# vocdoni/zk-franchise-proof-circuit

Measured on AMD Instinct MI355X. Metric: zkCensus proofs/sec (nLevels=160), higher is better.
Workload: dtype u256 (8 x u32 Montgomery, BN254 Fr/Fq)

## Files before the change

### zk-franchise-proof-circuit_amd/csrc/zkc_finalize.hip

```cpp
#include "zkc_prover.h"
#include "zkc_f29_g1.h"
#include "zkc_f29_g2.h"

namespace zkc {

template <class F>
__device__ XYZZ<F> fb_mul(const Affine<F>* __restrict__ tab, const uint32_t k[8]) {
    XYZZ<F> acc = XYZZ<F>::inf();
    for (int w = 0; w < 32; w++) {
        uint32_t limb = 0;
#pragma unroll
        for (int q = 0; q < 8; q++) limb = (q == (w >> 2)) ? k[q] : limb;
        const uint32_t d = (limb >> (8 * (w & 3))) & 0xff;
        if (d) acc = xyzz_add_affine(acc, tab[w * 255 + d - 1]);
    }
    return acc;
}
__device__ void store_fq_std(uint8_t* out, const Fq& a) {
    uint32_t s[8]; fp_to_std<FqParams>(s, a);
    uint4* d = reinterpret_cast<uint4*>(out);
    d[0] = make_uint4(s[0], s[1], s[2], s[3]); d[1] = make_uint4(s[4], s[5], s[6], s[7]);
}

__device__ G1XYZZ var_mul29(const G1XYZZ& P, const uint32_t k[8], Acc29* tab) {
    if (P.is_inf()) return P;
    f29_pt_set_inf(tab[0]); tab[1] = f29_pt_from_xyzz(P);
    for (int i = 2; i < 16; i++) { Acc29 t = tab[i - 1]; f29_pt_add(t, t, tab[1]); tab[i] = t; }
    Acc29 acc; f29_pt_set_inf(acc);
    for (int w = 63; w >= 0; w--) {
        if (!f29_pt_is_inf(acc)) for (int d = 0; d < 4; d++) f29_pt_dbl(acc, acc);
        uint32_t limb = 0;
#pragma unroll
        for (int q = 0; q < 8; q++) limb = (q == (w >> 3)) ? k[q] : limb;
        const uint32_t dg = (limb >> (4 * (w & 7))) & 15u;
        if (dg) f29_pt_add(acc, acc, tab[dg]);
    }
    return f29_pt_is_inf(acc) ? G1XYZZ::inf() : f29_pt_to_xyzz(acc);
}

__device__ G1XYZZ var_mul29_g(const G1XYZZ& P, const uint32_t k[8], Acc29* __restrict__ tab) {
    if (P.is_inf()) return P;
    { Acc29 one = f29_pt_from_xyzz(P), t = one; tab[1] = one; for (int i = 2; i < 16; i++) { f29_pt_add(t, t, one); tab[i] = t; } }
    Acc29 acc; f29_pt_set_inf(acc);
    for (int w = 63; w >= 0; w--) {
        if (!f29_pt_is_inf(acc)) for (int d = 0; d < 4; d++) f29_pt_dbl(acc, acc);
        uint32_t limb = 0;
#pragma unroll
        for (int q = 0; q < 8; q++) limb = (q == (w >> 3)) ? k[q] : limb;
        const uint32_t dg = (limb >> (4 * (w & 7))) & 15u;
        if (dg) { const Acc29 e = tab[dg]; f29_pt_add(acc, acc, e); }
    }
    return f29_pt_is_inf(acc) ? G1XYZZ::inf() : f29_pt_to_xyzz(acc);
}

template <class P>
__device__ P fold_const(const P* __restrict__ tab, const FinalizeArgs& a, int q) {
    if (a.dc[q] == 255) return P::inf();
    return xyzz_add(tab[0], xyzz_add(tab[1 + a.dc[q]], tab[1 + a.fold_n + a.ds[q]]));
}
extern "C" __global__ void __launch_bounds__(256)
zkc_finalize(FinalizeArgs a) {
    __shared__ G1XYZZ sh[8];
    __shared__ Acc29 tab[2][16];
    const int q = blockIdx.x, wave = threadIdx.x >> 6, lane = threadIdx.x & 63;
    uint32_t r[8], s[8];
    { const uint4* p = reinterpret_cast<const uint4*>(a.rs + 64 * (size_t)q); uint4 x = p[0], y = p[1], z = p[2], w = p[3];
      r[0] = x.x; r[1] = x.y; r[2] = x.z; r[3] = x.w; r[4] = y.x; r[5] = y.y; r[6] = y.z; r[7] = y.w;
      s[0] = z.x; s[1] = z.y; s[2] = z.z; s[3] = z.w; s[4] = w.x; s[5] = w.y; s[6] = w.z; s[7] = w.w; }
    const int nq = gridDim.x;
    uint8_t* out = a.out + 256 * (size_t)q;
    if (wave == 0 && lane < 2) {
        const G1XYZZ P = lane == 0 ? xyzz_add(a.r1[nq + 3 * q + 0], fold_const(a.foldA, a, q)) : xyzz_add(a.r1[nq + 3 * q + 1], fold_const(a.foldB1, a, q));
        sh[lane] = var_mul29(P, lane == 0 ? s : r, tab[lane]);
    } else if (wave == 1 && lane < 5) {
        uint32_t k[8];
        if (lane == 2) { Fr rs = fp_from_std<FrParams>(r) * fp_from_std<FrParams>(s); fp_to_std<FrParams>(k, rs); }
        else {
#pragma unroll
            for (int i = 0; i < 8; i++) k[i] = (lane == 0 || lane == 4) ? r[i] : s[i];
        }
        const G1Affine* tb = lane <= 2 ? a.tblDelta1 : lane == 3 ? a.tblAlpha1 : a.tblBeta1;
        const G1XYZZ v = fb_mul<Fq>(tb, k);
        sh[2 + lane] = v;
        if (lane == 0) {
            const G1XYZZ A = xyzz_add(a.r1[nq + 3 * q + 0], fold_const(a.foldA, a, q));
            G1Affine p = xyzz_to_affine(xyzz_add(xyzz_add_affine(A, a.alpha1), v));
            store_fq_std(out, p.x); store_fq_std(out + 32, p.y);
        }
    } else if (wave == 2 && lane == 0) {
        const G2XYZZ sd = fb_mul<Fq2>(a.tblDelta2, s);
        G2Affine p = xyzz_to_affine(xyzz_add(xyzz_add_affine(xyzz_add(a.r2[q], fold_const(a.foldB2, a, q)), a.beta2), sd));
        store_fq_std(out + 64, p.x.c0); store_fq_std(out + 96, p.x.c1); store_fq_std(out + 128, p.y.c0); store_fq_std(out + 160, p.y.c1);
    }
    __syncthreads();
    if (threadIdx.x == 0) {
        G1XYZZ c = xyzz_add(xyzz_add(a.r1[nq + 3 * q + 2], fold_const(a.foldC, a, q)), a.r1[q]);
        c = xyzz_add(c, sh[0]); c = xyzz_add(c, sh[5]); c = xyzz_add(c, sh[1]); c = xyzz_add(c, sh[6]); c = xyzz_add(c, sh[4]);
        G1Affine p = xyzz_to_affine(c);
        store_fq_std(out + 192, p.x); store_fq_std(out + 224, p.y);
    }
}

__device__ __forceinline__ void load_rs(const FinalizeArgs& a, int q, uint32_t r[8], uint32_t s[8]) {
    const uint4* p = reinterpret_cast<const uint4*>(a.rs + 64 * (size_t)q); const uint4 x = p[0], y = p[1], z = p[2], w = p[3];
    r[0] = x.x; r[1] = x.y; r[2] = x.z; r[3] = x.w; r[4] = y.x; r[5] = y.y; r[6] = y.z; r[7] = y.w;
    s[0] = z.x; s[1] = z.y; s[2] = z.z; s[3] = z.w; s[4] = w.x; s[5] = w.y; s[6] = w.z; s[7] = w.w;
}
extern "C" __global__ void __launch_bounds__(64)
zkc_finalize_products(FinalizeArgs a, int nq) {
    const int q = blockIdx.x * 64 + threadIdx.x, task = blockIdx.y;
    if (q >= nq) return;
    uint32_t r[8], s[8]; load_rs(a, q, r, s);
    G1XYZZ* res1 = reinterpret_cast<G1XYZZ*>(a.scratch);
    G2XYZZ* res2 = reinterpret_cast<G2XYZZ*>(res1 + 7 * (size_t)nq);
    Acc29* tabs = reinterpret_cast<Acc29*>(res2 + nq);
    if (task < 2) {
        const G1XYZZ P = task == 0 ? xyzz_add(a.r1[nq + 3 * q + 0], fold_const(a.foldA, a, q)) : xyzz_add(a.r1[nq + 3 * q + 1], fold_const(a.foldB1, a, q));
        res1[(size_t)task * nq + q] = var_mul29_g(P, task == 0 ? s : r, tabs + ((size_t)task * nq + q) * 16);
    } else if (task == 3) {
        return;
    } else if (task < 7) {
        uint32_t k[8];
        if (task == 4) { Fr rs = fp_from_std<FrParams>(r) * fp_from_std<FrParams>(s); fp_to_std<FrParams>(k, rs); }
        else {
#pragma unroll
            for (int i = 0; i < 8; i++) k[i] = (task == 2 || task == 6) ? r[i] : s[i];
        }
        const G1Affine* tb = task <= 4 ? a.tblDelta1 : task == 5 ? a.tblAlpha1 : a.tblBeta1;
        res1[(size_t)task * nq + q] = fb_mul<Fq>(tb, k);
    } else {
        res2[q] = fb_mul<Fq2>(a.tblDelta2, s);
    }
}
extern "C" __global__ void __launch_bounds__(64)
zkc_finalize_combine(FinalizeArgs a, int nq) {
    const int q = blockIdx.x * 64 + threadIdx.x, role = blockIdx.y;
    if (q >= nq) return;
    const G1XYZZ* res1 = reinterpret_cast<const G1XYZZ*>(a.scratch);
    const G2XYZZ* res2 = reinterpret_cast<const G2XYZZ*>(res1 + 7 * (size_t)nq);
    uint8_t* out = a.out + 256 * (size_t)q;
    if (role == 0) {
        const G1XYZZ A = xyzz_add(a.r1[nq + 3 * q + 0], fold_const(a.foldA, a, q));
        G1Affine p = xyzz_to_affine(xyzz_add(xyzz_add_affine(A, a.alpha1), res1[2 * (size_t)nq + q]));
        store_fq_std(out, p.x); store_fq_std(out + 32, p.y);
    } else if (role == 1) {
        G1XYZZ c = xyzz_add(xyzz_add(a.r1[nq + 3 * q + 2], fold_const(a.foldC, a, q)), a.r1[q]);
        c = xyzz_add(c, res1[0 * (size_t)nq + q]); c = xyzz_add(c, res1[5 * (size_t)nq + q]); c = xyzz_add(c, res1[1 * (size_t)nq + q]);
        c = xyzz_add(c, res1[6 * (size_t)nq + q]); c = xyzz_add(c, res1[4 * (size_t)nq + q]);
        G1Affine p = xyzz_to_affine(c);
        store_fq_std(out + 192, p.x); store_fq_std(out + 224, p.y);
    } else {
        G2Affine p = xyzz_to_affine(xyzz_add(xyzz_add_affine(xyzz_add(a.r2[q], fold_const(a.foldB2, a, q)), a.beta2), res2[q]));
        store_fq_std(out + 64, p.x.c0); store_fq_std(out + 96, p.x.c1); store_fq_std(out + 128, p.y.c0); store_fq_std(out + 160, p.y.c1);
    }
}

extern "C" __global__ void __launch_bounds__(64) zkc_fb4_build_g1(const G1XYZZ* __restrict__ bases, int nbases, G1XYZZ* __restrict__ out) {
    const int t = blockIdx.x * 64 + threadIdx.x, b = t >> 6, w = t & 63;
    if (b >= nbases) return;
    G1XYZZ* o = out + (size_t)t * FB4_ROW;
    const G1XYZZ B = bases[b];
    if (B.is_inf()) { for (int d = 0; d < FB4_ROW; d++) o[d] = G1XYZZ::inf(); return; }
    Acc29 P = f29_pt_from_xyzz(B);
    for (int i = 0; i < 4 * w; i++) f29_pt_dbl(P, P);
    Acc29 acc = P; o[0] = f29_pt_to_xyzz(acc);
    for (int d = 1; d < FB4_ROW; d++) { f29_pt_add(acc, acc, P); o[d] = f29_pt_to_xyzz(acc); }
}
extern "C" __global__ void __launch_bounds__(64) zkc_fb4_build_g2(G2XYZZ B, G2XYZZ beta2, G2XYZZ beta2_base, G2XYZZ* __restrict__ out) {
    const int w = threadIdx.x;
    if (w == 0) { out[(size_t)FB4_WIN * FB4_ROW] = beta2; out[(size_t)FB4_WIN * FB4_ROW + 1] = beta2_base; }
    G2XYZZ* o = out + (size_t)w * FB4_ROW;
    Acc29G2 P = f29g2_pt_from_xyzz(B);
    for (int i = 0; i < 4 * w; i++) f29g2_pt_dbl(P, P);
    Acc29G2 acc = P; o[0] = f29g2_pt_to_xyzz(acc);
    for (int d = 1; d < FB4_ROW; d++) { f29g2_pt_add(acc, acc, P); o[d] = f29g2_pt_to_xyzz(acc); }
}
int fb4_build(zkc_ctx* ctx, hipStream_t st, const G1XYZZ* d_bases, int nbases, G1XYZZ* d_out, const G2XYZZ& delta2, const G2XYZZ& beta2, const G2XYZZ& beta2_base, G2XYZZ* d_out2) {
    hipLaunchKernelGGL(zkc_fb4_build_g1, dim3(nbases), dim3(64), 0, st, d_bases, nbases, d_out);
    hipLaunchKernelGGL(zkc_fb4_build_g2, dim3(1), dim3(64), 0, st, delta2, beta2, beta2_base, d_out2);
    hipError_t e = hipGetLastError();
    if (e != hipSuccess) return zkc_fail(ctx, ZKC_ERR_HIP, std::string("zkc_fb4_build: ") + hipGetErrorString(e));
    return ZKC_OK;
}
extern "C" __global__ void __launch_bounds__(256) zkc_blind_scalars(BlindArgs a) {
    const int q = blockIdx.y >> 1, sec = blockIdx.y & 1;
    const uint32_t j = blockIdx.x * 256 + threadIdx.x, cnt = sec ? a.nB[q] : a.nA[q];
    if (j >= cnt) return;
    const uint32_t* map = sec ? a.mapB[q] : a.mapA[q];
    const uint32_t idx = map ? map[j] : j;
    const uint4* kp = reinterpret_cast<const uint4*>(a.rs + 64 * (size_t)q + (sec ? 0 : 32)); const uint4 k0 = kp[0], k1 = kp[1];
    const uint32_t ks[8] = {k0.x, k0.y, k0.z, k0.w, k1.x, k1.y, k1.z, k1.w};
    const uint4* wp = reinterpret_cast<const uint4*>(a.w[q] + 8 * (size_t)idx); const uint4 w0 = wp[0], w1 = wp[1];
    const uint32_t ws[8] = {w0.x, w0.y, w0.z, w0.w, w1.x, w1.y, w1.z, w1.w};
    uint4* o = reinterpret_cast<uint4*>(a.out[q] + ((size_t)sec * a.nv + idx) * 8);
    if ((ws[0] | ws[1] | ws[2] | ws[3] | ws[4] | ws[5] | ws[6] | ws[7]) == 0) { o[0] = make_uint4(0, 0, 0, 0); o[1] = make_uint4(0, 0, 0, 0); return; }
    uint32_t pr[8]; fp_to_std<FrParams>(pr, fp_from_std<FrParams>(ws) * fp_from_std<FrParams>(ks));
    o[0] = make_uint4(pr[0], pr[1], pr[2], pr[3]); o[1] = make_uint4(pr[4], pr[5], pr[6], pr[7]);
}
int blind_scalars_launch(zkc_ctx* ctx, hipStream_t st, const BlindArgs& a, int nproofs) {
    uint32_t mx = 1; for (int q = 0; q < nproofs; q++) mx = std::max(mx, std::max(a.nA[q], a.nB[q]));
    hipLaunchKernelGGL(zkc_blind_scalars, dim3((mx + 255) / 256, 2 * nproofs), dim3(256), 0, st, a);
    hipError_t e = hipGetLastError();
    if (e != hipSuccess) return zkc_fail(ctx, ZKC_ERR_HIP, std::string("zkc_blind_scalars: ") + hipGetErrorString(e));
    return ZKC_OK;
}

__device__ __forceinline__ uint32_t nibble_of(const uint32_t k[8], int i) {
    uint32_t limb = 0;
#pragma unroll
    for (int q = 0; q < 8; q++) limb = (q == (i >> 3)) ? k[q] : limb;
    return (limb >> (4 * (i & 7))) & 15u;
}
__device__ __forceinline__ void shfl_xor_words(uint32_t* dst, const uint32_t* src, int nwords, int mask) {
    for (int k = 0; k < nwords; k++) dst[k] = (uint32_t)__shfl_xor((int)src[k], mask, 64);
}
__device__ __forceinline__ Acc29 load_pt29(const G1XYZZ& p) { Acc29 a; if (p.is_inf()) f29_pt_set_inf(a); else a = f29_pt_from_xyzz(p); return a; }
__device__ __forceinline__ Acc29G2 load_pt29(const G2XYZZ& p) { Acc29G2 a; if (p.is_inf()) f29g2_pt_set_inf(a); else a = f29g2_pt_from_xyzz(p); return a; }
__device__ __forceinline__ void store_xyzz(uint8_t* out, const Acc29& p) {
    G1XYZZ* o = reinterpret_cast<G1XYZZ*>(out);
    if (f29_pt_is_inf(p)) *o = G1XYZZ::inf(); else *o = f29_pt_to_xyzz(p);
}
__device__ __forceinline__ void store_xyzz(uint8_t* out, const Acc29G2& p) {
    G2XYZZ* o = reinterpret_cast<G2XYZZ*>(out);
    if (f29g2_pt_is_inf(p)) *o = G2XYZZ::inf(); else *o = f29g2_pt_to_xyzz(p);
}
extern "C" __global__ void __launch_bounds__(64)
zkc_blind_tree_g1(FinalizeArgs a) {
    const int task = blockIdx.x, q = blockIdx.y, nq = gridDim.y, lane = threadIdx.x;
    uint32_t r[8], s[8]; load_rs(a, q, r, s);
    const bool folded = a.dc[q] != 255; const int n = a.fold_n, dc = a.dc[q], ds = a.ds[q];
    const G1XYZZ* res = a.r1 + nq + 5 * (size_t)q;
    Acc29* outv = reinterpret_cast<Acc29*>(a.scratch) + (size_t)q * 10 + task;
    Acc29 v; f29_pt_set_inf(v);
    if (task < 8) {
        int base; bool use_r;
        switch (task) {
            case 0: base = 0; use_r = true; break;
            case 1: base = 0; use_r = true; break;
            case 2: base = folded ? 3 : 1; use_r = false; break;
            case 3: base = folded ? 5 + dc : -1; use_r = false; break;
            case 4: base = folded ? 5 + n + ds : -1; use_r = false; break;
            case 5: base = folded ? 4 : 2; use_r = true; break;
            case 6: base = folded ? 5 + 2 * n + dc : -1; use_r = true; break;
            default: base = folded ? 5 + 3 * n + ds : -1; use_r = true; break;
        }
        uint32_t k[8];
#pragma unroll
        for (int i = 0; i < 8; i++) k[i] = use_r ? r[i] : s[i];
        if (task == 1) { const Fr rs = fp_from_std<FrParams>(r) * fp_from_std<FrParams>(s); fp_to_std<FrParams>(k, rs); }
        if (base >= 0) {
            const uint32_t d = nibble_of(k, lane);
            if (d) v = load_pt29(a.fb4[((size_t)base * FB4_WIN + lane) * FB4_ROW + d - 1]);
            v = wave_sum_g1(v);
        }
    } else if (task == 8) {
        if (lane == 0) v = load_pt29(res[0]);
        else if (lane == 1) v = load_pt29(a.fb4[((size_t)(folded ? 3 : 1) * FB4_WIN) * FB4_ROW]);
        else if (lane == 2 && folded) v = load_pt29(a.foldA[1 + dc]);
        else if (lane == 3 && folded) v = load_pt29(a.foldA[1 + n + ds]);
        v = wave_sum_g1(v, 2);
    } else {
        if (lane == 0) v = load_pt29(res[2]);
        else if (lane == 1 && folded) v = load_pt29(a.foldC[0]);
        else if (lane == 2 && folded) v = load_pt29(a.foldC[1 + dc]);
        else if (lane == 3 && folded) v = load_pt29(a.foldC[1 + n + ds]);
        else if (lane == 4) v = load_pt29(a.r1[q]);
        else if (lane == 5) v = load_pt29(res[3]);
        else if (lane == 6) v = load_pt29(res[4]);
        v = wave_sum_g1(v, 4);
    }
    if (lane == 0) *outv = v;
}
extern "C" __global__ void __launch_bounds__(128)
zkc_blind_tree_g1_out(FinalizeArgs a) {
    const int q = blockIdx.x, wave = threadIdx.x >> 6, lane = threadIdx.x & 63;
    const Acc29* sv = reinterpret_cast<const Acc29*>(a.scratch) + (size_t)q * 10;
    uint8_t* out = a.out_xyzz + 512 * (size_t)q;
    Acc29 v; f29_pt_set_inf(v);
    if (wave == 0) {
        if (lane == 0) v = sv[9]; else if (lane < 8) v = sv[lane];
        v = wave_sum_g1(v, 4);
        if (lane == 0) store_xyzz(out + 384, v);
    } else {
        if (lane == 0) v = sv[8]; else if (lane == 1) v = sv[0];
        v = wave_sum_g1(v, 1);
        if (lane == 0) store_xyzz(out, v);
    }
}
extern "C" __global__ void __launch_bounds__(128)
zkc_blind_tree_g2(FinalizeArgs a) {
    __shared__ Acc29G2 pre;
    const int q = blockIdx.x, wave = threadIdx.x >> 6, lane = threadIdx.x & 63;
    const bool folded = a.dc[q] != 255;
    Acc29G2 v; f29g2_pt_set_inf(v);
    if (wave == 0) {
        uint32_t r[8], s[8]; load_rs(a, q, r, s);
        const uint32_t d = nibble_of(s, lane);
        if (d) v = load_pt29(a.fb4g2[(size_t)lane * FB4_ROW + d - 1]);
        v = wave_sum_g2(v, 32);
    } else {
        if (lane == 0) v = load_pt29(a.r2[q]);
        else if (lane == 1) v = load_pt29(a.fb4g2[(size_t)FB4_WIN * FB4_ROW + (folded ? 1 : 0)]);
        else if (lane == 2 && folded) v = load_pt29(a.foldB2[1 + a.dc[q]]);
        else if (lane == 3 && folded) v = load_pt29(a.foldB2[1 + a.fold_n + a.ds[q]]);
        v = wave_sum_g2(v, 2);
        if (lane == 0) pre = v;
    }
    __syncthreads();
    if (threadIdx.x == 0) { Acc29G2 t; f29g2_pt_add(t, v, pre); store_xyzz(a.out_xyzz + 512 * (size_t)q + 128, t); }
}
int finalize_tree_g2_launch(zkc_ctx* ctx, hipStream_t st, const FinalizeArgs& a, int nproofs) {
    hipLaunchKernelGGL(zkc_blind_tree_g2, dim3(nproofs), dim3(128), 0, st, a);
    hipError_t e = hipGetLastError();
    if (e != hipSuccess) return zkc_fail(ctx, ZKC_ERR_HIP, std::string("zkc_blind_tree_g2: ") + hipGetErrorString(e));
    return ZKC_OK;
}

size_t finalize_scratch_bytes(int nproofs) { return (size_t)nproofs * (7 * sizeof(G1XYZZ) + sizeof(G2XYZZ) + 2 * 16 * sizeof(Acc29)); }

int finalize_launch(zkc_ctx* ctx, hipStream_t st, const FinalizeArgs& a, int nproofs) {
    const bool v1 = sw::on<sw::ZKC_FINALIZE_WAVES>();
    if (a.per == 5) {
        hipLaunchKernelGGL(zkc_blind_tree_g1, dim3(10, nproofs), dim3(64), 0, st, a);
        hipLaunchKernelGGL(zkc_blind_tree_g1_out, dim3(nproofs), dim3(128), 0, st, a);
    }
    else if (v1 || !a.scratch || nproofs <= 2) hipLaunchKernelGGL(zkc_finalize, dim3(nproofs), dim3(256), 0, st, a);
    else {
        hipLaunchKernelGGL(zkc_finalize_products, dim3((nproofs + 63) / 64, 8), dim3(64), 0, st, a, nproofs);
        hipLaunchKernelGGL(zkc_finalize_combine, dim3((nproofs + 63) / 64, 3), dim3(64), 0, st, a, nproofs);
    }
    hipError_t e = hipGetLastError();
    if (e != hipSuccess) return zkc_fail(ctx, ZKC_ERR_HIP, std::string("zkc_finalize: ") + hipGetErrorString(e));
    return ZKC_OK;
}

}
```

### zk-franchise-proof-circuit_amd/csrc/zkc_msm_sort.hip

```cpp
#include "zkc_prover.h"
#include <algorithm>

namespace zkc {

struct TileState { uint32_t s[MSM_TILE_SCALARS / MSM_TILE][8]; uint32_t pt[MSM_TILE_SCALARS / MSM_TILE]; uint32_t carry[MSM_TILE_SCALARS / MSM_TILE]; bool live[MSM_TILE_SCALARS / MSM_TILE]; };
__device__ __forceinline__ void msm_tile_load(TileState& t, const MsmJob& job, uint32_t i0) {
#pragma unroll
    for (int k = 0; k < MSM_TILE_SCALARS / MSM_TILE; k++) {
        const uint32_t i = i0 + k * MSM_TILE;
        t.live[k] = i < job.count; t.pt[k] = 0; t.carry[k] = 0;
#pragma unroll
        for (int q = 0; q < 8; q++) t.s[k][q] = 0;
        if (t.live[k]) {
            const uint32_t wire = job.vmap ? job.vmap[i] : i;
            const uint4* sp = reinterpret_cast<const uint4*>(job.scalars + 8 * (size_t)wire); const uint4 a = sp[0], b = sp[1];
            t.s[k][0] = a.x; t.s[k][1] = a.y; t.s[k][2] = a.z; t.s[k][3] = a.w; t.s[k][4] = b.x; t.s[k][5] = b.y; t.s[k][6] = b.z; t.s[k][7] = b.w;
            t.pt[k] = (uint32_t)((int32_t)wire - job.pt_shift);
        }
    }
}
__device__ __forceinline__ uint32_t msm_tile_digit(TileState& t, int k, uint32_t w, uint32_t c, uint32_t& neg) {
    const uint32_t half = 1u << (c - 1), mask = (1u << c) - 1;
    const uint32_t bit = w * c, li = bit >> 5, sh = bit & 31;
    uint32_t lo = 0, hi = 0;
#pragma unroll
    for (int q = 0; q < 8; q++) { lo = ((uint32_t)q == li) ? t.s[k][q] : lo; hi = ((uint32_t)q == li + 1) ? t.s[k][q] : hi; }
    const uint64_t two = (uint64_t)lo | ((uint64_t)hi << 32);
    uint32_t d = (uint32_t)((two >> sh) & mask) + t.carry[k];
    neg = 0;
    if (d > half) { d = (1u << c) - d; neg = 1; t.carry[k] = 1; } else t.carry[k] = 0;
    return d;
}

__global__ void __launch_bounds__(MSM_TILE)
zkc_msm_count(const MsmJobList* __restrict__ jlp, const uint16_t* __restrict__ tilejob, uint32_t* __restrict__ tilecnt) {
    __shared__ uint32_t cnt[1u << MSM_MAX_HBITS];
    const MsmJobList& jl = *jlp;
    const uint32_t j = tilejob[blockIdx.x];
    const MsmJob job = jl.job[j];
    const uint32_t nbins = 1u << job.hbits, tile = blockIdx.x - job.tile0, ntiles = (job.count + MSM_TILE_SCALARS - 1) / MSM_TILE_SCALARS;
    for (uint32_t b = threadIdx.x; b < nbins; b += MSM_TILE) cnt[b] = 0;
    __syncthreads();
    TileState t; msm_tile_load(t, job, tile * MSM_TILE_SCALARS + threadIdx.x);
    for (uint32_t w = 0; w < job.nw; w++) {
#pragma unroll
        for (int k = 0; k < MSM_TILE_SCALARS / MSM_TILE; k++) { uint32_t neg; const uint32_t d = msm_tile_digit(t, k, w, job.c, neg); if (t.live[k] && d) atomicAdd(&cnt[(d - 1) >> job.lbits], 1u); }
    }
    __syncthreads();
    for (uint32_t b = threadIdx.x; b < nbins; b += MSM_TILE) tilecnt[job.cnt0 + b * ntiles + tile] = cnt[b];
}
__global__ void __launch_bounds__(256)
zkc_msm_binscan(const MsmJobList* __restrict__ jlp, uint32_t* __restrict__ tilecnt, uint32_t* __restrict__ hist, uint32_t* __restrict__ bin_start,
                unsigned long long* __restrict__ entry_counter) {
    __shared__ uint32_t part[256];
    __shared__ uint32_t carry_sh;
    const MsmJob& job = jlp->job[blockIdx.x];
    const uint32_t nbins = 1u << job.hbits, ntiles = (job.count + MSM_TILE_SCALARS - 1) / MSM_TILE_SCALARS, total = nbins * ntiles;
    uint32_t* c = tilecnt + job.cnt0;
    if (threadIdx.x == 0) carry_sh = job.ent_off;
    __syncthreads();
    for (uint32_t base = 0; base < total; base += 1024) {
        uint32_t v[4], sum = 0;
#pragma unroll
        for (int k = 0; k < 4; k++) { const uint32_t i = base + threadIdx.x * 4 + k; v[k] = i < total ? c[i] : 0; sum += v[k]; }
        part[threadIdx.x] = sum; __syncthreads();
        for (int o = 1; o < 256; o <<= 1) { uint32_t a = (int)threadIdx.x >= o ? part[threadIdx.x - o] : 0; __syncthreads(); part[threadIdx.x] += a; __syncthreads(); }
        uint32_t run = carry_sh + part[threadIdx.x] - sum;
#pragma unroll
        for (int k = 0; k < 4; k++) { const uint32_t i = base + threadIdx.x * 4 + k; if (i < total) c[i] = run; run += v[k]; }
        __syncthreads();
        if (threadIdx.x == 255) carry_sh = run;
        __syncthreads();
    }
    const uint32_t end = carry_sh;
    if (entry_counter && threadIdx.x == 0) atomicAdd(entry_counter, (unsigned long long)(end - job.ent_off));
    for (uint32_t b = threadIdx.x; b < nbins; b += 256) {
        const uint32_t st = c[b * ntiles], en = b + 1 < nbins ? c[(b + 1) * ntiles] : end;
        bin_start[job.bin0 + b] = st; hist[job.bin0 + b] = en - st;
    }
}
__global__ void __launch_bounds__(MSM_TILE)
zkc_msm_split(const MsmJobList* __restrict__ jlp, const uint16_t* __restrict__ tilejob, const uint32_t* __restrict__ tilecnt, uint32_t* __restrict__ vals) {
    __shared__ uint32_t cur[1u << MSM_MAX_HBITS];
    const MsmJobList& jl = *jlp;
    const uint32_t j = tilejob[blockIdx.x];
    const MsmJob job = jl.job[j];
    const uint32_t nbins = 1u << job.hbits, tile = blockIdx.x - job.tile0, ntiles = (job.count + MSM_TILE_SCALARS - 1) / MSM_TILE_SCALARS;
    for (uint32_t b = threadIdx.x; b < nbins; b += MSM_TILE) cur[b] = tilecnt[job.cnt0 + b * ntiles + tile];
    TileState t; msm_tile_load(t, job, tile * MSM_TILE_SCALARS + threadIdx.x);
    const uint32_t lowmask = (1u << job.lbits) - 1, lowshift = 31 - job.lbits;
    for (uint32_t w = 0; w < job.nw; w++) {
        __syncthreads();
#pragma unroll
        for (int k = 0; k < MSM_TILE_SCALARS / MSM_TILE; k++) {
            uint32_t neg; const uint32_t d = msm_tile_digit(t, k, w, job.c, neg);
            if (t.live[k] && d) {
                const uint32_t idx = d - 1, pos = atomicAdd(&cur[idx >> job.lbits], 1u);
                vals[pos] = (neg << 31) | ((idx & lowmask) << lowshift) | (t.pt[k] + w * job.tbl_count);
            }
        }
    }
}
template <bool CHUNKED>
__global__ void __launch_bounds__(256)
zkc_msm_bucket(const MsmJobList* __restrict__ jlp, const uint32_t* __restrict__ hist, const uint32_t* __restrict__ bin_start, const uint32_t* __restrict__ vals,
               uint32_t* __restrict__ vals2, uint32_t* __restrict__ off, uint32_t* __restrict__ bcnt) {
    __shared__ uint32_t cnt[256], pos[256];
    __shared__ uint32_t stage[256 * 32];
    const MsmJobList& jl = *jlp;
    const uint32_t bin = blockIdx.x, j = jl.job_of_bin(bin);
    const MsmJob& job = jl.job[j];
    const uint32_t lbits = job.lbits, nb2 = 1u << lbits, lowshift = 31 - lbits, lowmask = nb2 - 1, rowmask = (1u << lowshift) - 1;
    const uint32_t start = bin_start[bin], n = hist[bin];
    const uint32_t bucket_first = job.bucket0 + ((bin - job.bin0) << lbits);
    constexpr int BIG = 32, SMALL = 8;
    const bool in_regs = n <= 256u * BIG;
    uint32_t e[BIG];
    cnt[threadIdx.x] = 0; __syncthreads();
    if (in_regs) {
#pragma unroll
        for (int k = 0; k < BIG; k++) { const uint32_t i = k * 256 + threadIdx.x; e[k] = i < n ? vals[start + i] : 0u; }
#pragma unroll
        for (int k = 0; k < BIG; k++) if ((uint32_t)k * 256 + threadIdx.x < n) atomicAdd(&cnt[(e[k] >> lowshift) & lowmask], 1u);
    } else {
        for (uint32_t i0 = 0; i0 < n; i0 += 256 * SMALL) {
            uint32_t v[SMALL];
#pragma unroll
            for (int k = 0; k < SMALL; k++) { const uint32_t i = i0 + k * 256 + threadIdx.x; v[k] = i < n ? vals[start + i] : 0u; }
#pragma unroll
            for (int k = 0; k < SMALL; k++) if (i0 + k * 256 + threadIdx.x < n) atomicAdd(&cnt[(v[k] >> lowshift) & lowmask], 1u);
        }
    }
    __syncthreads();
    const uint32_t mine = cnt[threadIdx.x];
    pos[threadIdx.x] = mine; __syncthreads();
    for (int o = 1; o < 256; o <<= 1) { uint32_t a = (int)threadIdx.x >= o ? pos[threadIdx.x - o] : 0; __syncthreads(); pos[threadIdx.x] += a; __syncthreads(); }
    const uint32_t excl = pos[threadIdx.x] - mine;
    __syncthreads();
    if (threadIdx.x < nb2) { off[bucket_first + threadIdx.x] = start + excl; bcnt[bucket_first + threadIdx.x] = mine; }
    pos[threadIdx.x] = excl; __syncthreads();
    constexpr uint32_t excl_base = 0;
    if (in_regs) {
#pragma unroll
        for (int k = 0; k < BIG; k++) {
            if ((uint32_t)k * 256 < n) {
                if ((uint32_t)k * 256 + threadIdx.x < n) { const uint32_t p = atomicAdd(&pos[(e[k] >> lowshift) & lowmask], 1u) - excl_base; stage[p] = (e[k] & 0x80000000u) | (e[k] & rowmask); }
                __syncthreads();
            }
        }
        for (uint32_t i = threadIdx.x; i < n; i += 256) vals2[start + i] = stage[i];
    } else if constexpr (!CHUNKED) {
        for (uint32_t i0 = 0; i0 < n; i0 += 256 * SMALL) {
            uint32_t v[SMALL];
#pragma unroll
            for (int k = 0; k < SMALL; k++) { const uint32_t i = i0 + k * 256 + threadIdx.x; v[k] = i < n ? vals[start + i] : 0u; }
#pragma unroll
            for (int k = 0; k < SMALL; k++) {
                if (i0 + k * 256 + threadIdx.x < n) { const uint32_t p = atomicAdd(&pos[(v[k] >> lowshift) & lowmask], 1u); vals2[start + p] = (v[k] & 0x80000000u) | (v[k] & rowmask); }
                __syncthreads();
            }
        }
    } else {
        uint32_t* ccnt = cnt;
        __shared__ uint32_t cbase[256];
        __shared__ uint32_t cpos[256];
        constexpr int CH = BIG / 2;
        uint8_t* sbkt = reinterpret_cast<uint8_t*>(stage + 256 * CH);
        for (uint32_t c0 = 0; c0 < n; c0 += 256u * CH) {
            const uint32_t m = n - c0 < 256u * CH ? n - c0 : 256u * CH;
            ccnt[threadIdx.x] = 0; __syncthreads();
// ... 178 lines not shown
```

### zk-franchise-proof-circuit_amd/csrc/zkc_ntt.hip

```cpp
#include "zkc_internal.h"
#include "zkc_prover.h"
#include "zkc_f29.h"
#include "zkc_kernels.h"

namespace zkc {

__device__ __forceinline__ Fr ld_fr(const Fr* p) {
    const uint4* d = reinterpret_cast<const uint4*>(p); uint4 a = d[0], b = d[1];
    Fr r; r.v[0] = a.x; r.v[1] = a.y; r.v[2] = a.z; r.v[3] = a.w; r.v[4] = b.x; r.v[5] = b.y; r.v[6] = b.z; r.v[7] = b.w; return r;
}
__device__ __forceinline__ void st_fr(Fr* p, const Fr& r) {
    uint4* d = reinterpret_cast<uint4*>(p);
    d[0] = make_uint4(r.v[0], r.v[1], r.v[2], r.v[3]); d[1] = make_uint4(r.v[4], r.v[5], r.v[6], r.v[7]);
}

constexpr uint32_t MV_UNIT = 0x80000000u, MV_NEG = 0x40000000u, MV_COL = 0x3fffffffu;
extern "C" __global__ void __launch_bounds__(256)
zkc_wtns_mont(const Fr* __restrict__ wtns_std, size_t wtns_stride, Fr* __restrict__ wm, size_t wm_stride, uint32_t nv) {
    const uint32_t i = blockIdx.x * blockDim.x + threadIdx.x;
    if (i >= nv) return;
    Fr r2;
#pragma unroll
    for (int k = 0; k < 8; k++) r2.v[k] = FrParams::r2[k];
    st_fr(wm + (size_t)blockIdx.y * wm_stride + i, ld_fr(wtns_std + (size_t)blockIdx.y * wtns_stride + i) * r2);
// ... 69 lines not shown
    o[0] = make_uint4(r[0], r[1], r[2], r[3]); o[1] = make_uint4(r[4], r[5], r[6], r[7]); o[2] = make_uint4(r[8], 0, 0, 0);
}
struct NttDom { static constexpr L9 D24 = f29_dominator<FrParams>(1u << 29, 1u << 24); static constexpr L9 D27 = f29_dominator<FrParams>(1u << 29, 1u << 27); };
__device__ __forceinline__ void ntt_ld_w(uint32_t w[9], const uint32_t* __restrict__ tw29, size_t e) {
    const uint4* wp = reinterpret_cast<const uint4*>(tw29 + (size_t)TW29_WORDS * e);
    const uint4 w0 = wp[0], w1 = wp[1], w2 = wp[2];
    w[0] = w0.x; w[1] = w0.y; w[2] = w0.z; w[3] = w0.w; w[4] = w1.x; w[5] = w1.y; w[6] = w1.z; w[7] = w1.w; w[8] = w2.x;
}
__device__ __forceinline__ void ntt_bfly(uint32_t* pu, uint32_t* pv, const uint32_t w[9], bool plain, bool carry) {
    uint32_t u[9], v[9], tt[9];
#pragma unroll
    for (int i = 0; i < 9; i++) { u[i] = pu[i]; v[i] = pv[i]; }
    if (plain) {
#pragma unroll
        for (int i = 0; i < 9; i++) { const uint32_t vi = v[i]; v[i] = u[i] + NttDom::D27.l[i] - vi; u[i] += vi; }
    } else {
        f29_mul<FrParams>(tt, v, w);
#pragma unroll
        for (int i = 0; i < 9; i++) { v[i] = u[i] + NttDom::D24.l[i] - tt[i]; u[i] += tt[i]; }
    }
    if (carry) { f29_carry(u); f29_carry(v); }
#pragma unroll
    for (int i = 0; i < 9; i++) { pu[i] = u[i]; pv[i] = v[i]; }
}
__device__ __forceinline__ void ntt_r4(uint32_t* p0, uint32_t* p1, uint32_t* p2, uint32_t* p3, const uint32_t wa[9], const uint32_t wb[9], const uint32_t wc[9], bool swap_mid) {
    uint32_t a[9], b[9], c[9], d[9], t[9];
#pragma unroll
    for (int i = 0; i < 9; i++) { a[i] = p0[i]; b[i] = p1[i]; c[i] = p2[i]; d[i] = p3[i]; }
    f29_mul<FrParams>(t, b, wa);
#pragma unroll
    for (int i = 0; i < 9; i++) { b[i] = a[i] + NttDom::D24.l[i] - t[i]; a[i] += t[i]; }
    f29_mul<FrParams>(t, d, wa);
#pragma unroll
    for (int i = 0; i < 9; i++) { d[i] = c[i] + NttDom::D24.l[i] - t[i]; c[i] += t[i]; }
    f29_mul<FrParams>(t, c, wb);
#pragma unroll
    for (int i = 0; i < 9; i++) { c[i] = a[i] + NttDom::D24.l[i] - t[i]; a[i] += t[i]; }
    f29_mul<FrParams>(t, d, wc);
#pragma unroll
    for (int i = 0; i < 9; i++) { d[i] = b[i] + NttDom::D24.l[i] - t[i]; b[i] += t[i]; }
    f29_carry(a); f29_carry(b); f29_carry(c); f29_carry(d);
    (void)swap_mid;
#pragma unroll
    for (int i = 0; i < 9; i++) { p0[i] = a[i]; p1[i] = b[i]; p2[i] = c[i]; p3[i] = d[i]; }
}
extern "C" __global__ void __launch_bounds__(256)
zkc_ntt_pass(const Fr* src_all, Fr* dst_all, const uint32_t* __restrict__ tw29, const Fr* __restrict__ scale,
             int logn, int s0, int b, int first) {
    const Fr* src = src_all + ((size_t)blockIdx.y << logn);
    Fr* dst = dst_all + ((size_t)blockIdx.y << logn);
    extern __shared__ uint32_t tile[];
    const int mid_n = 1 << b;
    const int lo_bits = s0;
    const int lo_t = (NTT_TILE >> b) < (1 << lo_bits) ? (NTT_TILE >> b) : (1 << lo_bits);
    const int tiles_per_hi = (1 << lo_bits) / lo_t;
    const int hi = blockIdx.x / tiles_per_hi, lo0 = (blockIdx.x % tiles_per_hi) * lo_t;
    const int elems = mid_n * lo_t;
    const size_t base = (size_t)hi << (s0 + b);
    for (int e = threadIdx.x; e < elems; e += blockDim.x) {
        const int mid = e / lo_t, l = e - mid * lo_t;
        size_t gi = base + ((size_t)mid << s0) + lo0 + l;
        if (first) gi = __brev((unsigned)gi) >> (32 - logn);
        const Fr x = ld_fr(src + gi);
        uint32_t t[9]; f29_from_fp_shl5(t, x.v);
#pragma unroll
        for (int k = 0; k < 9; k++) tile[9 * e + k] = t[k];
    }
    __syncthreads();
    int t = 1;
    auto single = [&](int t1, bool carry) {
        const int half = 1 << (t1 - 1);
        const int s = s0 + t1;
        for (int q = threadIdx.x; q < elems / 2; q += blockDim.x) {
            const int l = q % lo_t, pr = q / lo_t;
            const int j = pr & (half - 1), blk = pr >> (t1 - 1);
            const int m0 = (blk << t1) + j, m1 = m0 + half;
            const unsigned k = ((unsigned)j << s0) + lo0 + l;
            uint32_t w[9]; ntt_ld_w(w, tw29, (size_t)k << (logn - s));
            ntt_bfly(tile + 9 * (m0 * lo_t + l), tile + 9 * (m1 * lo_t + l), w, s == 1, carry);
        }
        __syncthreads();
    };
    if (s0 == 0) { single(1, true); t = 2; }
    for (; t + 1 <= b; t += 2) {
        const int half = 1 << (t - 1), s = s0 + t;
        for (int q = threadIdx.x; q < elems / 4; q += blockDim.x) {
            const int l = q % lo_t, u = q / lo_t;
            const int j = u & (half - 1), blk = u >> (t - 1);
            const int m = (blk << (t + 1)) + j;
            const unsigned k = ((unsigned)j << s0) + lo0 + l, kh = k + ((unsigned)half << s0);
            uint32_t wa[9], wb[9], wc[9];
            ntt_ld_w(wa, tw29, (size_t)k << (logn - s)); ntt_ld_w(wb, tw29, (size_t)k << (logn - s - 1)); ntt_ld_w(wc, tw29, (size_t)kh << (logn - s - 1));
            uint32_t* p = tile + 9 * (m * lo_t + l);
            ntt_r4(p, p + 9 * half * lo_t, p + 9 * 2 * half * lo_t, p + 9 * 3 * half * lo_t, wa, wb, wc, false);
        }
        __syncthreads();
    }
    if (t <= b) single(t, true);
    for (int e = threadIdx.x; e < elems; e += blockDim.x) {
        const int mid = e / lo_t, l = e - mid * lo_t;
        const size_t gi = base + ((size_t)mid << s0) + lo0 + l;
        uint32_t r[9];
#pragma unroll
        for (int k = 0; k < 9; k++) r[k] = tile[9 * e + k];
        if (scale) { const Fr sc = ld_fr(scale + gi); uint32_t s29[9], o[9]; f29_from_fp_shl5(s29, sc.v); f29_mul<FrParams>(o, r, s29);
#pragma unroll
            for (int k = 0; k < 9; k++) r[k] = o[k]; }
        else f29_reduce_small<FrParams>(r);
        st_fr(dst + gi, f29_to_fp<FrParams>(r));
    }
}

template <int RADIX, class Slot>
__device__ __forceinline__ void ntt_nr_stages(uint32_t* tile, Slot slot, int b, int lo_t, int q0, uint32_t prefix_of_l0, int prefix_per_l, const uint32_t* __restrict__ tw29, int logn, bool fresh) {
    const int mid_n = 1 << b;
    auto tw_of = [&](int q, uint32_t i) -> size_t { return q ? (size_t)((__brev(i) >> (32 - q)) << (logn - q - 1)) : (size_t)0; };
    int r = 0;
    if (fresh) {
        const int span = mid_n >> 1, pairs = span * lo_t;
        for (int x = threadIdx.x; x < pairs; x += blockDim.x) {
            const int l = x % lo_t, j = x / lo_t;
            uint32_t w[9] = {0, 0, 0, 0, 0, 0, 0, 0, 0};
            ntt_bfly(tile + 9 * slot(j, l), tile + 9 * slot(j + span, l), w, true, true);
        }
        __syncthreads();
        r = 1;
    }
    for (; RADIX >= 4 && r + 1 < b; r += 2) {
        const int q = q0 + r, span = mid_n >> (r + 1), hspan = span >> 1, units = (mid_n >> 2) * lo_t;
        for (int x = threadIdx.x; x < units; x += blockDim.x) {
            const int l = x % lo_t, u = x / lo_t;
            const int blk = u / hspan, j = u - blk * hspan;
            const int m = blk * 2 * span + j;
            const uint32_t i = ((prefix_of_l0 + (uint32_t)(prefix_per_l * l)) << r) | (uint32_t)blk;
            uint32_t wa[9], wb[9], wc[9];
            ntt_ld_w(wa, tw29, tw_of(q, i)); ntt_ld_w(wb, tw29, tw_of(q + 1, 2 * i)); ntt_ld_w(wc, tw29, tw_of(q + 1, 2 * i + 1));
            ntt_r4(tile + 9 * slot(m, l), tile + 9 * slot(m + span, l), tile + 9 * slot(m + hspan, l), tile + 9 * slot(m + span + hspan, l), wa, wb, wc, false);
        }
        __syncthreads();
    }
    for (; r < b; r++) {
        const int q = q0 + r, span = mid_n >> (r + 1), pairs = (mid_n >> 1) * lo_t;
        for (int x = threadIdx.x; x < pairs; x += blockDim.x) {
            const int l = x % lo_t, pr = x / lo_t;
            const int blk = pr / span, j = pr - blk * span;
            const int m0 = blk * 2 * span + j;
            const uint32_t i = ((prefix_of_l0 + (uint32_t)(prefix_per_l * l)) << r) | (uint32_t)blk;
            uint32_t w[9]; ntt_ld_w(w, tw29, tw_of(q, i));
            ntt_bfly(tile + 9 * slot(m0, l), tile + 9 * slot(m0 + span, l), w, false, RADIX >= 4 || (r & 1) == 1 || r == b - 1);
        }
        __syncthreads();
    }
}
template <int RADIX>
__device__ __forceinline__ void ntt_nr_head_body(const Fr* src_all, Fr* dst_all, const uint32_t* __restrict__ tw29, int logn, int q0, int b) {
    const Fr* src = src_all + ((size_t)blockIdx.y << logn);
    Fr* dst = dst_all + ((size_t)blockIdx.y << logn);
    extern __shared__ uint32_t tile[];
    const int mid_n = 1 << b, sh = logn - q0 - b, lo_t = NTT_TILE >> b, elems = mid_n * lo_t;
    const int bpp = (1 << sh) / lo_t;
    const uint32_t prefix = blockIdx.x / bpp;
    const size_t base = ((size_t)prefix << (logn - q0)) + (size_t)(blockIdx.x % bpp) * lo_t;
    for (int e = threadIdx.x; e < elems; e += blockDim.x) {
        const int mid = e / lo_t, l = e - mid * lo_t;
        const Fr x = ld_fr(src + (base + ((size_t)mid << sh) + l));
        uint32_t t[9]; f29_from_fp_shl5(t, x.v);
#pragma unroll
        for (int k = 0; k < 9; k++) tile[9 * e + k] = t[k];
    }
    __syncthreads();
    ntt_nr_stages<RADIX>(tile, [lo_t](int mid, int l) { return mid * lo_t + l; }, b, lo_t, q0, prefix, 0, tw29, logn, q0 == 0);
    for (int e = threadIdx.x; e < elems; e += blockDim.x) {
        const int mid = e / lo_t, l = e - mid * lo_t;
        uint32_t r[9];
#pragma unroll
        for (int k = 0; k < 9; k++) r[k] = tile[9 * e + k];
        f29_reduce_small<FrParams>(r);
        st_fr(dst + (base + ((size_t)mid << sh) + l), f29_to_fp<FrParams>(r));
    }
}
extern "C" __global__ void __launch_bounds__(256)
zkc_ntt_nr_head(const Fr* src_all, Fr* dst_all, const uint32_t* __restrict__ tw29, int logn, int q0, int b) { ntt_nr_head_body<1>(src_all, dst_all, tw29, logn, q0, b); }
extern "C" __global__ void __launch_bounds__(256)
zkc_ntt_nr_head_r4(const Fr* src_all, Fr* dst_all, const uint32_t* __restrict__ tw29, int logn, int q0, int b) { ntt_nr_head_body<4>(src_all, dst_all, tw29, logn, q0, b); }
extern "C" __global__ void __launch_bounds__(256)
zkc_ntt_mid(Fr* __restrict__ data_all, const uint32_t* __restrict__ tw_inv29, const uint32_t* __restrict__ tw_fwd29, const Fr* __restrict__ scale_br, int logn) {
    Fr* __restrict__ data = data_all + ((size_t)blockIdx.y << logn);
    extern __shared__ uint32_t tile[];
    constexpr int B = 9, MID = 1 << B, NSUB = NTT_TILE / MID;
    const size_t base = (size_t)blockIdx.x * NTT_TILE;
    for (int e = threadIdx.x; e < NTT_TILE; e += blockDim.x) {
        const Fr x = ld_fr(data + base + e);
        uint32_t t[9]; f29_from_fp_shl5(t, x.v);
#pragma unroll
        for (int k = 0; k < 9; k++) tile[9 * e + k] = t[k];
    }
    __syncthreads();
    ntt_nr_stages<4>(tile, [](int mid, int l) { return l * MID + mid; }, B, NSUB, logn - B, (uint32_t)blockIdx.x * NSUB, 1, tw_inv29, logn, false);
    for (int e = threadIdx.x; e < NTT_TILE; e += blockDim.x) {
        uint32_t r[9], s29[9], o[9];
#pragma unroll
        for (int k = 0; k < 9; k++) r[k] = tile[9 * e + k];
        const Fr sc = ld_fr(scale_br + base + e);
        f29_from_fp_shl5(s29, sc.v); f29_mul<FrParams>(o, r, s29);
#pragma unroll
        for (int k = 0; k < 9; k++) tile[9 * e + k] = o[k];
    }
    __syncthreads();
    for (int x = threadIdx.x; x < NTT_TILE / 2; x += blockDim.x) {
        const int l = x / (MID / 2), pr = x - l * (MID / 2);
        uint32_t w[9] = {0, 0, 0, 0, 0, 0, 0, 0, 0};
        ntt_bfly(tile + 9 * (l * MID + 2 * pr), tile + 9 * (l * MID + 2 * pr + 1), w, true, true);
    }
    __syncthreads();
    for (int t = 2; t + 1 <= B; t += 2) {
        const int half = 1 << (t - 1);
        for (int x = threadIdx.x; x < NTT_TILE / 4; x += blockDim.x) {
            const int l = x / (MID / 4), u = x - l * (MID / 4);
            const int j = u & (half - 1), blk = u >> (t - 1);
            const int m = (blk << (t + 1)) + j;
            uint32_t wa[9], wb[9], wc[9];
            ntt_ld_w(wa, tw_fwd29, (size_t)j << (logn - t)); ntt_ld_w(wb, tw_fwd29, (size_t)j << (logn - t - 1)); ntt_ld_w(wc, tw_fwd29, (size_t)(j + half) << (logn - t - 1));
            uint32_t* p = tile + 9 * (l * MID + m);
            ntt_r4(p, p + 9 * half, p + 9 * 2 * half, p + 9 * 3 * half, wa, wb, wc, false);
        }
        __syncthreads();
    }
    for (int e = threadIdx.x; e < NTT_TILE; e += blockDim.x) {
        uint32_t r[9];
#pragma unroll
        for (int k = 0; k < 9; k++) r[k] = tile[9 * e + k];
        f29_reduce_small<FrParams>(r);
        st_fr(data + base + e, f29_to_fp<FrParams>(r));
    }
}
extern "C" __global__ void __launch_bounds__(256)
zkc_bitrev_copy(const Fr* __restrict__ src, Fr* __restrict__ dst, int logn) {
    const uint32_t i = blockIdx.x * blockDim.x + threadIdx.x;
    if (i >> logn) return;
    st_fr(dst + i, ld_fr(src + (__brev(i) >> (32 - logn))));
}
int ntt_bitrev_table(zkc_ctx* ctx, const Fr* d_src, Fr** out, int logn) {
    ZKC_HIP_CHECK(ctx, hipMalloc((void**)out, sizeof(Fr) << logn));
    hipLaunchKernelGGL(zkc_bitrev_copy, dim3(((1u << logn) + 255) / 256), dim3(256), 0, ctx->stream, d_src, *out, logn);
    ZKC_HIP_CHECK(ctx, hipGetLastError());
    return ZKC_OK;
}
int ntt_pair_run(zkc_ctx* ctx, hipStream_t st, Fr* data, const uint32_t* tw_inv29, const uint32_t* tw_fwd29, const Fr* scale_br, int logn, int nvec) {
    if (logn < 12 || logn > 27) return zkc_fail(ctx, ZKC_ERR_BAD_ARG, "ntt_pair_run: 12 <= logn <= 27");
    const int bh = logn - 9;
    const int b1 = bh <= 9 ? bh : (bh + 1) / 2, b2 = bh - b1;
    const unsigned blocks = (1u << logn) / NTT_TILE;
    const int radix = (int)sw::value<sw::ZKC_NTT_RADIX>(4);
    auto head = radix >= 4 ? zkc_ntt_nr_head_r4 : zkc_ntt_nr_head;
    hipLaunchKernelGGL(head, dim3(blocks, nvec), dim3(256), (size_t)NTT_TILE * 36, st, (const Fr*)data, data, tw_inv29, logn, 0, b1);
    if (b2) hipLaunchKernelGGL(head, dim3(blocks, nvec), dim3(256), (size_t)NTT_TILE * 36, st, (const Fr*)data, data, tw_inv29, logn, b1, b2);
    hipLaunchKernelGGL(zkc_ntt_mid, dim3(blocks, nvec), dim3(256), (size_t)NTT_TILE * 36, st, data, tw_inv29, tw_fwd29, scale_br, logn);
    hipLaunchKernelGGL(zkc_ntt_pass, dim3(blocks, nvec), dim3(256), (size_t)NTT_TILE * 36, st, (const Fr*)data, data, tw_fwd29, (const Fr*)nullptr, logn, 9, b1, 0);
    if (b2) hipLaunchKernelGGL(zkc_ntt_pass, dim3(blocks, nvec), dim3(256), (size_t)NTT_TILE * 36, st, (const Fr*)data, data, tw_fwd29, (const Fr*)nullptr, logn, 9 + b1, b2, 0);
    hipError_t e = hipGetLastError();
    if (e != hipSuccess) return zkc_fail(ctx, ZKC_ERR_HIP, std::string("ntt_pair_run: ") + hipGetErrorString(e));
    return ZKC_OK;
}

int ntt_make_tw29(zkc_ctx* ctx, const Fr* d_tw, uint32_t count, uint32_t** out) {
    ZKC_HIP_CHECK(ctx, hipMalloc((void**)out, (size_t)count * TW29_WORDS * 4));
    hipLaunchKernelGGL(zkc_tw29, dim3((count + 255) / 256), dim3(256), 0, ctx->stream, d_tw, *out, count);
    ZKC_HIP_CHECK(ctx, hipGetLastError());
    ZKC_HIP_CHECK(ctx, hipStreamSynchronize(ctx->stream));
    return ZKC_OK;
}

int ntt_run(zkc_ctx* ctx, hipStream_t st, const Fr* src, Fr* dst, const uint32_t* tw29, const Fr* scale, int logn, int nvec) {
    int s0 = 0; bool first = true;
    while (s0 < logn) {
        int b = logn - s0 < 9 ? logn - s0 : 9;
        if (logn - s0 > 9 && logn - s0 < 18) b = (logn - s0 + 1) / 2;
        if (b > 9) b = 9;
        const int lo_t = (NTT_TILE >> b) < (1 << s0) ? (NTT_TILE >> b) : (1 << s0);
        const int nblocks = (1 << logn) / ((1 << b) * lo_t);
        const bool last = s0 + b == logn;
        hipLaunchKernelGGL(zkc_ntt_pass, dim3(nblocks, nvec), dim3(256), (size_t)(1 << b) * lo_t * 36, st,
                           first ? src : dst, dst, tw29, last ? scale : nullptr, logn, s0, b, first ? 1 : 0);
        hipError_t e = hipGetLastError();
        if (e != hipSuccess) return zkc_fail(ctx, ZKC_ERR_HIP, std::string("zkc_ntt_pass: ") + hipGetErrorString(e));
        s0 += b; first = false;
    }
    return ZKC_OK;
}

}
```

### zk-franchise-proof-circuit_amd/csrc/zkc_prove.hip

```cpp
#include "zkc_prover.h"
#include "zkc_fixedbase.h"
#include "zkc_hostparse.h"
#include "zkc_kernels.h"
#include <cstring>
#include <ctime>
#include <cstdio>
#include <algorithm>
#include <atomic>

using namespace zkc;

static void matvec_launch(zkc_zkey* zk, zkc_lane& L, const uint32_t* d_wtns0, int nb, hipStream_t mv) {
    const uint32_t n = zk->n, nv = zk->nVars;
    const bool units = zk->n_unit_coeffs > 0 && nv <= 3 * (size_t)n && sw::on<sw::ZKC_MATVEC_UNITS>();
    if (units) hipLaunchKernelGGL(zkc_wtns_mont, dim3((nv + 255) / 256, nb), dim3(256), 0, mv, (const Fr*)d_wtns0, (size_t)nv, L.d_t, 3 * (size_t)n, nv);
    hipLaunchKernelGGL(zkc_matvec_jds, dim3((2 * n + 63 * zk->nlong + 255) / 256, nb), dim3(256), 0, mv, zk->d_perm, zk->d_rowlen, zk->d_jdptr, zk->d_col, zk->d_val,
                       (const Fr*)d_wtns0, (size_t)nv, L.d_abc, (int)n, zk->nlong, units ? (const Fr*)L.d_t : (const Fr*)nullptr, 3 * (size_t)n);
    hipLaunchKernelGGL(zkc_pointwise_mul, dim3((n + 255) / 256, nb), dim3(256), 0, mv, L.d_abc, (int)n);
}
static constexpr uint32_t MATVEC_LONG = 16;

namespace {
uint32_t rd32(const uint8_t* p) { uint32_t v; memcpy(&v, p, 4); return v; }
uint64_t rd64(const uint8_t* p) { uint64_t v; memcpy(&v, p, 8); return v; }
G1Affine rd_g1(const uint8_t* p) { G1Affine a; memcpy(a.x.v, p, 32); memcpy(a.y.v, p + 32, 32); return a; }
G2Affine rd_g2(const uint8_t* p) { G2Affine a; memcpy(a.x.c0.v, p, 32); memcpy(a.x.c1.v, p + 32, 32); memcpy(a.y.c0.v, p + 64, 32); memcpy(a.y.c1.v, p + 96, 32); return a; }
Fr fr_root_of_unity(int logn) {
    uint32_t e[8]; for (int i = 0; i < 8; i++) e[i] = FrParams::p[i]; e[0] -= 1;
    for (int i = 0; i < 8; i++) e[i] = (e[i] >> 28) | (i < 7 ? e[i + 1] << 4 : 0);
    Fr g = fp_from_u32<FrParams>(5), w = Fr::one();
    for (int i = 255; i >= 0; i--) { w = w * w; if ((e[i >> 5] >> (i & 31)) & 1) w = w * g; }
    for (int i = 28; i > logn; i--) w = w * w;
    return w;
}
template <class T> int dmalloc(zkc_ctx* ctx, T** p, size_t count) { ZKC_HIP_CHECK(ctx, hipMalloc((void**)p, count * sizeof(T))); return ZKC_OK; }
void g1_to_std(uint8_t* out, const G1Affine& a) { uint32_t s[8]; fp_to_std<FqParams>(s, a.x); memcpy(out, s, 32); fp_to_std<FqParams>(s, a.y); memcpy(out + 32, s, 32); }
void g2_to_std(uint8_t* out, const G2Affine& a) {
    uint32_t s[8]; fp_to_std<FqParams>(s, a.x.c0); memcpy(out, s, 32); fp_to_std<FqParams>(s, a.x.c1); memcpy(out + 32, s, 32);
    fp_to_std<FqParams>(s, a.y.c0); memcpy(out + 64, s, 32); fp_to_std<FqParams>(s, a.y.c1); memcpy(out + 96, s, 32);
}
}

uint32_t* zkc_get_template(zkc_ctx* ctx, int nLevels);
int zkc_lane_streams(zkc_ctx* ctx, int l, bool with_red, zkc_ctx::LaneStreams* out);

extern "C" __global__ void __launch_bounds__(64)
zkc_fold_check(WitnessLayout L, const uint32_t* __restrict__ wtns, const uint32_t* __restrict__ tmpl, uint32_t* __restrict__ flags, int B) {
    const int n = L.n, g = blockIdx.x, tree = blockIdx.y, b = blockIdx.z;
    const int blk = tree == 0 ? L.off_census : L.off_sikver;
    int start, end;
    if (g < n - 1) {
        const int nctrl = (g == n - 3) + (g > 0 && g < n - 2) + 1;
        start = blk + L.lvl_off(g) + nctrl; end = blk + (g + 1 < n - 1 ? L.lvl_off(g + 1) : L.lvl_off(n - 1));
    } else { start = blk + L.off_n2bold; end = start + 253 + 127 + 133; }
    const uint4* w = reinterpret_cast<const uint4*>(wtns + (size_t)b * L.nWires * 8) + 2 * (size_t)start;
    const uint4* t = reinterpret_cast<const uint4*>(tmpl) + 2 * (size_t)start;
    uint32_t diff = 0;
    for (int i = threadIdx.x; i < 2 * (end - start); i += 64) { uint4 x = w[i], y = t[i]; diff |= (x.x ^ y.x) | (x.y ^ y.y) | (x.z ^ y.z) | (x.w ^ y.w); }
    const unsigned long long any = __ballot(diff != 0);
    if (threadIdx.x == 0) flags[((size_t)b * 2 + tree) * n + g] = any ? 1u : 0u;
}

extern "C" __global__ void __launch_bounds__(64)
zkc_input_depths(const uint32_t* __restrict__ inputs, int nInputs, int n, uint32_t* __restrict__ out) {
    const int b = blockIdx.x, tree = blockIdx.y;
    const uint32_t* sib = inputs + ((size_t)b * nInputs + 12 + (size_t)tree * n) * 8;
    int d = 0;
    for (int i = threadIdx.x; i < n; i += 64) {
        const uint4* q = reinterpret_cast<const uint4*>(sib + 8 * (size_t)i); const uint4 x = q[0], y = q[1];
        if (x.x | x.y | x.z | x.w | y.x | y.y | y.z | y.w) d = i + 1;
    }
    for (int m = 32; m >= 1; m >>= 1) { const int o = __shfl_xor(d, m, 64); d = o > d ? o : d; }
    if (threadIdx.x == 0) out[2 * b + tree] = (uint32_t)d;
}

extern "C" void zkc_zkey_free(zkc_zkey* zk) {
    if (!zk) return;
    ZKC_LOCK(zk->ctx);
    (void)hipSetDevice(zk->ctx->device);
    (void)hipStreamSynchronize(zk->ctx->stream);
    void* ptrs[] = {zk->d_perm, zk->d_rowlen, zk->d_jdptr, zk->d_col, zk->d_val, zk->d_tw_fwd, zk->d_tw_inv, zk->d_tw_fwd29, zk->d_tw_inv29, zk->d_coset, zk->d_coset_br, zk->d_g1, zk->d_g2, zk->d_g2_29, zk->d_g2_29_lone, zk->d_g2_29_deep,
                    zk->d_tblDelta1, zk->d_tblAlpha1, zk->d_tblBeta1, zk->d_tblDelta2, zk->d_fb4, zk->d_fb4g2, zk->d_depths};
    for (void* p : ptrs) if (p) (void)hipFree(p);
    for (auto& kv : zk->fold.vmaps) if (kv.second.d) (void)hipFree(kv.second.d);
    for (void* q : {(void*)zk->fold.d_foldA, (void*)zk->fold.d_foldB1, (void*)zk->fold.d_foldC, (void*)zk->fold.d_foldB2}) if (q) (void)hipFree(q);
    if (zk->h_depths) (void)hipHostFree(zk->h_depths);
    for (auto& c : zk->call) { for (void* q : {(void*)c.d_rs, (void*)c.d_proofs, (void*)c.d_flags, (void*)c.d_status3}) if (q) (void)hipFree(q); if (c.h_flags) (void)hipHostFree(c.h_flags); if (c.h_out) (void)hipHostFree(c.h_out); if (c.h_rs) (void)hipHostFree(c.h_rs); if (c.h_xyzz) (void)hipHostFree(c.h_xyzz); if (c.h_early) (void)hipHostFree(c.h_early); if (c.d_xyzz) (void)hipFree(c.d_xyzz); for (hipEvent_t e : c.ev_done) if (e) (void)hipEventDestroy(e); for (hipEvent_t e : c.ev_chunk) (void)hipEventDestroy(e); }
    if (zk->ctx->lanes) for (int l = 0; l < zk->nlanes; l++) for (hipStream_t q : {zk->ctx->lanes[l].st, zk->ctx->lanes[l].st2, zk->ctx->lanes[l].fin, zk->ctx->lanes[l].red}) if (q) (void)hipStreamSynchronize(q);
    delete zk;
}

static size_t dev_free_bytes() { size_t f = 0, t = 0; if (hipMemGetInfo(&f, &t) != hipSuccess) { (void)hipGetLastError(); return 0; } return f; }
static int fold_prepare(zkc_zkey* zk);
static int fb4_prepare(zkc_zkey* zk);
struct LaneNeed { size_t abc, p, fin, bs, e1, b1, e2, b2; int j1, j2; };
static LaneNeed lane_need(const zkc_zkey* zk, int inflight) {
    const uint32_t n = zk->n, nv = zk->nVars; const int NWS = msm_nw(zk->c_sec), NWB = msm_nw(zk->c_h);
    const size_t per_proof_entries = (size_t)NWS * 3 * nv + (size_t)NWB * n;
    const size_t per_proof_buckets = 3 * (size_t)msm_half(std::max(zk->c_sec, zk->c_deep)) + msm_half(zk->c_h);
    LaneNeed nd; nd.abc = 3 * (size_t)n * inflight; nd.p = 8 * (size_t)n * inflight; nd.fin = finalize_scratch_bytes(inflight); nd.bs = 2 * 2 * 8 * (size_t)nv;
    nd.e1 = per_proof_entries * inflight; nd.b1 = per_proof_buckets * inflight; nd.j1 = 4 * inflight;
    nd.e2 = (size_t)NWS * nv * inflight; nd.b2 = (size_t)msm_half(std::max(zk->c_sec, zk->c_deep)) * inflight; nd.j2 = inflight;
    return nd;
}
static bool lane_holds(const zkc_lane& L, const LaneNeed& nd) {
    return L.cap_abc >= nd.abc && L.cap_p >= nd.p && L.cap_fin >= nd.fin && L.cap_bs >= nd.bs && L.w1.max_entries >= nd.e1 && L.w1.max_buckets >= nd.b1 && L.w1.max_jobs >= nd.j1 &&
           L.w2.max_entries >= nd.e2 && L.w2.max_buckets >= nd.b2 && L.w2.max_jobs >= nd.j2;
}
static void lane_release(zkc_lane& L) {
    for (void** q : {(void**)&L.d_abc, (void**)&L.d_t, (void**)&L.d_p, &L.d_fin, (void**)&L.d_bs}) if (*q) { (void)hipFree(*q); *q = nullptr; }
    msm_work_free(L.w1); msm_work_free(L.w2);
    L.cap_abc = L.cap_p = L.cap_fin = L.cap_bs = 0; L.bytes = 0;
}
static zkc_lane* ctx_lanes(zkc_ctx* ctx) { if (!ctx->lanes) ctx->lanes = new zkc_lane[MAX_LANES]; return ctx->lanes; }
static size_t ctx_work_bytes(const zkc_ctx* ctx) { size_t t = 0; if (ctx->lanes) for (int l = 0; l < MAX_LANES; l++) t += ctx->lanes[l].bytes; return t; }
void zkc_ctx_lanes_destroy(zkc_ctx* ctx) {
    if (!ctx->lanes) return;
    for (int l = 0; l < MAX_LANES; l++) {
        zkc_lane& L = ctx->lanes[l];
        lane_release(L);
        for (hipEvent_t e : {L.ev_msm, L.ev_msm2, L.ev_sorted, L.ev_ntt, L.ev_mv, L.ev_acc, L.ev_fin[0], L.ev_fin[1], L.ev_red}) if (e) (void)hipEventDestroy(e);
    }
    delete[] ctx->lanes; ctx->lanes = nullptr;
}
static int lane_init(zkc_ctx* ctx, int l) {
    zkc_lane& L = ctx_lanes(ctx)[l];
    if (L.made) return ZKC_OK;
    zkc_ctx::LaneStreams ls; int rc = zkc_lane_streams(ctx, l, sw::on<sw::ZKC_REDUCE_STREAM>(), &ls); if (rc) return rc;
    L.st = ls.st; L.st2 = ls.st2; L.fin = ls.fin; L.red = ls.red;
    for (hipEvent_t* e : {&L.ev_msm, &L.ev_msm2, &L.ev_sorted, &L.ev_ntt, &L.ev_mv, &L.ev_acc, &L.ev_fin[0], &L.ev_fin[1], &L.ev_red}) if (!*e) ZKC_HIP_CHECK(ctx, hipEventCreateWithFlags(e, hipEventDisableTiming));
    L.made = true; return ZKC_OK;
}
struct LaneSt { hipStream_t st, st2, fin, red; };
static LaneSt lane_st(const zkc_zkey* zk, const zkc_lane& L) { hipStream_t c = zk->ctx->stream; return zk->serial_streams ? LaneSt{c, c, c, c} : LaneSt{L.st, L.st2, L.fin, L.red}; }
static int lane_ensure(zkc_zkey* zk, int l, int inflight) {
    zkc_ctx* ctx = zk->ctx; int rc;
    if ((rc = lane_init(ctx, l))) return rc;
    zkc_lane& L = ctx->lanes[l];
    inflight = std::max(1, std::min(inflight, zk->max_inflight));
    if (lane_holds(L, lane_need(zk, inflight))) return ZKC_OK;
    inflight = std::min(inflight <= 4 ? 4 : zk->max_inflight, zk->max_inflight);
    LaneNeed nd = lane_need(zk, inflight);
    nd.abc = std::max(nd.abc, L.cap_abc); nd.p = std::max(nd.p, L.cap_p); nd.fin = std::max(nd.fin, L.cap_fin); nd.bs = std::max(nd.bs, L.cap_bs);
    nd.e1 = std::max(nd.e1, L.w1.max_entries); nd.b1 = std::max(nd.b1, L.w1.max_buckets); nd.j1 = std::max(nd.j1, L.w1.max_jobs);
    nd.e2 = std::max(nd.e2, L.w2.max_entries); nd.b2 = std::max(nd.b2, L.w2.max_buckets); nd.j2 = std::max(nd.j2, L.w2.max_jobs);
    for (hipStream_t q : {L.st, L.st2, L.fin, L.red}) if (q) ZKC_HIP_CHECK(ctx, hipStreamSynchronize(q));
    ZKC_HIP_CHECK(ctx, hipStreamSynchronize(ctx->stream));
    lane_release(L);
    const size_t free_before = dev_free_bytes();
    const auto fail_at = sw::given<sw::ZKC_TEST_FAIL_ALLOC>();
    rc = (fail_at && inflight >= *fail_at) ? zkc_fail(ctx, ZKC_ERR_HIP, "lanes_ensure: allocation failure injected by ZKC_TEST_FAIL_ALLOC") : ZKC_OK;
    if (!rc) rc = dmalloc(ctx, &L.d_abc, nd.abc);
    if (!rc) rc = dmalloc(ctx, &L.d_t, nd.abc);
    if (!rc) rc = dmalloc(ctx, &L.d_p, nd.p);
    if (!rc && hipMalloc(&L.d_fin, nd.fin) != hipSuccess) rc = zkc_fail(ctx, ZKC_ERR_HIP, "lanes_ensure: hipMalloc failed (blinding scratch)");
    if (!rc) rc = dmalloc(ctx, &L.d_bs, nd.bs);
    if (!rc) rc = msm_work_alloc(ctx, L.w1, nd.e1, nd.b1, nd.j1, false);
    if (!rc) rc = msm_work_alloc(ctx, L.w2, nd.e2, nd.b2, nd.j2, true);
    if (rc) { (void)hipGetLastError(); lane_release(L); return rc; }
    L.cap_abc = nd.abc; L.cap_p = nd.p; L.cap_fin = nd.fin; L.cap_bs = nd.bs;
    { const size_t f = dev_free_bytes(); L.bytes = free_before > f ? free_before - f : 0; }
    return ZKC_OK;
}
static int lanes_ensure(zkc_zkey* zk, int inflight, int first = 0, int count = -1) {
    if (count < 0) count = zk->nlanes - first;
    for (int l = first; l < first + count && l < zk->nlanes; l++) { const int rc = lane_ensure(zk, l, inflight); if (rc) return rc; }
    return ZKC_OK;
}
extern "C" int zkc_zkey_load(zkc_ctx* ctx, const void* zkey_bytes, size_t len, zkc_zkey** out) { return zkc::zkey_load_opts(ctx, zkey_bytes, len, 0, 0, out); }
size_t zkc::zkey_device_bytes(const zkc_zkey* zk, size_t* tables, size_t* work) {
    if (!zk) return 0;
    const size_t w = ctx_work_bytes(zk->ctx);
    if (tables) *tables = zk->bytes_tables; if (work) *work = w;
    return zk->bytes_tables + w;
}
int zkc::zkey_load_opts(zkc_ctx* ctx, const void* zkey_bytes, size_t len, int opt_lanes, int opt_inflight, zkc_zkey** out) {
    if (!ctx || !zkey_bytes || !out) return zkc_fail(ctx, ZKC_ERR_BAD_ARG, "zkc_zkey_load: bad argument");
    ZKC_LOCK(ctx);
    ZKC_HIP_CHECK(ctx, hipSetDevice(ctx->device));
    const size_t free_at_entry = dev_free_bytes(), work_at_entry = ctx_work_bytes(ctx);
    const uint8_t* buf = (const uint8_t*)zkey_bytes;
    parse::BinSections bs; parse::ZkeyHeader zh; std::string perr;
    if (!parse::binfile_sections(buf, len, "zkey", 1, bs, perr) || !parse::zkey_check(bs, zh, perr)) return zkc_fail(ctx, ZKC_ERR_FORMAT, perr);
    const uint8_t* const* sec = bs.sec;
    const uint8_t* h = sec[2];
    zkc_zkey* zk = new zkc_zkey(); zk->ctx = ctx;
    zk->nVars = zh.nVars; zk->nPub = zh.nPub; zk->n = zh.n; zk->logn = zh.logn; zk->nCoeffs = zh.nCoeffs;
    parse::sha256(buf, len, zk->sha256); parse::zkey_fingerprint(buf, len, bs, zk->fingerprint);
    const uint32_t n = zk->n, nv = zk->nVars, np = zk->nPub, nc = nv - np - 1;
    zk->alpha1 = rd_g1(h + 84); zk->beta1 = rd_g1(h + 148); zk->beta2 = rd_g2(h + 212); zk->gamma2 = rd_g2(h + 340);
    zk->delta1 = rd_g1(h + 468); zk->delta2 = rd_g2(h + 532);
    for (uint32_t i = 0; i <= np; i++) zk->ic.push_back(rd_g1(sec[3] + 64ull * i));
    {
        auto zero64 = [](const uint8_t* q) { for (int i = 0; i < 64; i++) if (q[i]) return false; return true; };
        zk->fold.infA.resize(nv); zk->fold.infB.resize(nv); zk->fold.infC.assign(nv, 0);
        for (uint32_t i = 0; i < nv; i++) { zk->fold.infA[i] = zero64(sec[5] + 64ull * i); zk->fold.infB[i] = zero64(sec[6] + 64ull * i); if (i > np) zk->fold.infC[i] = zero64(sec[8] + 64ull * (i - np - 1)); }
    }
    if (np == 8 && !sw::on<sw::ZKC_NO_FOLD>()) for (int nl = 3; nl <= 253; nl++) if ((uint32_t)WitnessLayout::make(nl).nWires == nv) { zk->nLevels = nl; break; }
    int rc = ZKC_OK;
    auto bail = [&](int code) { zkc_zkey_free(zk); return code; };
#define ZKC_HIP_BAIL(call)                                                                                      \
    do { hipError_t _e = (call); if (_e != hipSuccess) return bail(zkc_fail(ctx, ZKC_ERR_HIP, std::string(#call) + ": " + hipGetErrorString(_e))); } while (0)
#define ZKC_UP(dst, src, bytes) ZKC_HIP_BAIL(hipMemcpy((dst), (src), (bytes), hipMemcpyHostToDevice))
    {
        std::vector<uint32_t> rowptr(2 * (size_t)n + 1, 0), col(zk->nCoeffs); std::vector<Fr> val(zk->nCoeffs);
        const uint8_t* c = sec[4] + 4;
        for (uint32_t i = 0; i < zk->nCoeffs; i++) {
            uint32_t m = rd32(c + 44ull * i), cc = rd32(c + 44ull * i + 4), s = rd32(c + 44ull * i + 8);
            rowptr[(size_t)m * n + cc + 1]++;
        }
        for (size_t r = 0; r < 2 * (size_t)n; r++) rowptr[r + 1] += rowptr[r];
        std::vector<uint32_t> fill(rowptr.begin(), rowptr.end() - 1);
        for (uint32_t i = 0; i < zk->nCoeffs; i++) {
            uint32_t m = rd32(c + 44ull * i), cc = rd32(c + 44ull * i + 4), s = rd32(c + 44ull * i + 8);
            uint32_t k = fill[(size_t)m * n + cc]++;
            col[k] = s; memcpy(val[k].v, c + 44ull * i + 12, 32);
        }
        const size_t nrows = 2 * (size_t)n;
        std::vector<uint32_t> perm(nrows), rowlen(nrows);
        for (size_t r = 0; r < nrows; r++) perm[r] = (uint32_t)r;
        std::stable_sort(perm.begin(), perm.end(), [&](uint32_t a, uint32_t b) { return rowptr[a + 1] - rowptr[a] > rowptr[b + 1] - rowptr[b]; });
        for (size_t r = 0; r < nrows; r++) rowlen[r] = rowptr[perm[r] + 1] - rowptr[perm[r]];
        const uint32_t maxlen = nrows ? rowlen[0] : 0;
        zk->nlong = 0; while (zk->nlong < nrows && rowlen[zk->nlong] > MATVEC_LONG) zk->nlong++;
        std::vector<uint32_t> jdptr(maxlen + 1, 0);
        { size_t live = nrows; for (uint32_t k = 0; k < maxlen; k++) { while (live > 0 && rowlen[live - 1] <= k) live--; jdptr[k + 1] = jdptr[k] + (uint32_t)live; } }
        std::vector<uint32_t> jcol(zk->nCoeffs); std::vector<Fr> jval(zk->nCoeffs);
        if (nv >= (1u << 30)) return bail(zkc_fail(ctx, ZKC_ERR_FORMAT, "zkey too large for 30-bit wire indices"));
        Fr one_r2, neg_r2; for (int i = 0; i < 8; i++) one_r2.v[i] = FrParams::r2[i];
        neg_r2 = Fr::zero() - one_r2;
        zk->n_unit_coeffs = 0;
        for (size_t r = 0; r < nrows; r++) for (uint32_t k = 0; k < rowlen[r]; k++) {
            const size_t dst = (size_t)jdptr[k] + r, src = (size_t)rowptr[perm[r]] + k;
            uint32_t c = col[src];
            if (val[src] == one_r2) { c |= 0x80000000u; zk->n_unit_coeffs++; } else if (val[src] == neg_r2) { c |= 0xc0000000u; zk->n_unit_coeffs++; }
            jcol[dst] = c; jval[dst] = val[src];
        }
        if ((rc = dmalloc(ctx, &zk->d_perm, nrows)) || (rc = dmalloc(ctx, &zk->d_rowlen, nrows)) || (rc = dmalloc(ctx, &zk->d_jdptr, jdptr.size())) ||
            (rc = dmalloc(ctx, &zk->d_col, jcol.size() + 1)) || (rc = dmalloc(ctx, &zk->d_val, jval.size() + 1))) return bail(rc);
        ZKC_UP(zk->d_perm, perm.data(), nrows * 4); ZKC_UP(zk->d_rowlen, rowlen.data(), nrows * 4); ZKC_UP(zk->d_jdptr, jdptr.data(), jdptr.size() * 4);
        ZKC_UP(zk->d_col, jcol.data(), jcol.size() * 4);
        ZKC_UP(zk->d_val, jval.data(), jval.size() * sizeof(Fr));
    }
    {
        const Fr w = fr_root_of_unity((int)zk->logn), g = fr_root_of_unity((int)zk->logn + 1);
        const Fr wi = fp_inv<FrParams>(w), ninv = fp_inv<FrParams>(fp_from_u32<FrParams>(n));
        std::vector<Fr> f(n / 2), b(n / 2), cs(n);
        f[0] = b[0] = Fr::one(); for (uint32_t i = 1; i < n / 2; i++) { f[i] = f[i - 1] * w; b[i] = b[i - 1] * wi; }
        cs[0] = ninv; for (uint32_t i = 1; i < n; i++) cs[i] = cs[i - 1] * g;
        if ((rc = dmalloc(ctx, &zk->d_tw_fwd, n / 2)) || (rc = dmalloc(ctx, &zk->d_tw_inv, n / 2)) || (rc = dmalloc(ctx, &zk->d_coset, n))) return bail(rc);
        ZKC_UP(zk->d_tw_fwd, f.data(), f.size() * sizeof(Fr));
        ZKC_UP(zk->d_tw_inv, b.data(), b.size() * sizeof(Fr));
        ZKC_UP(zk->d_coset, cs.data(), cs.size() * sizeof(Fr));
        if ((rc = ntt_make_tw29(ctx, zk->d_tw_fwd, n / 2, &zk->d_tw_fwd29)) || (rc = ntt_make_tw29(ctx, zk->d_tw_inv, n / 2, &zk->d_tw_inv29))) return bail(rc);
        if ((rc = ntt_bitrev_table(ctx, zk->d_coset, &zk->d_coset_br, (int)zk->logn))) return bail(rc);
    }
    { const auto e_c = sw::given<sw::ZKC_C_SECTIONS>(); zk->c_sec = e_c ? (int)*e_c : zk->nLevels >= 0 ? MSM_C_SMALL : msm_c_for(nv); }
    { const auto e_h = sw::given<sw::ZKC_C_H>(); zk->c_h = e_h ? (int)*e_h : zk->nLevels >= 0 ? MSM_C_BIG : std::max(msm_c_for(n), n >= 12000 ? 15 : 12); }
    const int NWS = msm_nw(zk->c_sec);
    { const int dt = (int)sw::value<sw::ZKC_DEEP_TABLES>(1); const auto e_c = sw::given<sw::ZKC_C_DEEP>();
      const int cd = e_c ? (int)*e_c : msm_c_for(dt == 2 ? (size_t)40000 : (size_t)nv * 4 / 5);
      zk->c_deep = (zk->nLevels >= 0 && (nv >= (1u << 16) || dt == 2) && zk->c_sec < cd && dt != 0) ? cd : 0; }
    zk->c_h = std::max(zk->c_h, std::max(zk->c_sec, zk->c_deep));
    const int NWB = msm_nw(zk->c_h);
    zk->offA = 0; zk->offB1 = NWS * nv; zk->offC = 2 * NWS * nv; zk->offH = 2 * NWS * nv + NWS * nc;
    const int NWD = zk->c_deep ? msm_nw(zk->c_deep) : 0;
    zk->offA_deep = zk->offH + NWB * n; zk->offB1_deep = zk->offA_deep + NWD * nv; zk->offC_deep = zk->offB1_deep + NWD * nv;
    const size_t g1_points = (size_t)NWS * (2 * (size_t)nv + nc) + (size_t)NWB * n + (size_t)NWD * (2 * (size_t)nv + nc);
    if (g1_points >= (1ull << 31)) return bail(zkc_fail(ctx, ZKC_ERR_FORMAT, "zkey too large for 31-bit point indices"));
    if ((rc = dmalloc(ctx, &zk->d_g1, g1_points)) || (rc = dmalloc(ctx, &zk->d_g2, (size_t)NWS * nv))) return bail(rc);
    ZKC_UP(zk->d_g1 + zk->offA, sec[5], 64ull * nv); ZKC_UP(zk->d_g1 + zk->offB1, sec[6], 64ull * nv);
    ZKC_UP(zk->d_g1 + zk->offC, sec[8], 64ull * nc); ZKC_UP(zk->d_g1 + zk->offH, sec[9], 64ull * n);
    ZKC_UP(zk->d_g2, sec[7], 128ull * nv);
    if ((rc = msm_precompute_g1(ctx, nv, zk->d_g1 + zk->offA, zk->c_sec)) || (rc = msm_precompute_g1(ctx, nv, zk->d_g1 + zk->offB1, zk->c_sec)) ||
        (rc = msm_precompute_g1(ctx, nc, zk->d_g1 + zk->offC, zk->c_sec)) || (rc = msm_precompute_g1(ctx, n, zk->d_g1 + zk->offH, zk->c_h)) ||
        (rc = msm_precompute_g2(ctx, nv, zk->d_g2, zk->c_sec))) return bail(rc);
    if ((rc = dmalloc(ctx, &zk->d_g2_29, 60 * (size_t)NWS * nv)) || (rc = msm_g2_table29(ctx, zk->d_g2, zk->d_g2_29, (size_t)NWS * nv))) return bail(rc);
    if (zk->c_deep) {
        ZKC_UP(zk->d_g1 + zk->offA_deep, sec[5], 64ull * nv); ZKC_UP(zk->d_g1 + zk->offB1_deep, sec[6], 64ull * nv); ZKC_UP(zk->d_g1 + zk->offC_deep, sec[8], 64ull * nc);
        if ((rc = msm_precompute_g1(ctx, nv, zk->d_g1 + zk->offA_deep, zk->c_deep)) || (rc = msm_precompute_g1(ctx, nv, zk->d_g1 + zk->offB1_deep, zk->c_deep)) ||
            (rc = msm_precompute_g1(ctx, nc, zk->d_g1 + zk->offC_deep, zk->c_deep))) return bail(rc);
        G2Affine* tmp = nullptr;
        if ((rc = dmalloc(ctx, &tmp, (size_t)NWD * nv))) return bail(rc);
        hipError_t e2 = hipMemcpyAsync(tmp, zk->d_g2, 128ull * nv, hipMemcpyDeviceToDevice, ctx->stream);
        if (e2 == hipSuccess) rc = msm_precompute_g2(ctx, nv, tmp, zk->c_deep);
        if (e2 == hipSuccess && !rc) rc = dmalloc(ctx, &zk->d_g2_29_deep, 60 * (size_t)NWD * nv);
        if (e2 == hipSuccess && !rc) rc = msm_g2_table29(ctx, tmp, zk->d_g2_29_deep, (size_t)NWD * nv);
        if (e2 == hipSuccess && !rc) e2 = hipStreamSynchronize(ctx->stream);
        (void)hipFree(tmp);
        if (rc) return bail(rc);
        if (e2 != hipSuccess) return bail(zkc_fail(ctx, ZKC_ERR_HIP, std::string("second section tables: ") + hipGetErrorString(e2)));
    }
    {
        if (sw::on<sw::ZKC_G2_LONE_TABLE>() && (zk->nLevels >= 0 || nv < (1u << 16))) {
            constexpr int NWL = msm_nw(MSM_C_G2_LONE);
            G2Affine* tmp = nullptr;
            if ((rc = dmalloc(ctx, &tmp, (size_t)NWL * nv))) return bail(rc);
            hipError_t e2 = hipMemcpyAsync(tmp, zk->d_g2, 128ull * nv, hipMemcpyDeviceToDevice, ctx->stream);
            if (e2 == hipSuccess) rc = msm_precompute_g2(ctx, nv, tmp, MSM_C_G2_LONE);
            if (e2 == hipSuccess && !rc) rc = dmalloc(ctx, &zk->d_g2_29_lone, 60 * (size_t)NWL * nv);
            if (e2 == hipSuccess && !rc) rc = msm_g2_table29(ctx, tmp, zk->d_g2_29_lone, (size_t)NWL * nv);
            if (e2 == hipSuccess && !rc) e2 = hipStreamSynchronize(ctx->stream);
            (void)hipFree(tmp);
            if (rc) return bail(rc);
            if (e2 != hipSuccess) return bail(zkc_fail(ctx, ZKC_ERR_HIP, std::string("lone-proof G2 table: ") + hipGetErrorString(e2)));
        }
    }
    const auto e_inf = sw::given<sw::ZKC_INFLIGHT>();
    zk->max_inflight = opt_inflight > 0 ? std::min(opt_inflight, MSM_MAX_JOBS / 4) : e_inf ? (int)*e_inf : zk->nLevels >= 0 ? 64 : 96;
    {
        const size_t per_proof_entries = (size_t)NWS * 3 * nv + (size_t)NWB * n, census_pass = 96ull * (22ull * 3 * 82754 + 15ull * 131072);
        const int fit = (int)std::max<size_t>(1, census_pass / std::max<size_t>(per_proof_entries, 1));
        zk->max_inflight = std::min(zk->max_inflight, fit);
    }
    { const auto e_l = sw::given<sw::ZKC_LANES>(); zk->nlanes = opt_lanes > 0 ? std::min(opt_lanes, (int)MAX_LANES) : e_l ? (int)*e_l : zk->nLevels >= 0 ? (int)MAX_LANES : 1; }
    zk->serial_streams = sw::on<sw::ZKC_SERIAL_STREAMS>();
    if ((rc = lanes_ensure(zk, 1, 0, 1))) return bail(rc);
    {
        FixedBase<Fq> td(zk->delta1), ta(zk->alpha1), tb(zk->beta1); FixedBase<Fq2> t2(zk->delta2);
        if ((rc = dmalloc(ctx, &zk->d_tblDelta1, td.tab.size())) || (rc = dmalloc(ctx, &zk->d_tblAlpha1, ta.tab.size())) ||
            (rc = dmalloc(ctx, &zk->d_tblBeta1, tb.tab.size())) || (rc = dmalloc(ctx, &zk->d_tblDelta2, t2.tab.size()))) return bail(rc);
        ZKC_UP(zk->d_tblDelta1, td.tab.data(), td.tab.size() * sizeof(G1Affine)); ZKC_UP(zk->d_tblAlpha1, ta.tab.data(), ta.tab.size() * sizeof(G1Affine));
        ZKC_UP(zk->d_tblBeta1, tb.tab.data(), tb.tab.size() * sizeof(G1Affine)); ZKC_UP(zk->d_tblDelta2, t2.tab.data(), t2.tab.size() * sizeof(G2Affine));
    }
    ZKC_HIP_BAIL(hipStreamSynchronize(ctx->stream));
    if (zk->nLevels >= 0 && (rc = fold_prepare(zk))) return bail(rc);
    if ((rc = fb4_prepare(zk))) return bail(rc);
    { const size_t f = dev_free_bytes(), grown = ctx_work_bytes(ctx) > work_at_entry ? ctx_work_bytes(ctx) - work_at_entry : 0; zk->bytes_tables = free_at_entry > f + grown ? free_at_entry - f - grown : 0; }
    *out = zk;
    return ZKC_OK;
#undef ZKC_UP
#undef ZKC_HIP_BAIL
}

int zkc::prove_reserve(zkc_zkey* zk, int inflight) {
    if (!zk) return ZKC_ERR_BAD_ARG;
    ZKC_LOCK(zk->ctx);
    ZKC_HIP_CHECK(zk->ctx, hipSetDevice(zk->ctx->device));
    return lanes_ensure(zk, inflight);
}
extern "C" int zkc_zkey_pass_info(const zkc_zkey* zk, int* pass_size, int* lanes) {
    if (!zk) return ZKC_ERR_BAD_ARG;
    if (pass_size) *pass_size = zk->max_inflight; if (lanes) *lanes = zk->nlanes;
    return ZKC_OK;
}
extern "C" int zkc_zkey_info(const zkc_zkey* zk, uint32_t* nVars, uint32_t* nPublic, uint32_t* domainSize) {
    if (!zk) return ZKC_ERR_BAD_ARG;
    if (nVars) *nVars = zk->nVars; if (nPublic) *nPublic = zk->nPub; if (domainSize) *domainSize = zk->n;
    return ZKC_OK;
}

static std::vector<std::pair<int, int>> fold_group_ranges(const WitnessLayout& L, int tree) {
    std::vector<std::pair<int, int>> r; const int n = L.n, blk = tree == 0 ? L.off_census : L.off_sikver;
    for (int g = 0; g < n - 1; g++) {
        const int nctrl = (g == n - 3) + (g > 0 && g < n - 2) + 1;
        r.push_back({blk + L.lvl_off(g) + nctrl, blk + (g + 1 < n - 1 ? L.lvl_off(g + 1) : L.lvl_off(n - 1))});
    }
    r.push_back({blk + L.off_n2bold, blk + L.off_n2bold + 253 + 127 + 133});
    return r;
}
template <class X> static void suffix_sums(std::vector<X>& suf, const X* g, int n) {
    suf.assign(n, X::inf());
    for (int D = n - 2; D >= 0; D--) suf[D] = xyzz_add(suf[D + 1], g[D]);
}
template <class PT> static int fold_upload(zkc_ctx* ctx, PT** d, const std::vector<PT>& b, const std::vector<PT>* suf) {
    std::vector<PT> t; t.push_back(b[0]); t.insert(t.end(), suf[0].begin(), suf[0].end()); t.insert(t.end(), suf[1].begin(), suf[1].end());
    ZKC_HIP_CHECK(ctx, hipMalloc((void**)d, t.size() * sizeof(PT)));
    ZKC_HIP_CHECK(ctx, hipMemcpy(*d, t.data(), t.size() * sizeof(PT), hipMemcpyHostToDevice));
    return ZKC_OK;
}
static int fold_prepare(zkc_zkey* zk) {
    if (zk->fold.ready) return ZKC_OK;
    zkc_ctx* ctx = zk->ctx; const WitnessLayout L = WitnessLayout::make(zk->nLevels); const int n = L.n;
    uint32_t* tmpl = zkc_get_template(ctx, zk->nLevels); if (!tmpl) return ZKC_ERR_HIP;
    std::vector<uint32_t> wires, gstart;
    for (int tree = 0; tree < 2; tree++) for (auto& rg : fold_group_ranges(L, tree)) { gstart.push_back((uint32_t)wires.size()); for (int w = rg.first; w < rg.second; w++) wires.push_back((uint32_t)w); }
    gstart.push_back((uint32_t)wires.size());
    const uint32_t ng = 2 * n;
    uint32_t *d_w = nullptr, *d_g = nullptr;
    ZKC_HIP_CHECK(ctx, hipMalloc((void**)&d_w, wires.size() * 4)); ZKC_HIP_CHECK(ctx, hipMalloc((void**)&d_g, gstart.size() * 4));
    ZKC_HIP_CHECK(ctx, hipMemcpy(d_w, wires.data(), wires.size() * 4, hipMemcpyHostToDevice));
    ZKC_HIP_CHECK(ctx, hipMemcpy(d_g, gstart.data(), gstart.size() * 4, hipMemcpyHostToDevice));
    std::vector<G1XYZZ> gA(ng), gB1(ng), gC(ng); std::vector<G2XYZZ> gB2(ng);
    int rc;
    if ((rc = fold_group_sums_g1(ctx, zk->d_g1 + zk->offA, tmpl, d_w, (uint32_t)wires.size(), 0, d_g, ng, gA.data())) ||
        (rc = fold_group_sums_g1(ctx, zk->d_g1 + zk->offB1, tmpl, d_w, (uint32_t)wires.size(), 0, d_g, ng, gB1.data())) ||
        (rc = fold_group_sums_g1(ctx, zk->d_g1 + zk->offC, tmpl, d_w, (uint32_t)wires.size(), (int32_t)zk->nPub + 1, d_g, ng, gC.data())) ||
        (rc = fold_group_sums_g2(ctx, zk->d_g2, tmpl, d_w, (uint32_t)wires.size(), 0, d_g, ng, gB2.data()))) return rc;
    ZKC_HIP_CHECK(ctx, hipFree(d_w)); ZKC_HIP_CHECK(ctx, hipFree(d_g));
    auto& f = zk->fold;
    for (int t = 0; t < 2; t++) {
        suffix_sums(f.sufA[t], gA.data() + t * n, n); suffix_sums(f.sufB1[t], gB1.data() + t * n, n);
        suffix_sums(f.sufC[t], gC.data() + t * n, n); suffix_sums(f.sufB2[t], gB2.data() + t * n, n);
    }
    f.baseA = {xyzz_add(gA[n - 1], gA[2 * n - 1])}; f.baseB1 = {xyzz_add(gB1[n - 1], gB1[2 * n - 1])};
    f.baseC = {xyzz_add(gC[n - 1], gC[2 * n - 1])}; f.baseB2 = {xyzz_add(gB2[n - 1], gB2[2 * n - 1])};
    if ((rc = fold_upload(ctx, &f.d_foldA, f.baseA, f.sufA)) || (rc = fold_upload(ctx, &f.d_foldB1, f.baseB1, f.sufB1)) || (rc = fold_upload(ctx, &f.d_foldC, f.baseC, f.sufC)) ||
        (rc = fold_upload(ctx, &f.d_foldB2, f.baseB2, f.sufB2))) return rc;
    f.ready = true;
    return ZKC_OK;
}
static int fb4_prepare(zkc_zkey* zk) {
    if (!sw::on<sw::ZKC_BLIND_TREE>() || zk->d_fb4) return ZKC_OK;
    zkc_ctx* ctx = zk->ctx;
    std::vector<G1XYZZ> bases = {G1XYZZ::from_affine(zk->delta1), G1XYZZ::from_affine(zk->alpha1), G1XYZZ::from_affine(zk->beta1)};
    const auto& f = zk->fold;
    if (f.ready) {
        bases.push_back(xyzz_add_affine(f.baseA[0], zk->alpha1)); bases.push_back(xyzz_add_affine(f.baseB1[0], zk->beta1));
        for (int t = 0; t < 2; t++) bases.insert(bases.end(), f.sufA[t].begin(), f.sufA[t].end());
        for (int t = 0; t < 2; t++) bases.insert(bases.end(), f.sufB1[t].begin(), f.sufB1[t].end());
    }
    G1XYZZ* d_bases = nullptr; int rc;
    if ((rc = dmalloc(ctx, &d_bases, bases.size()))) return rc;
    if ((rc = dmalloc(ctx, &zk->d_fb4, bases.size() * FB4_WIN * FB4_ROW)) || (rc = dmalloc(ctx, &zk->d_fb4g2, (size_t)FB4_WIN * FB4_ROW + 2))) { (void)hipFree(d_bases); return rc; }
    hipError_t e = hipMemcpyAsync(d_bases, bases.data(), bases.size() * sizeof(G1XYZZ), hipMemcpyHostToDevice, ctx->stream);
    if (e == hipSuccess) { rc = fb4_build(ctx, ctx->stream, d_bases, (int)bases.size(), zk->d_fb4, G2XYZZ::from_affine(zk->delta2), G2XYZZ::from_affine(zk->beta2),
                                             f.ready ? xyzz_add_affine(f.baseB2[0], zk->beta2) : G2XYZZ::from_affine(zk->beta2), zk->d_fb4g2); if (!rc) e = hipStreamSynchronize(ctx->stream); }
    (void)hipFree(d_bases);
    if (rc || e != hipSuccess) {
        (void)hipFree(zk->d_fb4); (void)hipFree(zk->d_fb4g2); zk->d_fb4 = nullptr; zk->d_fb4g2 = nullptr;
        return rc ? rc : zkc_fail(ctx, ZKC_ERR_HIP, std::string("fb4_prepare: ") + hipGetErrorString(e));
    }
    zk->fb4_bases = (int)bases.size();
    return ZKC_OK;
}
static int fold_vmap(zkc_zkey* zk, int Dc, int Ds, zkc_zkey::Fold::VMap* out) {
    auto it = zk->fold.vmaps.find({Dc, Ds});
    if (it != zk->fold.vmaps.end()) { *out = it->second; return ZKC_OK; }
    zkc_ctx* ctx = zk->ctx; const WitnessLayout L = WitnessLayout::make(zk->nLevels); const int n = L.n;
    std::vector<uint8_t> folded(L.nWires, 0);
    for (int tree = 0; tree < 2; tree++) {
        auto rg = fold_group_ranges(L, tree); const int D = tree == 0 ? Dc : Ds;
        for (int g = D; g < n - 1; g++) for (int w = rg[g].first; w < rg[g].second; w++) folded[w] = 1;
        for (int w = rg[n - 1].first; w < rg[n - 1].second; w++) folded[w] = 1;
    }
    std::vector<uint32_t> v; zkc_zkey::Fold::VMap m;
    m.offA = 0; for (int w = 0; w < L.nWires; w++) if (!folded[w] && !zk->fold.infA[w]) v.push_back((uint32_t)w); m.nA = (uint32_t)v.size();
    m.offB = (uint32_t)v.size(); for (int w = 0; w < L.nWires; w++) if (!folded[w] && !zk->fold.infB[w]) v.push_back((uint32_t)w); m.nB = (uint32_t)v.size() - m.offB;
    m.offC = (uint32_t)v.size(); for (int w = (int)zk->nPub + 1; w < L.nWires; w++) if (!folded[w] && !zk->fold.infC[w]) v.push_back((uint32_t)w); m.nC = (uint32_t)v.size() - m.offC;
    ZKC_HIP_CHECK(ctx, hipMalloc((void**)&m.d, v.size() * 4 + 4));
    ZKC_HIP_CHECK(ctx, hipMemcpyAsync(m.d, v.data(), v.size() * 4, hipMemcpyHostToDevice, ctx->stream));
    ZKC_HIP_CHECK(ctx, hipStreamSynchronize(ctx->stream));
    zk->fold.vmaps[{Dc, Ds}] = m; *out = m;
    return ZKC_OK;
}

static int nofold_vmap(zkc_zkey* zk, zkc_zkey::Fold::VMap* out) {
    auto it = zk->fold.vmaps.find({-1, -1});
    if (it != zk->fold.vmaps.end()) { *out = it->second; return ZKC_OK; }
    zkc_ctx* ctx = zk->ctx; const uint32_t nv = zk->nVars, np = zk->nPub;
    std::vector<uint32_t> v; zkc_zkey::Fold::VMap m;
    m.offA = 0; for (uint32_t w = 0; w < nv; w++) if (!zk->fold.infA[w]) v.push_back(w); m.nA = (uint32_t)v.size();
    m.offB = (uint32_t)v.size(); for (uint32_t w = 0; w < nv; w++) if (!zk->fold.infB[w]) v.push_back(w); m.nB = (uint32_t)v.size() - m.offB;
    m.offC = (uint32_t)v.size(); for (uint32_t w = np + 1; w < nv; w++) if (!zk->fold.infC[w]) v.push_back(w); m.nC = (uint32_t)v.size() - m.offC;
    if ((size_t)m.nA + m.nB + m.nC + (size_t)nv / 50 < 3 * (size_t)nv - np - 1) {
        ZKC_HIP_CHECK(ctx, hipMalloc((void**)&m.d, v.size() * 4 + 4));
        ZKC_HIP_CHECK(ctx, hipMemcpyAsync(m.d, v.data(), v.size() * 4, hipMemcpyHostToDevice, ctx->stream));
        ZKC_HIP_CHECK(ctx, hipStreamSynchronize(ctx->stream));
    }
    zk->fold.vmaps[{-1, -1}] = m; *out = m;
    return ZKC_OK;
}

static int h_matvec_dev(zkc_zkey* zk, zkc_lane& L, const uint32_t* d_wtns0, int nb, hipStream_t mv) {
    zkc_ctx* ctx = zk->ctx; const uint32_t n = zk->n, nv = zk->nVars;
    zkc_prof_scope _ps(ctx, ZKC_PROF_MATVEC, (uint64_t)nb * ((uint64_t)zk->nCoeffs * 68 + 3ull * n * 32), mv);
    matvec_launch(zk, L, d_wtns0, nb, mv);
    ZKC_HIP_CHECK(ctx, hipGetLastError());
    return ZKC_OK;
}
static int h_evals_dev(zkc_zkey* zk, zkc_lane& L, hipStream_t st, const uint32_t* d_wtns0, int nb, bool with_matvec = true) {
    zkc_ctx* ctx = zk->ctx; const uint32_t n = zk->n;
    if (with_matvec) { int rc0 = h_matvec_dev(zk, L, d_wtns0, nb, st); if (rc0) return rc0; }
    zkc_prof_scope _pn(ctx, ZKC_PROF_NTT, (uint64_t)nb * (6ull * 2 * n * 32 + 4ull * n * 32), st);
    int rc;
    if (!sw::on<sw::ZKC_NTT_SEPARATE>() && zk->logn >= 12 && zk->logn <= 27) {
        if ((rc = ntt_pair_run(ctx, st, L.d_abc, zk->d_tw_inv29, zk->d_tw_fwd29, zk->d_coset_br, (int)zk->logn, 3 * nb))) return rc;
    } else {
        if ((rc = ntt_run(ctx, st, L.d_abc, L.d_t, zk->d_tw_inv29, zk->d_coset, (int)zk->logn, 3 * nb))) return rc;
        if ((rc = ntt_run(ctx, st, L.d_t, L.d_abc, zk->d_tw_fwd29, nullptr, (int)zk->logn, 3 * nb))) return rc;
    }
    hipLaunchKernelGGL(zkc_join_abc, dim3((n + 255) / 256, nb), dim3(256), 0, st, L.d_abc, L.d_p, (int)n);
    ZKC_HIP_CHECK(ctx, hipGetLastError());
    return ZKC_OK;
}

extern "C" int zkc_debug_stage(zkc_zkey* zk, const void* d_wtns, int stage, void* host_out) {
    if (!zk || !d_wtns || !host_out) return ZKC_ERR_BAD_ARG;
    zkc_ctx* ctx = zk->ctx; const uint32_t n = zk->n;
    ZKC_LOCK(ctx);
    ZKC_HIP_CHECK(ctx, hipSetDevice(ctx->device)); ZKC_HIP_CHECK(ctx, hipStreamSynchronize(ctx->stream));
    { int rc0 = lanes_ensure(zk, 1, 0, 1); if (rc0) return rc0; }
    zkc_lane& L0 = ctx->lanes[0]; const hipStream_t st0 = lane_st(zk, L0).st;
    if (stage == 0) {
        matvec_launch(zk, L0, (const uint32_t*)d_wtns, 1, st0);
        ZKC_HIP_CHECK(ctx, hipGetLastError());
        ZKC_HIP_CHECK(ctx, hipMemcpyAsync(host_out, L0.d_abc, 96ull * n, hipMemcpyDeviceToHost, st0));
    } else {
        int rc = h_evals_dev(zk, L0, st0, (const uint32_t*)d_wtns, 1); if (rc) return rc;
        ZKC_HIP_CHECK(ctx, hipMemcpyAsync(host_out, L0.d_p, 32ull * n, hipMemcpyDeviceToHost, st0));
    }
    ZKC_HIP_CHECK(ctx, hipStreamSynchronize(st0));
    return ZKC_OK;
}

extern "C" int zkc_msm_debug(zkc_zkey* zk, int which, const void* d_scalars, uint32_t count, void* host_out) {
    if (!zk || !d_scalars || !host_out || which < 0 || which > 4) return ZKC_ERR_BAD_ARG;
    zkc_ctx* ctx = zk->ctx;
    ZKC_LOCK(ctx);
    ZKC_HIP_CHECK(ctx, hipSetDevice(ctx->device)); ZKC_HIP_CHECK(ctx, hipStreamSynchronize(ctx->stream));
    { int rc0 = lanes_ensure(zk, 1, 0, 1); if (rc0) return rc0; }
    zkc_lane& L0 = ctx->lanes[0]; const hipStream_t st_l0 = lane_st(zk, L0).st;
    const uint32_t full = which == 3 ? zk->nVars - zk->nPub - 1 : which == 4 ? zk->n : zk->nVars;
    if (count != full) return zkc_fail(ctx, ZKC_ERR_BAD_ARG, "zkc_msm_debug: count must equal the section size");
    static thread_local MsmJobList jl; jl.clear(256, 1024, which == 2 ? (uint32_t)MSM_MAX_VW_PER_JOB : (uint32_t)MSM_MAX_VW_G1);
    const uint32_t offs[5] = {zk->offA, zk->offB1, 0, zk->offC, zk->offH};
    jl.add((const uint32_t*)d_scalars, nullptr, count, offs[which], full, 0, which == 4 ? zk->c_h : zk->c_sec);
    int rc = which == 2 ? msm_pass_g2(zk, L0.w2, jl, 0, true, st_l0) : msm_pass_g1(zk, L0.w1, jl, 0, true, st_l0); if (rc) return rc;
    ZKC_HIP_CHECK(ctx, hipStreamSynchronize(st_l0));
    if (which == 2) g2_to_std((uint8_t*)host_out, xyzz_to_affine(*(G2XYZZ*)L0.w2.h_results));
    else g1_to_std((uint8_t*)host_out, xyzz_to_affine(*(G1XYZZ*)L0.w1.h_results));
    return ZKC_OK;
}

int zkc_witness_chunk_async(zkc_ctx* ctx, int nLevels, const void* d_inputs, int B, void* d_wtns, int32_t* d_status3, int32_t* d_status, hipStream_t st);
int zkc::prove_batch_begin(zkc_zkey* zk, int cs, const void* d_wtns, uint32_t nWitness, int B, const uint8_t* rs, bool want_publics, const void* d_inputs, int32_t* d_status,
                           int lane0, hipEvent_t wait_first, const uint8_t* host_depths, bool no_early) {
    if (!zk || !d_wtns || !rs || B <= 0 || cs < 0 || cs >= CALL_SLOTS || lane0 >= zk->nlanes) return zkc_fail(zk ? zk->ctx : nullptr, ZKC_ERR_BAD_ARG, "zkc_prove_batch_dev: bad argument");
    zkc_ctx* ctx = zk->ctx;
    ZKC_LOCK(ctx);
    if (nWitness != zk->nVars) return zkc_fail(ctx, ZKC_ERR_INVALID_WITNESS_LENGTH, "Invalid witness length. Circuit: " + std::to_string(zk->nVars) + ", witness: " + std::to_string(nWitness));
    for (int b = 0; b < 2 * B; b++) { uint32_t t[8]; memcpy(t, rs + 32 * (size_t)b, 32); if (!fp_std_lt_p<FrParams>(t)) return zkc_fail(ctx, ZKC_ERR_BAD_ARG, "r or s >= field order"); }
    ZKC_HIP_CHECK(ctx, hipSetDevice(ctx->device));
    const uint32_t nv = zk->nVars, np = zk->nPub, nc = nv - np - 1, n = zk->n;
    const bool can_fold = zk->nLevels >= 0;
    WitnessLayout L{}; int rc;
    {
        const int npasses0 = (B + zk->max_inflight - 1) / zk->max_inflight, per0 = (B + npasses0 - 1) / npasses0;
        if ((rc = lanes_ensure(zk, per0, lane0 >= 0 ? lane0 : 0, lane0 >= 0 ? 1 : std::min(zk->nlanes, npasses0)))) return rc;
    }
    hipStream_t st0 = (lane0 >= 0 && !zk->serial_streams && B <= zk->max_inflight) ? ctx->lanes[lane0].st : ctx->stream;
    zkc_zkey::CallSlot& CS = zk->call[cs];
    if (CS.pending) return zkc_fail(ctx, ZKC_ERR_BAD_ARG, "prove_batch_begin: this call slot has a call in flight (finish it first)");
    if (CS.cap < (size_t)B) {
        if (CS.d_rs) { ZKC_HIP_CHECK(ctx, hipFree(CS.d_rs)); ZKC_HIP_CHECK(ctx, hipFree(CS.d_proofs)); ZKC_HIP_CHECK(ctx, hipHostFree(CS.h_out)); ZKC_HIP_CHECK(ctx, hipHostFree(CS.h_rs)); ZKC_HIP_CHECK(ctx, hipFree(CS.d_xyzz)); ZKC_HIP_CHECK(ctx, hipHostFree(CS.h_xyzz));
                       CS.d_rs = CS.d_proofs = CS.h_out = CS.h_rs = CS.d_xyzz = CS.h_xyzz = nullptr; CS.cap = 0; }
        const size_t want = std::max<size_t>((size_t)B, std::max<size_t>(256, std::min<size_t>(2 * CS.cap, 4096)));
        ZKC_HIP_CHECK(ctx, hipMalloc((void**)&CS.d_rs, 64 * want)); ZKC_HIP_CHECK(ctx, hipMalloc((void**)&CS.d_proofs, 256 * want));
        ZKC_HIP_CHECK(ctx, hipHostMalloc((void**)&CS.h_out, (256 + 32 * (size_t)zk->nPub) * want)); ZKC_HIP_CHECK(ctx, hipHostMalloc((void**)&CS.h_rs, 64 * want));
        ZKC_HIP_CHECK(ctx, hipMalloc((void**)&CS.d_xyzz, 512 * want)); ZKC_HIP_CHECK(ctx, hipHostMalloc((void**)&CS.h_xyzz, 512 * want)); CS.cap = want;
    }
    static const unsigned ev_host_flags = hipEventDisableTiming;
    for (int l = 0; l < zk->nlanes; l++) if (!CS.ev_done[l]) ZKC_HIP_CHECK(ctx, hipEventCreateWithFlags(&CS.ev_done[l], ev_host_flags));
    CS.as_xyzz.assign((size_t)B, 0); CS.lanes_used = 0;
    if (wait_first) ZKC_HIP_CHECK(ctx, hipStreamWaitEvent(st0, wait_first, 0));
    uint8_t* const h_pub = CS.h_out + 256ull * CS.cap;
    if (rs != CS.h_rs_copy.data()) CS.h_rs_copy.assign(rs, rs + 64 * (size_t)B);
    memcpy(CS.h_rs, rs, 64 * (size_t)B);
    ZKC_HIP_CHECK(ctx, hipMemcpyAsync(CS.d_rs, CS.h_rs, 64 * (size_t)B, hipMemcpyHostToDevice, st0));
    uint32_t* tmpl = nullptr;
    if (can_fold) {
        L = WitnessLayout::make(zk->nLevels);
        if ((rc = fold_prepare(zk))) return rc;
        tmpl = zkc_get_template(ctx, zk->nLevels); if (!tmpl) return ZKC_ERR_HIP;
        const size_t nflags = (size_t)B * 2 * L.n;
        if (CS.flags_cap < nflags) {
            if (CS.d_flags) { ZKC_HIP_CHECK(ctx, hipFree(CS.d_flags)); ZKC_HIP_CHECK(ctx, hipHostFree(CS.h_flags)); CS.d_flags = CS.h_flags = nullptr; CS.flags_cap = 0; }
            const size_t want = std::max(nflags, (size_t)256 * 2 * L.n);
            ZKC_HIP_CHECK(ctx, hipMalloc((void**)&CS.d_flags, want * 4)); ZKC_HIP_CHECK(ctx, hipHostMalloc((void**)&CS.h_flags, want * 4)); CS.flags_cap = want;
        }
    }
    CS.early_n = 0; CS.arg_wtns = d_wtns; CS.arg_nw = nWitness; CS.arg_publics = want_publics; CS.arg_lane0 = lane0; CS.arg_inputs = d_inputs != nullptr; CS.arg_wait = nullptr;
    const size_t ecap = MSM_MAX_JOBS / 4;
    const bool early_wanted = !no_early && can_fold && B <= zk->max_inflight && (B <= 2 ? zk->d_fb4 != nullptr : sw::on<sw::ZKC_EARLY_LAYOUT>());
    if (early_wanted && !CS.h_early) { ZKC_HIP_CHECK(ctx, hipHostMalloc((void**)&CS.h_early, (ecap + ecap * 2 * 256) * 4)); CS.early_cap = ecap; }
    if (early_wanted && host_depths) {
        bool ok = true; for (int i = 0; i < 2 * B; i++) ok = ok && host_depths[i] < (uint8_t)L.n && L.n <= 255;
        if (ok) { CS.early_n = B; CS.early_depth.assign(host_depths, host_depths + 2 * (size_t)B); }
    } else if (early_wanted && d_inputs) {
        if (!zk->d_depths) { ZKC_HIP_CHECK(ctx, hipMalloc((void**)&zk->d_depths, 2 * ecap * 4)); ZKC_HIP_CHECK(ctx, hipHostMalloc((void**)&zk->h_depths, 2 * ecap * 4)); }
        uint32_t* hd = zk->h_depths;
        if (wait_first) ZKC_HIP_CHECK(ctx, hipStreamWaitEvent(ctx->stream2, wait_first, 0));
        hipLaunchKernelGGL(zkc_input_depths, dim3(B, 2), dim3(64), 0, ctx->stream2, (const uint32_t*)d_inputs, L.nInputs, L.n, zk->d_depths);
        ZKC_HIP_CHECK(ctx, hipGetLastError());
        ZKC_HIP_CHECK(ctx, hipMemcpyAsync(hd, zk->d_depths, 8 * (size_t)B, hipMemcpyDeviceToHost, ctx->stream2));
        ZKC_HIP_CHECK(ctx, hipStreamSynchronize(ctx->stream2));
        bool ok = true; for (int i = 0; i < 2 * B; i++) ok = ok && hd[i] < (uint32_t)L.n;
        if (ok) { CS.early_n = B; CS.early_depth.resize(2 * (size_t)B); for (int i = 0; i < 2 * B; i++) CS.early_depth[i] = (uint8_t)hd[i]; }
    }
    const int npasses = (B + zk->max_inflight - 1) / zk->max_inflight;
    const int per_pass = (B + npasses - 1) / npasses;
    while ((int)CS.ev_chunk.size() < npasses) { hipEvent_t e; ZKC_HIP_CHECK(ctx, hipEventCreateWithFlags(&e, ev_host_flags)); CS.ev_chunk.push_back(e); }
    int32_t* d_status3 = nullptr;
    if (d_inputs) {
        if ((rc = zkc_ensure(ctx, (void**)&CS.d_status3, &CS.status3_cap, std::max<size_t>((size_t)B, 256) * 3 * sizeof(int32_t)))) return rc;
        d_status3 = CS.d_status3;
    }
    const int wgroup = (int)sw::value<sw::ZKC_WITNESS_GROUP>(8);
    for (int c = 0; c < npasses; c++) {
        const int p0 = c * per_pass, nb = std::min(per_pass, B - p0);
        uint32_t* wc = (uint32_t*)d_wtns + (size_t)p0 * nv * 8;
        if (d_inputs && (c % wgroup == 0 || c == 1)) {
            const int glast = c == 0 ? 1 : std::min(((c / wgroup) + 1) * wgroup, npasses);
            const int g0 = p0, gn = std::min((glast - c) * per_pass, B - g0);
            if (gn > 0 && (rc = zkc_witness_chunk_async(ctx, zk->nLevels, (const uint8_t*)d_inputs + (size_t)g0 * L.nInputs * 32, gn, wc, d_status3 + 3 * (size_t)g0, d_status + g0, st0))) return rc;
        }
        if (can_fold) {
            uint32_t* fl = CS.d_flags + (size_t)p0 * 2 * L.n;
            hipLaunchKernelGGL(zkc_fold_check, dim3(L.n, 2, nb), dim3(64), 0, st0, L, (const uint32_t*)wc, tmpl, fl, nb);
            ZKC_HIP_CHECK(ctx, hipGetLastError());
            ZKC_HIP_CHECK(ctx, hipMemcpyAsync(CS.h_flags + (size_t)p0 * 2 * L.n, fl, (size_t)nb * 2 * L.n * 4, hipMemcpyDeviceToHost, st0));
        }
        if (CS.early_n) {
            if (d_status) ZKC_HIP_CHECK(ctx, hipMemcpyAsync(CS.h_early, d_status, 4 * (size_t)B, hipMemcpyDeviceToHost, st0));
            else memset(CS.h_early, 0, 4 * (size_t)B);
            ZKC_HIP_CHECK(ctx, hipMemcpyAsync(CS.h_early + CS.early_cap, CS.d_flags + (size_t)p0 * 2 * L.n, (size_t)nb * 2 * L.n * 4, hipMemcpyDeviceToHost, st0));
        }
        ZKC_HIP_CHECK(ctx, hipEventRecord(CS.ev_chunk[c], st0));
    }
    const bool trace_host = sw::on<sw::ZKC_TRACE_HOST>();
    auto now_ms = [] { timespec t; clock_gettime(CLOCK_MONOTONIC, &t); return t.tv_sec * 1e3 + t.tv_nsec * 1e-6; };
    const double t_begin = now_ms(); double tr[6] = {0};
    int pass = 0, done_on_st_lane = -1;
    const bool one_lane = lane0 >= 0 || zk->nlanes == 1;
    for (int p0 = 0; p0 < B; p0 += per_pass, pass++) {
        const int nb = std::min(per_pass, B - p0);
        const int li = lane0 >= 0 ? lane0 : pass % zk->nlanes; CS.lanes_used |= 1u << li;
        zkc_lane& LN = ctx->lanes[li]; const LaneSt LS = lane_st(zk, LN); const int slot = LN.npass & 1;
        tr[0] = now_ms();
        const bool early = CS.early_n > 0;
        if (!early) ZKC_HIP_CHECK(ctx, zkc_wait_event(CS.ev_chunk[pass]));
        tr[1] = now_ms();
        ZKC_HIP_CHECK(ctx, hipStreamWaitEvent(LS.st, CS.ev_chunk[pass], 0)); ZKC_HIP_CHECK(ctx, hipStreamWaitEvent(LS.st2, CS.ev_chunk[pass], 0));
        hipStream_t st = LS.st, st2 = LS.st2, fin = LS.fin;
        const uint32_t* w0 = (const uint32_t*)d_wtns + (size_t)p0 * nv * 8;
        uint8_t dcq[MSM_MAX_JOBS / 4], dsq[MSM_MAX_JOBS / 4]; bool fold = can_fold;
        if (early) for (int q = 0; q < nb; q++) { dcq[q] = CS.early_depth[2 * q]; dsq[q] = CS.early_depth[2 * q + 1]; }
        else for (int q = 0; q < nb && fold; q++) for (int t = 0; t < 2; t++) {
            const uint32_t* f = CS.h_flags + ((size_t)(p0 + q) * 2 + t) * L.n;
            if (f[L.n - 1]) { fold = false; break; }
            int D = 0; for (int g = 0; g < L.n - 1; g++) if (f[g]) D = g + 1;
            (t == 0 ? dcq : dsq)[q] = (uint8_t)D;
        }
        static thread_local zkc_zkey::Fold::VMap vms[MSM_MAX_JOBS / 4];
        if (fold) for (int q = 0; q < nb; q++) if ((rc = fold_vmap(zk, dcq[q], dsq[q], &vms[q]))) return rc;
        const bool nofold_lists = sw::on<sw::ZKC_NOFOLD_LISTS>();
        if (!fold && nofold_lists) {
            zkc_zkey::Fold::VMap nf; if ((rc = nofold_vmap(zk, &nf))) return rc;
            for (int q = 0; q < nb; q++) vms[q] = nf;
        }
        const bool listed = fold || (nofold_lists && vms[0].d != nullptr);
        if (LN.npass >= 2) { ZKC_HIP_CHECK(ctx, hipStreamWaitEvent(st, LN.ev_fin[slot], 0)); ZKC_HIP_CHECK(ctx, hipStreamWaitEvent(st2, LN.ev_fin[slot], 0)); }
        LN.npass++;
        const bool mv_prefetch = !sw::on<sw::ZKC_MATVEC_INLINE>() && one_lane;
        const bool mv_done = mv_prefetch && pass > 0;
        if (mv_done) ZKC_HIP_CHECK(ctx, hipStreamWaitEvent(st, LN.ev_mv, 0));
        if ((rc = h_evals_dev(zk, LN, st, w0, nb, !mv_done))) return rc;
        ZKC_HIP_CHECK(ctx, hipEventRecord(LN.ev_ntt, st));
        tr[2] = now_ms();
        static thread_local MsmJobList j1, j2;
        const uint32_t vwb_env = (uint32_t)sw::value<sw::ZKC_VW_BIG>(0), vws_env = (uint32_t)sw::value<sw::ZKC_VW_SMALL>(0);
        const uint32_t vws = nb <= 4 ? 64u : vws_env ? vws_env : nb < 32 ? 256u : 2048u, vwb = nb <= 4 ? 256u : vwb_env ? vwb_env : nb < 32 ? 1024u : 4096u;
        size_t lone_entries = 0; for (int q = 0; q < nb; q++) lone_entries += (size_t)msm_nw(MSM_C_G2_LONE) * (listed ? vms[q].nB : nv);
        const size_t deep_wires = (size_t)sw::value<sw::ZKC_DEEP_WIRES>(16000);
        size_t live_wires = 0; for (int q = 0; q < nb; q++) live_wires += listed ? (size_t)vms[q].nA + vms[q].nB + vms[q].nC : 2 * (size_t)nv + nc;
        const bool deep = zk->c_deep != 0 && nb > 2 && live_wires >= 3 * deep_wires * (size_t)nb;
        const int cw = deep ? zk->c_deep : zk->c_sec;
        const uint32_t oA = deep ? zk->offA_deep : zk->offA, oB1 = deep ? zk->offB1_deep : zk->offB1, oC = deep ? zk->offC_deep : zk->offC;
        const int c2 = (nb <= 2 && zk->d_g2_29_lone && lone_entries <= LN.w2.max_entries) ? MSM_C_G2_LONE : cw;
        const uint32_t vwg2_env = (uint32_t)sw::value<sw::ZKC_VW_G2>(0);
        j1.clear(vws, vwb, MSM_MAX_VW_G1); j2.clear(c2 == MSM_C_G2_LONE ? 128u : (vwg2_env && nb >= 32) ? vwg2_env : vws, 1024, MSM_MAX_VW_PER_JOB);
        for (int q = 0; q < nb; q++) j1.add(LN.d_p + 8 * (size_t)n * q, nullptr, n, zk->offH, n, 0, zk->c_h);
        size_t tree_entries = 0; for (int q = 0; q < nb; q++) tree_entries += (size_t)msm_nw(zk->c_h) * n + (size_t)msm_nw(zk->c_sec) * (listed ? 2 * (size_t)vms[q].nA + 2 * (size_t)vms[q].nB + vms[q].nC : 4 * (size_t)nv + nc);
        const bool tree = zk->d_fb4 != nullptr && nb <= 2 && 6 * nb <= LN.w1.max_jobs && tree_entries <= LN.w1.max_entries && (size_t)nb * (5 * msm_half(zk->c_sec) + msm_half(zk->c_h)) <= LN.w1.max_buckets;
        BlindArgs ba{}; ba.rs = CS.d_rs + 64 * (size_t)p0; ba.nv = nv;
        for (int q = 0; q < nb; q++) {
            const uint32_t* w = w0 + (size_t)q * nv * 8;
            uint32_t* bs = tree ? LN.d_bs + (size_t)q * 2 * nv * 8 : nullptr;
            if (tree) { ba.w[q] = w; ba.out[q] = bs; }
            if (listed) {
                const zkc_zkey::Fold::VMap& vm = vms[q];
                j1.add(w, vm.d + vm.offA, vm.nA, oA, nv, 0, cw);
                j1.add(w, vm.d + vm.offB, vm.nB, oB1, nv, 0, cw);
                j1.add(w, vm.d + vm.offC, vm.nC, oC, nc, (int32_t)np + 1, cw);
                if (tree) { j1.add(bs, vm.d + vm.offA, vm.nA, oA, nv, 0, cw); j1.add(bs + 8ull * nv, vm.d + vm.offB, vm.nB, oB1, nv, 0, cw); }
                j2.add(w, vm.d + vm.offB, vm.nB, 0, nv, 0, c2);
                if (tree) { ba.mapA[q] = vm.d + vm.offA; ba.nA[q] = vm.nA; ba.mapB[q] = vm.d + vm.offB; ba.nB[q] = vm.nB; }
            } else {
                j1.add(w, nullptr, nv, oA, nv, 0, cw);
                j1.add(w, nullptr, nv, oB1, nv, 0, cw);
                j1.add(w + 8ull * (np + 1), nullptr, nc, oC, nc, 0, cw);
                if (tree) { j1.add(bs, nullptr, nv, oA, nv, 0, cw); j1.add(bs + 8ull * nv, nullptr, nv, oB1, nv, 0, cw); }
                j2.add(w, nullptr, nv, 0, nv, 0, c2);
                if (tree) { ba.mapA[q] = ba.mapB[q] = nullptr; ba.nA[q] = ba.nB[q] = nv; }
            }
        }
        if (tree && (rc = blind_scalars_launch(ctx, st, ba, nb))) return rc;
        FinalizeArgs fa{};
        fa.r1 = (const G1XYZZ*)LN.w1.results + (size_t)slot * LN.w1.max_jobs; fa.r2 = (const G2XYZZ*)LN.w2.results + (size_t)slot * LN.w2.max_jobs;
        fa.foldA = zk->fold.d_foldA; fa.foldB1 = zk->fold.d_foldB1; fa.foldC = zk->fold.d_foldC; fa.foldB2 = zk->fold.d_foldB2; fa.fold_n = can_fold ? L.n : 0;
        for (int q = 0; q < nb; q++) { fa.dc[q] = fold ? dcq[q] : (uint8_t)255; fa.ds[q] = fold ? dsq[q] : (uint8_t)255; }
        fa.tblDelta1 = zk->d_tblDelta1; fa.tblAlpha1 = zk->d_tblAlpha1; fa.tblBeta1 = zk->d_tblBeta1; fa.tblDelta2 = zk->d_tblDelta2;
        fa.alpha1 = zk->alpha1; fa.beta2 = zk->beta2; fa.rs = CS.d_rs + 64 * (size_t)p0; fa.out = CS.d_proofs + 256 * (size_t)p0; fa.scratch = LN.d_fin;
        fa.per = tree ? 5 : 3; fa.fb4 = zk->d_fb4; fa.fb4g2 = zk->d_fb4g2; fa.out_xyzz = CS.d_xyzz + 512 * (size_t)p0;
        const bool g2_early = !sw::on<sw::ZKC_G2_LATE>();
        const bool g2_hold_env = sw::on<sw::ZKC_G2_ACC_HOLD>(), g2_early_env = sw::on<sw::ZKC_G2_ACC_EARLY>();
        const bool g2_acc_with_sort = g2_hold_env || ((nb < 32 || !one_lane) && !g2_early_env);
        if (g2_early) {
            if ((rc = msm_pass_g2(zk, LN.w2, j2, slot, false, st2, g2_acc_with_sort ? LN.ev_ntt : nullptr))) return rc;
            if (tree && (rc = finalize_tree_g2_launch(ctx, st2, fa, nb))) return rc;
            ZKC_HIP_CHECK(ctx, hipEventRecord(LN.ev_msm2, st2));
        }
        tr[3] = now_ms();
        ZKC_HIP_CHECK(ctx, hipStreamWaitEvent(st, LN.ev_red, 0));
        const bool red_split = sw::on<sw::ZKC_REDUCE_STREAM>() && !zk->serial_streams && nb >= 32;
        if ((rc = msm_pass_g1(zk, LN.w1, j1, slot, false, st, LN.ev_sorted, LN.ev_acc, (red_split && LS.red) ? LS.red : nullptr, LN.ev_red))) return rc;
        tr[4] = now_ms();
        if (!g2_early) {
            ZKC_HIP_CHECK(ctx, hipStreamWaitEvent(st2, LN.ev_sorted, 0));
            if ((rc = msm_pass_g2(zk, LN.w2, j2, slot, false, st2))) return rc;
            if (tree && (rc = finalize_tree_g2_launch(ctx, st2, fa, nb))) return rc;
            ZKC_HIP_CHECK(ctx, hipEventRecord(LN.ev_msm2, st2));
        }
        if (want_publics)
            ZKC_HIP_CHECK(ctx, hipMemcpy2DAsync(h_pub + 32ull * np * p0, 32ull * np, w0 + 8, 32ull * nv, 32ull * np, nb, hipMemcpyDeviceToHost, st));
        ZKC_HIP_CHECK(ctx, hipEventRecord(LN.ev_msm, st));
        if (mv_prefetch && p0 + per_pass < B) {
            const int p1 = p0 + per_pass, nb1 = std::min(per_pass, B - p1);
            ZKC_HIP_CHECK(ctx, hipStreamWaitEvent(fin, sw::on<sw::ZKC_MV_PREFETCH_AT_NTT>() ? LN.ev_ntt : LN.ev_sorted, 0));
            ZKC_HIP_CHECK(ctx, hipStreamWaitEvent(fin, CS.ev_chunk[pass + 1], 0));
            if ((rc = h_matvec_dev(zk, LN, (const uint32_t*)d_wtns + (size_t)p1 * nv * 8, nb1, fin))) return rc;
            ZKC_HIP_CHECK(ctx, hipEventRecord(LN.ev_mv, fin));
        }
        hipStream_t bl = ((tree || lane0 >= 0) && npasses == 1) ? st : fin;
        if (bl == fin) { ZKC_HIP_CHECK(ctx, hipStreamWaitEvent(fin, LN.ev_msm, 0)); ZKC_HIP_CHECK(ctx, hipStreamWaitEvent(fin, LN.ev_red, 0)); }
        else { if (LN.npass >= 2) ZKC_HIP_CHECK(ctx, hipStreamWaitEvent(st, LN.ev_fin[slot ^ 1], 0)); if (red_split) ZKC_HIP_CHECK(ctx, hipStreamWaitEvent(st, LN.ev_red, 0)); }
        if (!tree) ZKC_HIP_CHECK(ctx, hipStreamWaitEvent(bl, LN.ev_msm2, 0));
        if ((rc = finalize_launch(ctx, bl, fa, nb))) return rc;
        if (tree) ZKC_HIP_CHECK(ctx, hipStreamWaitEvent(bl, LN.ev_msm2, 0));
        if (tree) { ZKC_HIP_CHECK(ctx, hipMemcpyAsync(CS.h_xyzz + 512ull * p0, CS.d_xyzz + 512 * (size_t)p0, 512ull * nb, hipMemcpyDeviceToHost, bl)); for (int q = 0; q < nb; q++) CS.as_xyzz[p0 + q] = 1; }
        else ZKC_HIP_CHECK(ctx, hipMemcpyAsync(CS.h_out + 256ull * p0, CS.d_proofs + 256 * (size_t)p0, 256ull * nb, hipMemcpyDeviceToHost, bl));
        ZKC_HIP_CHECK(ctx, hipEventRecord(LN.ev_fin[slot], bl));
        if (bl == st) done_on_st_lane = li;
        tr[5] = now_ms();
        if (trace_host) fprintf(stderr, "[zkc host] pass %2d: start %8.2f | chunk wait %6.2f | h_evals %6.2f | g2 pass %6.2f | g1 pass %6.2f | blinding %6.2f ms\n", pass, tr[0] - t_begin,
                                tr[1] - tr[0], tr[2] - tr[1], tr[3] - tr[2], tr[4] - tr[3], tr[5] - tr[4]);
    }
    for (int l = 0; l < zk->nlanes; l++) if (CS.lanes_used >> l & 1) { const LaneSt ls = lane_st(zk, ctx->lanes[l]); ZKC_HIP_CHECK(ctx, hipEventRecord(CS.ev_done[l], done_on_st_lane == l ? ls.st : ls.fin)); }
    CS.B = B; CS.pending = true;
    return ZKC_OK;
}
static std::atomic<unsigned long long> g_early_retries{0};
extern "C" unsigned long long zkc_debug_early_retries(void) { return g_early_retries.load(); }
int zkc::prove_batch_finish(zkc_zkey* zk, int cs, uint8_t* proofs, uint8_t* publics) {
    if (!zk || !proofs || cs < 0 || cs >= CALL_SLOTS) return zkc_fail(zk ? zk->ctx : nullptr, ZKC_ERR_BAD_ARG, "prove_batch_finish: bad argument");
    zkc_zkey::CallSlot& CS = zk->call[cs];
    if (!CS.pending) return zkc_fail(zk->ctx, ZKC_ERR_BAD_ARG, "prove_batch_finish: no call in flight on this slot");
    hipError_t e = hipSuccess;
    for (int l = 0; l < zk->nlanes && e == hipSuccess; l++) if (CS.lanes_used >> l & 1) e = zkc_wait_event(CS.ev_done[l], CS.B <= 2 ? 6000u : 0u);
    CS.pending = false;
    if (e != hipSuccess) { ZKC_LOCK(zk->ctx); return zkc_fail(zk->ctx, ZKC_ERR_HIP, std::string("prove_batch_finish: ") + hipGetErrorString(e)); }
    if (CS.early_n) {
        const WitnessLayout L = WitnessLayout::make(zk->nLevels);
        for (int q = 0; q < CS.early_n; q++) {
            if ((int32_t)CS.h_early[q] != ZKC_W_OK) continue;
            for (int t = 0; t < 2; t++) {
                const uint32_t* f = CS.h_early + CS.early_cap + ((size_t)q * 2 + t) * L.n;
                int D = 0; for (int g = 0; g < L.n - 1; g++) if (f[g]) D = g + 1;
                if (f[L.n - 1] || D > (int)CS.early_depth[2 * q + t]) {
                    if (!CS.arg_inputs) { g_early_retries++; int rc = prove_batch_begin(zk, cs, CS.arg_wtns, CS.arg_nw, CS.B, CS.h_rs_copy.data(), CS.arg_publics, nullptr, nullptr, CS.arg_lane0, nullptr, nullptr, true); if (rc) return rc; return prove_batch_finish(zk, cs, proofs, publics); }
                    ZKC_LOCK(zk->ctx); return zkc_fail(zk->ctx, ZKC_ERR_GENERIC, "prove_batch_finish: the witness does not fold at the depth its inputs gave (internal error)");
                }
            }
        }
    }
    memcpy(proofs, CS.h_out, 256ull * CS.B);
    for (int q = 0; q < CS.B; q++) if (CS.as_xyzz[q]) {
        const uint8_t* x = CS.h_xyzz + 512 * (size_t)q; uint8_t* o = proofs + 256 * (size_t)q;
        G1XYZZ a, c; G2XYZZ b; memcpy(&a, x, 128); memcpy(&b, x + 128, 256); memcpy(&c, x + 384, 128);
        g1_to_std(o, xyzz_to_affine_gcd(a)); g2_to_std(o + 64, xyzz_to_affine_gcd(b)); g1_to_std(o + 192, xyzz_to_affine_gcd(c));
    }
    if (publics) memcpy(publics, CS.h_out + 256ull * CS.cap, 32ull * zk->nPub * CS.B);
    return ZKC_OK;
}
static int prove_batch_impl(zkc_zkey* zk, const void* d_wtns, uint32_t nWitness, int B, const uint8_t* rs, uint8_t* proofs, uint8_t* publics,
                            const void* d_inputs, int32_t* d_status) {
    if (!zk || !proofs) return zkc_fail(zk ? zk->ctx : nullptr, ZKC_ERR_BAD_ARG, "zkc_prove_batch_dev: bad argument");
    ZKC_LOCK(zk->ctx);
    for (int c = 1; c < CALL_SLOTS; c++) if (zk->call[c].pending) return zkc_fail(zk->ctx, ZKC_ERR_BAD_ARG, "zkc_prove_batch_dev: the key has a split call in flight (proving service)");
    int rc = prove_batch_begin(zk, 0, d_wtns, nWitness, B, rs, publics != nullptr, d_inputs, d_status);
    if (rc) return rc;
    return prove_batch_finish(zk, 0, proofs, publics);
}

extern "C" int zkc_batch_begin(zkc_zkey* zk, int slot, const void* d_inputs, int B, void* d_wtns, int32_t* d_status, const uint8_t* rs) {
    if (!zk || !d_wtns || (d_inputs && !d_status) || slot < 0 || slot >= CALL_SLOTS) return zkc_fail(zk ? zk->ctx : nullptr, ZKC_ERR_BAD_ARG, "zkc_batch_begin: bad argument");
    if (d_inputs && zk->nLevels < 0) return zkc_fail(zk->ctx, ZKC_ERR_BAD_ARG, "zkc_batch_begin: the key is not a ZkFranchiseProofCircuit(nLevels) key; compute the witness elsewhere and pass d_inputs = NULL");
    return prove_batch_begin(zk, slot, d_wtns, zk->nVars, B, rs, true, d_inputs, d_status);
}
extern "C" int zkc_batch_finish(zkc_zkey* zk, int slot, uint8_t* proofs, uint8_t* publics) { return prove_batch_finish(zk, slot, proofs, publics); }

extern "C" int zkc_prove_batch_dev(zkc_zkey* zk, const void* d_wtns, uint32_t nWitness, int B, const uint8_t* rs, uint8_t* proofs, uint8_t* publics) {
    return prove_batch_impl(zk, d_wtns, nWitness, B, rs, proofs, publics, nullptr, nullptr);
}
extern "C" int zkc_fullprove_batch_dev(zkc_zkey* zk, const void* d_inputs, int B, void* d_wtns, int32_t* d_status, const uint8_t* rs, uint8_t* proofs, uint8_t* publics) {
    if (!zk || !d_inputs || !d_status) return zkc_fail(zk ? zk->ctx : nullptr, ZKC_ERR_BAD_ARG, "zkc_fullprove_batch_dev: bad argument");
    if (zk->nLevels < 0) return zkc_fail(zk->ctx, ZKC_ERR_BAD_ARG, "zkc_fullprove_batch_dev: the key is not a ZkFranchiseProofCircuit(nLevels) key; compute the witness elsewhere and call zkc_prove_batch_dev");
    return prove_batch_impl(zk, d_wtns, zk->nVars, B, rs, proofs, publics, d_inputs, d_status);
}

extern "C" int zkc_prove_dev(zkc_zkey* zk, const void* d_wtns, uint32_t nWitness, const uint8_t r32[32], const uint8_t s32[32],
                             uint8_t proof[256], uint8_t* public_out) {
    if (!r32 || !s32) return zkc_fail(zk ? zk->ctx : nullptr, ZKC_ERR_BAD_ARG, "zkc_prove_dev: bad argument");
    uint8_t rs[64]; memcpy(rs, r32, 32); memcpy(rs + 32, s32, 32);
    return zkc_prove_batch_dev(zk, d_wtns, nWitness, 1, rs, proof, public_out);
}

extern "C" int zkc_prove(zkc_zkey* zk, const void* wtns, uint32_t nWitness, const uint8_t r32[32], const uint8_t s32[32],
                         uint8_t proof[256], uint8_t* public_out) {
    if (!zk || !wtns) return zkc_fail(zk ? zk->ctx : nullptr, ZKC_ERR_BAD_ARG, "zkc_prove: bad argument");
    zkc_ctx* ctx = zk->ctx;
    ZKC_LOCK(ctx);
    if (nWitness != zk->nVars) return zkc_fail(ctx, ZKC_ERR_INVALID_WITNESS_LENGTH, "Invalid witness length. Circuit: " + std::to_string(zk->nVars) + ", witness: " + std::to_string(nWitness));
    if (const long long bad = first_unreduced_wire(wtns, nWitness); bad >= 0) return zkc_fail(ctx, ZKC_ERR_FORMAT, unreduced_wire_msg(bad));
    ZKC_HIP_CHECK(ctx, hipSetDevice(ctx->device));
    int rc = zkc_ensure(ctx, &ctx->d_scratch_out, &ctx->scratch_out_sz, 32ull * nWitness); if (rc) return rc;
    ZKC_HIP_CHECK(ctx, hipMemcpyAsync(ctx->d_scratch_out, wtns, 32ull * nWitness, hipMemcpyHostToDevice, ctx->stream));
    return zkc_prove_dev(zk, ctx->d_scratch_out, nWitness, r32, s32, proof, public_out);
}
```

### zk-franchise-proof-circuit_amd/csrc/zkc_prover.h

```cpp
#pragma once
#include <cstring>
#include "zkc_internal.h"
#include "zkc_curve.h"

namespace zkc {
constexpr int MSM_C_BIG = 17, MSM_C_SMALL = 12;
constexpr int MSM_C_G2_LONE = 8;
inline long long first_unreduced_wire(const void* w, size_t count) {
    const uint8_t* p = (const uint8_t*)w;
    for (size_t i = 0; i < count; i++) {
        uint32_t t[8]; memcpy(t, p + 32 * i, 32);
        if (t[7] >= FrParams::p[7] && !fp_std_lt_p<FrParams>(t)) return (long long)i;
    }
    return -1;
}
inline std::string unreduced_wire_msg(long long wire) { return "Witness value at wire " + std::to_string(wire) + " is not below the field order r"; }
inline int msm_c_for(size_t W) { return W < 12000 ? 12 : W < 22000 ? 13 : W < 90000 ? 15 : W < 180000 ? 16 : 17; }
constexpr int msm_nw(int c) { return (254 + c) / c; }
constexpr int msm_half(int c) { return 1 << (c - 1); }
constexpr int MSM_VW_MIN = 64, MSM_MAX_VW_PER_JOB = 64;
constexpr int MSM_MAX_VW_G1 = 256;
constexpr int MSM_SEG_MIN = 16;
#ifndef ZKC_MSM_SEG
#define ZKC_MSM_SEG 128
#endif
constexpr int MSM_SEG = ZKC_MSM_SEG;
constexpr int MSM_MERGE_T = 8;
constexpr int MSM_MAX_HEAVY = 1 << 20;
constexpr int MSM_MAX_JOBS = 512;
constexpr int MAX_LANES = 4, CALL_SLOTS = 4;
static_assert(sw::rows[sw::ZKC_C_SECTIONS].hi == MSM_C_BIG && sw::rows[sw::ZKC_C_H].hi == MSM_C_BIG && sw::rows[sw::ZKC_C_DEEP].hi == MSM_C_BIG, "zkc_switches.h: MSM_C_BIG");
static_assert(sw::rows[sw::ZKC_INFLIGHT].hi == MSM_MAX_JOBS / 4 && sw::rows[sw::ZKC_SERVICE_PASS].hi == MSM_MAX_JOBS / 4, "zkc_switches.h: MSM_MAX_JOBS / 4");
static_assert(sw::rows[sw::ZKC_LANES].hi == MAX_LANES && sw::rows[sw::ZKC_SERVICE_WORKERS].hi == MAX_LANES, "zkc_switches.h: MAX_LANES");

struct MsmJob {
    const uint32_t* scalars;
    const uint32_t* vmap;
    uint32_t count;
    uint32_t tbl_off;
    uint32_t tbl_count;
    int32_t pt_shift;
    uint32_t c, nw, vw;
    uint32_t ent_off, win_off;
    uint32_t bucket0, bin0, hbits, lbits, tile0, cnt0;
};
struct FinalizeArgs {
    const G1XYZZ* r1; const G2XYZZ* r2;
    const G1XYZZ *foldA, *foldB1, *foldC; const G2XYZZ* foldB2; int fold_n;
    uint8_t dc[MSM_MAX_JOBS / 4], ds[MSM_MAX_JOBS / 4];
    const G1Affine *tblDelta1, *tblAlpha1, *tblBeta1; const G2Affine* tblDelta2;
    G1Affine alpha1; G2Affine beta2;
    const uint8_t* rs; uint8_t* out;
    void* scratch;
    int per; const G1XYZZ* fb4; const G2XYZZ* fb4g2;
    uint8_t* out_xyzz;
};
constexpr int FB4_WIN = 64, FB4_ROW = 15;
struct BlindArgs { const uint32_t* w[2]; const uint32_t* mapA[2]; const uint32_t* mapB[2]; uint32_t nA[2], nB[2]; uint32_t* out[2]; const uint8_t* rs; uint32_t nv; };
constexpr int MSM_TILE = 256, MSM_TILE_SCALARS = 1024;
constexpr uint32_t MSM_MAX_HBITS = 10;
struct MsmJobList {
    MsmJob job[MSM_MAX_JOBS]; int njobs; uint32_t total_buckets, total_entries, total_windows, total_bins, total_tiles, total_tilecnt;
    uint32_t hs, hb, nbig;
    uint32_t hbits_big, hbits_small;
    uint32_t vw_big = 1024;
    uint32_t vw_small = 256;
    void add(const uint32_t* scalars, const uint32_t* vmap, uint32_t count, uint32_t tbl_off, uint32_t tbl_count, int32_t pt_shift, int c) {
        MsmJob& j = job[njobs++];
        uint32_t vw = c >= 16 ? vw_big : vw_small;
        if (vw > (uint32_t)msm_half(c)) vw = (uint32_t)msm_half(c);
        while ((uint32_t)msm_half(c) / vw > max_vw_per_job) vw <<= 1;
        j = MsmJob{scalars, vmap, count, tbl_off, tbl_count, pt_shift, (uint32_t)c, (uint32_t)msm_nw(c), vw, total_entries, total_windows, 0, 0, 0, 0, 0, 0};
        total_entries += count * (uint32_t)msm_nw(c); total_windows += (uint32_t)msm_half(c) / vw;
    }
    uint32_t max_vw_per_job = 256;
    void clear(uint32_t vw_small_jobs = 256, uint32_t vw_big_jobs = 1024, uint32_t max_per_job = 256) { vw_small = vw_small_jobs; vw_big = vw_big_jobs; max_vw_per_job = max_per_job; njobs = 0; total_buckets = total_entries = total_windows = total_bins = total_tiles = total_tilecnt = 0; hs = hb = nbig = 0; }
    bool finish() {
        hs = 0xffffffffu; hb = 0;
        for (int j = 0; j < njobs; j++) { const uint32_t h = 1u << (job[j].c - 1); hs = h < hs ? h : hs; hb = h > hb ? h : hb; }
        nbig = 0; total_buckets = total_bins = total_tiles = total_tilecnt = 0; hbits_big = hbits_small = 0;
        for (int j = 0; j < njobs; j++) {
            MsmJob& q = job[j]; const uint32_t h = 1u << (q.c - 1);
            if (h != hs && h != hb) return false;
            if (h == hb) { if ((uint32_t)j != nbig) return false; nbig++; }
            uint32_t hbits = q.c - 1 < 8 ? q.c - 1 : 8, lbits = q.c - 1 - hbits;
            const uint64_t rows = (uint64_t)q.nw * q.tbl_count;
            while (lbits > 8 || (lbits > 0 && rows >= (1ull << (31 - lbits)))) { lbits--; hbits++; }
            if (hbits > MSM_MAX_HBITS || rows >= (1ull << (31 - lbits))) return false;
            q.hbits = hbits; q.lbits = lbits;
            { uint32_t& cls = h == hb ? hbits_big : hbits_small; cls = (cls == 0 || cls == hbits) ? hbits : 0xffu; }
            q.bucket0 = total_buckets; total_buckets += h;
            q.bin0 = total_bins; total_bins += 1u << hbits;
            const uint32_t nt = (q.count + MSM_TILE_SCALARS - 1) / MSM_TILE_SCALARS;
            q.tile0 = total_tiles; total_tiles += nt; q.cnt0 = total_tilecnt; total_tilecnt += nt << hbits;
        }
        return true;
    }
    ZKC_HD uint32_t id_of(uint32_t d, uint32_t j) const { return job[j].bucket0 + d; }
    ZKC_HD uint32_t job_of_bin(uint32_t bin) const {
        if (hbits_big != 0xffu && hbits_small != 0xffu) {
            const uint32_t lim = nbig << hbits_big;
            return bin < lim ? bin >> hbits_big : nbig + ((bin - lim) >> hbits_small);
        }
        uint32_t lo = 0, hi = (uint32_t)njobs - 1;
        while (lo < hi) { const uint32_t mid = (lo + hi + 1) >> 1; if (job[mid].bin0 <= bin) lo = mid; else hi = mid - 1; }
        return lo;
    }
    ZKC_HD void decode(uint32_t id, uint32_t& d, uint32_t& j) const {
        const uint32_t lim = hb * nbig;
        if (id < lim) { j = id / hb; d = id - j * hb; }
        else { const uint32_t t = id - lim, q = t / hs; j = nbig + q; d = t - q * hs; }
    }
};
struct MsmWindow { uint32_t bucket0, out, per; };

struct MsmWork {
    uint32_t *vals = nullptr, *vals2 = nullptr;
    uint32_t *hist = nullptr, *bin_start = nullptr;
    uint32_t *tilecnt = nullptr; size_t max_tilecnt = 0;
    uint32_t *off = nullptr, *bcnt = nullptr;
    uint32_t *segcnt = nullptr, *segoff = nullptr, *seg2bucket = nullptr, *heavy = nullptr;
    uint32_t *seglen = nullptr, *perm = nullptr;
    uint32_t *scan_blk = nullptr, *lencnt = nullptr; size_t max_lencnt = 0;
    void *partial = nullptr;
    void *wres = nullptr;
    void *results = nullptr;
    void *h_results = nullptr;
    MsmJobList* d_jobs = nullptr;
    MsmWindow* d_windows = nullptr; size_t max_buckets = 0, max_bins = 0, max_windows = 0;
    uint16_t* d_tilejob = nullptr; uint16_t* h_tilejob[2] = {nullptr, nullptr}; size_t max_tiles = 0;
    MsmJobList* h_jobs[2] = {nullptr, nullptr}; MsmWindow* h_windows[2] = {nullptr, nullptr}; hipEvent_t h_ev[2] = {nullptr, nullptr}; int h_next = 0;
    size_t max_entries = 0, max_segments = 0; int max_jobs = 0; size_t xyzz_size = 0;
};
}

struct zkc_lane {
    hipStream_t st = nullptr, st2 = nullptr, fin = nullptr;
    hipStream_t red = nullptr; hipEvent_t ev_red = nullptr;
    zkc::Fr *d_abc = nullptr, *d_t = nullptr; uint32_t* d_p = nullptr;
    void* d_fin = nullptr;
    uint32_t* d_bs = nullptr;
    zkc::MsmWork w1, w2;
    size_t cap_abc = 0, cap_p = 0, cap_fin = 0, cap_bs = 0, bytes = 0; bool made = false;
    hipEvent_t ev_msm = nullptr, ev_msm2 = nullptr, ev_sorted = nullptr, ev_ntt = nullptr, ev_mv = nullptr, ev_acc = nullptr, ev_fin[2] = {nullptr, nullptr}; int npass = 0;
};

struct zkc_zkey {
    zkc_ctx* ctx = nullptr;
    uint32_t nVars = 0, nPub = 0, n = 0, logn = 0, nCoeffs = 0;
    int nLevels = -1;
    zkc::G1Affine alpha1, beta1, delta1;
    zkc::G2Affine beta2, gamma2, delta2;
    std::vector<zkc::G1Affine> ic;
    uint32_t *d_perm = nullptr, *d_rowlen = nullptr, *d_jdptr = nullptr, *d_col = nullptr; zkc::Fr* d_val = nullptr; uint32_t nlong = 0;
    uint32_t n_unit_coeffs = 0;
    zkc::Fr *d_tw_fwd = nullptr, *d_tw_inv = nullptr, *d_coset = nullptr;
    zkc::Fr *d_coset_br = nullptr;
    uint32_t *d_tw_fwd29 = nullptr, *d_tw_inv29 = nullptr;
    zkc::G1Affine* d_g1 = nullptr; zkc::G2Affine* d_g2 = nullptr;
    uint32_t* d_g2_29 = nullptr;
    uint32_t* d_g2_29_lone = nullptr;
    uint32_t offA = 0, offB1 = 0, offC = 0, offH = 0;
    int c_deep = 0; uint32_t offA_deep = 0, offB1_deep = 0, offC_deep = 0; uint32_t* d_g2_29_deep = nullptr;
    int c_h = zkc::MSM_C_BIG;
    int c_sec = zkc::MSM_C_SMALL;
    int max_inflight = 0;
    uint8_t sha256[32] = {0};
    size_t bytes_tables = 0;
    uint8_t fingerprint[32] = {0};
    int nlanes = 1; bool serial_streams = false;
    zkc::G1Affine *d_tblDelta1 = nullptr, *d_tblAlpha1 = nullptr, *d_tblBeta1 = nullptr; zkc::G2Affine* d_tblDelta2 = nullptr;
    uint32_t *d_depths = nullptr, *h_depths = nullptr; size_t depths_cap = 0;
    zkc::G1XYZZ* d_fb4 = nullptr; zkc::G2XYZZ* d_fb4g2 = nullptr; int fb4_bases = 0;
    struct CallSlot {
        uint8_t *d_rs = nullptr, *d_proofs = nullptr; size_t cap = 0;
        uint8_t* h_out = nullptr;
        uint8_t* h_rs = nullptr;
        uint8_t *d_xyzz = nullptr, *h_xyzz = nullptr; std::vector<uint8_t> as_xyzz;
        hipEvent_t ev_done[zkc::MAX_LANES] = {};
        std::vector<hipEvent_t> ev_chunk;
        uint32_t lanes_used = 0;
        int B = 0; bool pending = false;
        uint32_t *d_flags = nullptr, *h_flags = nullptr; size_t flags_cap = 0;
        int32_t* d_status3 = nullptr; size_t status3_cap = 0;
        int early_n = 0; std::vector<uint8_t> early_depth; uint32_t* h_early = nullptr; size_t early_cap = 0;
        const void* arg_wtns = nullptr; uint32_t arg_nw = 0; bool arg_publics = false, arg_inputs = false; int arg_lane0 = -1; hipEvent_t arg_wait = nullptr; std::vector<uint8_t> h_rs_copy;
    } call[zkc::CALL_SLOTS];
    struct Fold {
        std::vector<zkc::G1XYZZ> baseA, baseB1, baseC; std::vector<zkc::G2XYZZ> baseB2;
        std::vector<zkc::G1XYZZ> sufA[2], sufB1[2], sufC[2]; std::vector<zkc::G2XYZZ> sufB2[2];
        struct VMap { uint32_t* d = nullptr; uint32_t offA = 0, nA = 0, offB = 0, nB = 0, offC = 0, nC = 0; };
        std::map<std::pair<int, int>, VMap> vmaps;
        std::vector<uint8_t> infA, infB, infC;
        zkc::G1XYZZ *d_foldA = nullptr, *d_foldB1 = nullptr, *d_foldC = nullptr; zkc::G2XYZZ* d_foldB2 = nullptr;
        bool ready = false;
    } fold;
};

namespace zkc {
int ntt_run(zkc_ctx* ctx, hipStream_t st, const Fr* src, Fr* dst, const uint32_t* tw29, const Fr* scale, int logn, int nvec);
int ntt_make_tw29(zkc_ctx* ctx, const Fr* d_tw, uint32_t count, uint32_t** out);
int ntt_pair_run(zkc_ctx* ctx, hipStream_t st, Fr* data, const uint32_t* tw_inv29, const uint32_t* tw_fwd29, const Fr* scale_br, int logn, int nvec);
int ntt_bitrev_table(zkc_ctx* ctx, const Fr* d_src, Fr** out, int logn);
int msm_work_alloc(zkc_ctx* ctx, MsmWork& w, size_t max_entries, size_t max_buckets, int max_jobs, bool g2);
void msm_work_free(MsmWork& w);
int msm_pass_g1(zkc_zkey* zk, MsmWork& w, const MsmJobList& jl, int slot, bool to_host, hipStream_t st, hipEvent_t ev_sorted = nullptr, hipEvent_t ev_acc = nullptr,
                hipStream_t st_red = nullptr, hipEvent_t ev_red = nullptr);
int msm_pass_g2(zkc_zkey* zk, MsmWork& w, const MsmJobList& jl, int slot, bool to_host, hipStream_t st, hipEvent_t wait_before_acc = nullptr);
int msm_bucket_entries(zkc_ctx* ctx, MsmWork& w, const MsmJobList& jl, hipStream_t st, unsigned long long* d_entry_counter = nullptr);
int msm_build_segments(zkc_ctx* ctx, MsmWork& w, const MsmJobList& jl, uint32_t seg, size_t seg_bound, hipStream_t st);
int finalize_launch(zkc_ctx* ctx, hipStream_t st, const FinalizeArgs& a, int nproofs);
int finalize_tree_g2_launch(zkc_ctx* ctx, hipStream_t st, const FinalizeArgs& a, int nproofs);
int fb4_build(zkc_ctx* ctx, hipStream_t st, const G1XYZZ* d_bases, int nbases, G1XYZZ* d_out, const G2XYZZ& delta2, const G2XYZZ& beta2, const G2XYZZ& beta2_base, G2XYZZ* d_out2);
int blind_scalars_launch(zkc_ctx* ctx, hipStream_t st, const BlindArgs& a, int nproofs);
int prove_batch_begin(zkc_zkey* zk, int cs, const void* d_wtns, uint32_t nWitness, int B, const uint8_t* rs, bool want_publics, const void* d_inputs, int32_t* d_status,
                      int lane0 = -1, hipEvent_t wait_first = nullptr, const uint8_t* host_depths = nullptr, bool no_early = false);
int prove_batch_finish(zkc_zkey* zk, int cs, uint8_t* proofs, uint8_t* publics);
int prove_reserve(zkc_zkey* zk, int inflight);
int zkey_load_opts(zkc_ctx* ctx, const void* zkey_bytes, size_t len, int nlanes, int max_inflight, zkc_zkey** out);
size_t zkey_device_bytes(const zkc_zkey* zk, size_t* tables, size_t* work);
size_t finalize_scratch_bytes(int nproofs);
int msm_precompute_g1(zkc_ctx* ctx, uint32_t count, G1Affine* d_table, int c);
int msm_precompute_g2(zkc_ctx* ctx, uint32_t count, G2Affine* d_table, int c);
int msm_g2_table29(zkc_ctx* ctx, const G2Affine* d_table, uint32_t* d_out, size_t count);
int fold_group_sums_g1(zkc_ctx* ctx, const G1Affine* tbl, const uint32_t* d_scalars, const uint32_t* d_wires, uint32_t nw, int32_t pt_shift,
                       const uint32_t* d_gstart, uint32_t ngroups, G1XYZZ* h_out);
int fold_group_sums_g1_ws(zkc_ctx* ctx, const G1Affine* tbl, const uint32_t* d_scalars, const uint32_t* d_wires, uint32_t nw, const uint32_t* d_gstart, uint32_t ngroups,
                          G1XYZZ* d_tmp , G1XYZZ* d_out , G1XYZZ* h_out);
int fold_group_sums_g2(zkc_ctx* ctx, const G2Affine* tbl, const uint32_t* d_scalars, const uint32_t* d_wires, uint32_t nw, int32_t pt_shift,
                       const uint32_t* d_gstart, uint32_t ngroups, G2XYZZ* h_out);
}
```

### zk-franchise-proof-circuit_amd/csrc/zkc_switches.h

```cpp
#pragma once
#include <climits>
#include <cstdlib>
#include <optional>

namespace zkc { namespace sw {

enum Kind { SET, OFF_IF_ZERO, ON_IF_ONE, NUMBER, NUMBER_LONG, NUMBER_U64, TEXT };
enum When { PROCESS, LIVE };
constexpr long long ANY = LLONG_MIN;

#define ZKC_SWITCHES(X)                                                                                                                                                   \
                                                                                                                                            \
    X(ZKC_DEVICE,               TEXT,        ANY, ANY,   LIVE,    "service creation: the GPUs of the default proving service: \"2\", \"0,1,2,3\", \"all\"; unset: every visible device") \
    X(ZKC_INFLIGHT,             NUMBER,      1,   128,   LIVE,    "key load: proofs per pipeline pass (census key 64, any other 96, fewer for a large circuit); at most MSM_MAX_JOBS / 4") \
    X(ZKC_LANES,                NUMBER,      1,   4,     LIVE,    "key load: pipeline lanes the passes of a batch call rotate over (census key MAX_LANES = 4, any other 1)")      \
    X(ZKC_DEEP_TABLES,          NUMBER,      ANY, ANY,   LIVE,    "key load: 0 leaves out the second section tables that passes of deep voters take, 2 builds them for a census key of any size (default 1)") \
    X(ZKC_G2_LONE_TABLE,        OFF_IF_ZERO, ANY, ANY,   LIVE,    "key load: =0 skips the 8-bit-window G2 table of the lone-proof path")                                          \
    X(ZKC_BLIND_TREE,           OFF_IF_ZERO, ANY, ANY,   LIVE,    "key load: =0 gives a key whose passes of one or two proofs take the general blinding kernels")                 \
    X(ZKC_SERVICE_WORKERS,      NUMBER,      1,   4,     LIVE,    "service creation: workers (= lanes of a service key) per GPU (4); at most MAX_LANES")                          \
    X(ZKC_SERVICE_PASS,         NUMBER,      1,   128,   LIVE,    "service creation: proofs per pass of a service key (64); at most MSM_MAX_JOBS / 4")                            \
    X(ZKC_SERVICE_KEYS,         NUMBER,      1,   64,    LIVE,    "service creation: keys kept resident per GPU (4)")                                                             \
    X(ZKC_SERVICE_MAX_BATCH,    NUMBER,      1,   4096,  LIVE,    "service creation: requests one worker takes per call (256)")                                                   \
    X(ZKC_SERVICE_MIN_BATCH,    NUMBER,      1,   ANY,   LIVE,    "service creation: requests a collecting worker waits for before it goes (16)")                                 \
    X(ZKC_SERVICE_SPILL,        NUMBER,      1,   ANY,   LIVE,    "service creation: queue length at which a cold GPU is brought up (32)")                                        \
    X(ZKC_SERVICE_BUSY_WAIT_US, NUMBER,      0,   ANY,   LIVE,    "service creation: microseconds a collecting worker waits for more requests (300)")                             \
    X(ZKC_SERVICE_RESERVE,      OFF_IF_ZERO, ANY, ANY,   PROCESS, "=0: a service key load does not reserve a full pass of work space on every lane; the lanes grow on demand")    \
    X(ZKC_DEVICE_BLOCKING_SYNC, ON_IF_ONE,   ANY, ANY,   LIVE,    "context creation: =1 asks HIP for blocking waits on the device (hipDeviceScheduleBlockingSync)")               \
    X(ZKC_SPIN_WAIT,            SET,         ANY, ANY,   PROCESS, "set (any value, 0 included): host waits use hipEventSynchronize instead of polling with short sleeps")         \
    X(ZKC_VERIFY_BATCH_GPU,     NUMBER,      ANY, ANY,   LIVE,    "per verify call: 0 keeps the Miller loops of zkc_verify_batch on the host, positive forces the GPU, negative or unset: GPU from 128 proofs") \
    X(ZKC_NO_SHA_NI,            SET,         ANY, ANY,   PROCESS, "set (any value, 0 included): portable SHA-256 instead of the CPU's SHA extensions")                            \
                                                                                                                              \
    X(ZKC_NO_FOLD,              SET,         ANY, ANY,   LIVE,    "key load: set (any value, 0 included): no constant folding of the voter-independent witness part for this key") \
    X(ZKC_SERIAL_STREAMS,       SET,         ANY, ANY,   LIVE,    "key load: set (any value, 0 included): every stage of this key's passes on the context's one stream (isolated stage times)") \
    X(ZKC_C_SECTIONS,           NUMBER,      8,   17,    LIVE,    "key load: window bits of the witness sections (census key 12, any other by its wire count); at most MSM_C_BIG") \
    X(ZKC_C_H,                  NUMBER,      8,   17,    LIVE,    "key load: window bits of the H section (census key 17, any other by its domain size); at most MSM_C_BIG")      \
    X(ZKC_C_DEEP,               NUMBER,      13,  17,    LIVE,    "key load: window bits of the second section tables (by the wire count); at most MSM_C_BIG")                    \
    X(ZKC_DEEP_WIRES,           NUMBER_LONG, ANY, ANY,   PROCESS, "live wires per section and proof from which a pass takes the second section tables (16000)")                   \
    X(ZKC_WITNESS_GROUP,        NUMBER,      1,   ANY,   PROCESS, "passes whose voters share one witness launch in a batch call (8)")                                             \
    X(ZKC_VW_BIG,               NUMBER,      ANY, ANY,   PROCESS, "buckets per reduction wave of the H jobs in passes of more than four proofs (0 or unset: 4096, 1024 below 32 proofs)") \
    X(ZKC_VW_SMALL,             NUMBER,      ANY, ANY,   PROCESS, "the same for the witness sections (0 or unset: 2048, 256 below 32 proofs)")                                    \
    X(ZKC_VW_G2,                NUMBER,      ANY, ANY,   PROCESS, "the same for the G2 jobs of passes of 32 proofs and more (0 or unset: as the witness sections)")              \
    X(ZKC_G2_ACC,               NUMBER,      ANY, ANY,   PROCESS, "form of the G2 accumulation: 0 registers hold the next row, 1 / 2 LDS-DMA prefetch at one / two waves per SIMD (0)") \
    X(ZKC_G2_BUCKET_WAVE,       OFF_IF_ZERO, ANY, ANY,   PROCESS, "=0: small G2 passes keep lane-per-segment accumulation instead of half a wave per bucket")                     \
    X(ZKC_G2_LATE,              SET,         ANY, ANY,   PROCESS, "set (any value, 0 included): the G2 MSM of a pass starts after the G1 sort instead of with the pass")          \
    X(ZKC_G2_ACC_HOLD,          SET,         ANY, ANY,   PROCESS, "set (any value, 0 included): the G2 accumulation always waits for the G1 stream to leave its transforms")      \
    X(ZKC_G2_ACC_EARLY,         SET,         ANY, ANY,   PROCESS, "set (any value, 0 included): the G2 accumulation never waits for them (ZKC_G2_ACC_HOLD wins)")                 \
    X(ZKC_ACC_CHAIN,            OFF_IF_ZERO, ANY, ANY,   PROCESS, "=0: the G1 accumulations of a context's lanes are not chained one behind the other")                           \
    X(ZKC_REDUCE_STREAM,        ON_IF_ONE,   ANY, ANY,   PROCESS, "=1: the bucket reduction of a full pass runs on a stream of its own (the lanes then get that stream)")         \
    X(ZKC_MATVEC_UNITS,         OFF_IF_ZERO, ANY, ANY,   PROCESS, "=0: buildABC multiplies by its +-1 coefficients instead of adding the wire")                                   \
    X(ZKC_MATVEC_INLINE,        SET,         ANY, ANY,   PROCESS, "set (any value, 0 included): buildABC of the next pass is not prefetched on the blinding stream")              \
    X(ZKC_MV_PREFETCH_AT_NTT,   ON_IF_ONE,   ANY, ANY,   PROCESS, "=1: that prefetch starts beside the pass' bucketing instead of beside its accumulation")                       \
    X(ZKC_EARLY_LAYOUT,         OFF_IF_ZERO, ANY, ANY,   PROCESS, "=0: one-pass calls of more than two voters wait for their fold flags instead of reading the depths off the inputs") \
    X(ZKC_NOFOLD_LISTS,         OFF_IF_ZERO, ANY, ANY,   PROCESS, "=0: unfolded passes keep the wires whose bases are at infinity")                                               \
    X(ZKC_NTT_SEPARATE,         SET,         ANY, ANY,   PROCESS, "set (any value, 0 included): two self-contained transforms instead of the fused pair")                         \
    X(ZKC_NTT_RADIX,            NUMBER,      ANY, ANY,   PROCESS, "below 4: the head transform kernel runs one stage at a time instead of two (4)")                               \
    X(ZKC_FINALIZE_WAVES,       SET,         ANY, ANY,   PROCESS, "set (any value, 0 included): the one-wave-per-task blinding kernel for every pass")                            \
    X(ZKC_VERIFY_CHUNK,         NUMBER,      2,   16384, LIVE,    "per verify call: pairs per round of Miller-loop kernels (16384)")                                              \
    X(ZKC_SMT_WAVE_MAX,         NUMBER_U64,  ANY, ANY,   LIVE,    "per check call: census proof batches up to this size take the wave-per-proof form (64; 0: never)")            \
    X(ZKC_TRACE_HOST,           SET,         ANY, ANY,   PROCESS, "set (any value, 0 included): prints where the enqueueing thread spends its time, per pass")                    \
    X(ZKC_VERIFY_TRACE,         SET,         ANY, ANY,   LIVE,    "per verify call: set (any value, 0 included): prints the stage times of zkc_verify_batch")                     \
    X(ZKC_DEBUG_SYNC,           SET,         ANY, ANY,   PROCESS, "set (any value, 0 included): synchronises after and logs every MSM launch; read when the library is loaded")   \
                                                                                                                                                \
    X(ZKC_TEST_FAIL_ALLOC,      NUMBER,      ANY, ANY,   LIVE,    "lane growth: the work-space allocation for this many proofs in flight or more fails")                          \
    X(ZKC_TEST_FAIL_KEY_LOADS,  NUMBER,      ANY, ANY,   LIVE,    "service key load: fails as out of memory while the device holds this many keys or more")

enum Id {
#define X(name, kind, lo, hi, when, doc) name,
    ZKC_SWITCHES(X)
#undef X
    COUNT
};
struct Row { const char* name; Kind kind; long long lo, hi; When when; const char* doc; };
inline constexpr Row rows[COUNT] = {
#define X(name, kind, lo, hi, when, doc) {#name, kind, lo, (hi) == ANY ? LLONG_MAX : (hi), when, doc},
    ZKC_SWITCHES(X)
#undef X
};

struct Raw { bool set; long long num; const char* str; };
inline Raw read(const Row& r) {
    const char* e = getenv(r.name);
    if (!e) return {false, 0, nullptr};
    const long long v = r.kind == NUMBER_U64 ? (long long)strtoull(e, nullptr, 10) : r.kind == NUMBER_LONG ? (long long)atol(e) : (long long)atoi(e);
    return {true, v < r.lo ? r.lo : v > r.hi ? r.hi : v, e};
}
template <Id I> inline Raw get() {
    if constexpr (rows[I].when == PROCESS) { static const Raw cached = read(rows[I]); return cached; }
    else return read(rows[I]);
}
constexpr bool is_number(Kind k) { return k == NUMBER || k == NUMBER_LONG || k == NUMBER_U64; }

template <Id I> inline bool on() {
    static_assert(rows[I].kind == SET || rows[I].kind == OFF_IF_ZERO || rows[I].kind == ON_IF_ONE, "not an on/off switch");
    const Raw r = get<I>();
    return rows[I].kind == SET ? r.set : rows[I].kind == OFF_IF_ZERO ? !(r.set && r.num == 0) : (r.set && r.num == 1);
}
template <Id I> inline std::optional<long long> given() {
    static_assert(is_number(rows[I].kind), "not a number");
    const Raw r = get<I>();
    return r.set ? std::optional<long long>(r.num) : std::nullopt;
}
template <Id I> inline long long value(long long dflt) { return given<I>().value_or(dflt); }
template <Id I> inline const char* text() {
    static_assert(rows[I].kind == TEXT && rows[I].when == LIVE, "not a live text switch");
    return get<I>().str;
}

}}
```

Measured before the change: 3148.

## Merge C-section MSM into H job tail and fuse A*B product into NTT head

The C-section G1 MSM is folded into the H MSM as a tail of the same job, sharing the H job's window size and precomputed table. This removes a separate job and its own bucket reduction, and the finalize kernels are updated for one fewer per-proof result. The pointwise A*B product is also moved into the first NTT head pass, which forms C on the fly from A and B. That drops a separate kernel and a read/write pass over memory. The cost is a larger H table and extra branches in the scalar gather, and the merge is disabled when 31-bit indices would overflow.

```diff
diff --git a/zk-franchise-proof-circuit_amd/csrc/zkc_finalize.hip b/zk-franchise-proof-circuit_amd/csrc/zkc_finalize.hip
--- a/zk-franchise-proof-circuit_amd/csrc/zkc_finalize.hip
+++ b/zk-franchise-proof-circuit_amd/csrc/zkc_finalize.hip
@@ -70,7 +70,7 @@
     const int nq = gridDim.x;
     uint8_t* out = a.out + 256 * (size_t)q;
     if (wave == 0 && lane < 2) {
-        const G1XYZZ P = lane == 0 ? xyzz_add(a.r1[nq + 3 * q + 0], fold_const(a.foldA, a, q)) : xyzz_add(a.r1[nq + 3 * q + 1], fold_const(a.foldB1, a, q));
+        const G1XYZZ P = lane == 0 ? xyzz_add(a.r1[nq + (3 - a.merged) * q + 0], fold_const(a.foldA, a, q)) : xyzz_add(a.r1[nq + (3 - a.merged) * q + 1], fold_const(a.foldB1, a, q));
         sh[lane] = var_mul29(P, lane == 0 ? s : r, tab[lane]);
     } else if (wave == 1 && lane < 5) {
         uint32_t k[8];
@@ -83,7 +83,7 @@
         const G1XYZZ v = fb_mul<Fq>(tb, k);
         sh[2 + lane] = v;
         if (lane == 0) {
-            const G1XYZZ A = xyzz_add(a.r1[nq + 3 * q + 0], fold_const(a.foldA, a, q));
+            const G1XYZZ A = xyzz_add(a.r1[nq + (3 - a.merged) * q + 0], fold_const(a.foldA, a, q));
             G1Affine p = xyzz_to_affine(xyzz_add(xyzz_add_affine(A, a.alpha1), v));
             store_fq_std(out, p.x); store_fq_std(out + 32, p.y);
         }
@@ -94,7 +94,7 @@
     }
     __syncthreads();
     if (threadIdx.x == 0) {
-        G1XYZZ c = xyzz_add(xyzz_add(a.r1[nq + 3 * q + 2], fold_const(a.foldC, a, q)), a.r1[q]);
+        G1XYZZ c = xyzz_add(xyzz_add(a.merged ? G1XYZZ::inf() : a.r1[nq + 3 * q + 2], fold_const(a.foldC, a, q)), a.r1[q]);
         c = xyzz_add(c, sh[0]); c = xyzz_add(c, sh[5]); c = xyzz_add(c, sh[1]); c = xyzz_add(c, sh[6]); c = xyzz_add(c, sh[4]);
         G1Affine p = xyzz_to_affine(c);
         store_fq_std(out + 192, p.x); store_fq_std(out + 224, p.y);
@@ -115,7 +115,7 @@
     G2XYZZ* res2 = reinterpret_cast<G2XYZZ*>(res1 + 7 * (size_t)nq);
     Acc29* tabs = reinterpret_cast<Acc29*>(res2 + nq);
     if (task < 2) {
-        const G1XYZZ P = task == 0 ? xyzz_add(a.r1[nq + 3 * q + 0], fold_const(a.foldA, a, q)) : xyzz_add(a.r1[nq + 3 * q + 1], fold_const(a.foldB1, a, q));
+        const G1XYZZ P = task == 0 ? xyzz_add(a.r1[nq + (3 - a.merged) * q + 0], fold_const(a.foldA, a, q)) : xyzz_add(a.r1[nq + (3 - a.merged) * q + 1], fold_const(a.foldB1, a, q));
         res1[(size_t)task * nq + q] = var_mul29_g(P, task == 0 ? s : r, tabs + ((size_t)task * nq + q) * 16);
     } else if (task == 3) {
         return;
@@ -140,11 +140,11 @@
     const G2XYZZ* res2 = reinterpret_cast<const G2XYZZ*>(res1 + 7 * (size_t)nq);
     uint8_t* out = a.out + 256 * (size_t)q;
     if (role == 0) {
-        const G1XYZZ A = xyzz_add(a.r1[nq + 3 * q + 0], fold_const(a.foldA, a, q));
+        const G1XYZZ A = xyzz_add(a.r1[nq + (3 - a.merged) * q + 0], fold_const(a.foldA, a, q));
         G1Affine p = xyzz_to_affine(xyzz_add(xyzz_add_affine(A, a.alpha1), res1[2 * (size_t)nq + q]));
         store_fq_std(out, p.x); store_fq_std(out + 32, p.y);
     } else if (role == 1) {
-        G1XYZZ c = xyzz_add(xyzz_add(a.r1[nq + 3 * q + 2], fold_const(a.foldC, a, q)), a.r1[q]);
+        G1XYZZ c = xyzz_add(xyzz_add(a.merged ? G1XYZZ::inf() : a.r1[nq + 3 * q + 2], fold_const(a.foldC, a, q)), a.r1[q]);
         c = xyzz_add(c, res1[0 * (size_t)nq + q]); c = xyzz_add(c, res1[5 * (size_t)nq + q]); c = xyzz_add(c, res1[1 * (size_t)nq + q]);
         c = xyzz_add(c, res1[6 * (size_t)nq + q]); c = xyzz_add(c, res1[4 * (size_t)nq + q]);
         G1Affine p = xyzz_to_affine(c);
@@ -229,7 +229,8 @@
     const int task = blockIdx.x, q = blockIdx.y, nq = gridDim.y, lane = threadIdx.x;
     uint32_t r[8], s[8]; load_rs(a, q, r, s);
     const bool folded = a.dc[q] != 255; const int n = a.fold_n, dc = a.dc[q], ds = a.ds[q];
-    const G1XYZZ* res = a.r1 + nq + 5 * (size_t)q;
+    const G1XYZZ* res = a.r1 + nq + (5 - a.merged) * (size_t)q;
+    const int bsum = a.merged ? 2 : 3;
     Acc29* outv = reinterpret_cast<Acc29*>(a.scratch) + (size_t)q * 10 + task;
     Acc29 v; f29_pt_set_inf(v);
     if (task < 8) {
@@ -260,13 +261,13 @@
         else if (lane == 3 && folded) v = load_pt29(a.foldA[1 + n + ds]);
         v = wave_sum_g1(v, 2);
     } else {
-        if (lane == 0) v = load_pt29(res[2]);
+        if (lane == 0) { if (!a.merged) v = load_pt29(res[2]); }
         else if (lane == 1 && folded) v = load_pt29(a.foldC[0]);
         else if (lane == 2 && folded) v = load_pt29(a.foldC[1 + dc]);
         else if (lane == 3 && folded) v = load_pt29(a.foldC[1 + n + ds]);
         else if (lane == 4) v = load_pt29(a.r1[q]);
-        else if (lane == 5) v = load_pt29(res[3]);
-        else if (lane == 6) v = load_pt29(res[4]);
+        else if (lane == 5) v = load_pt29(res[bsum]);
+        else if (lane == 6) v = load_pt29(res[bsum + 1]);
         v = wave_sum_g1(v, 4);
     }
     if (lane == 0) *outv = v;
diff --git a/zk-franchise-proof-circuit_amd/csrc/zkc_msm_sort.hip b/zk-franchise-proof-circuit_amd/csrc/zkc_msm_sort.hip
--- a/zk-franchise-proof-circuit_amd/csrc/zkc_msm_sort.hip
+++ b/zk-franchise-proof-circuit_amd/csrc/zkc_msm_sort.hip
@@ -12,10 +12,12 @@
 #pragma unroll
         for (int q = 0; q < 8; q++) t.s[k][q] = 0;
         if (t.live[k]) {
-            const uint32_t wire = job.vmap ? job.vmap[i] : i;
-            const uint4* sp = reinterpret_cast<const uint4*>(job.scalars + 8 * (size_t)wire); const uint4 a = sp[0], b = sp[1];
+            const uint32_t n1 = job.count - job.count2; const bool tail = i >= n1;
+            const uint32_t* const vm = tail ? job.vmap2 : job.vmap; const uint32_t i1 = tail ? i - n1 : i;
+            const uint32_t wire = vm ? vm[i1] : i1;
+            const uint4* sp = reinterpret_cast<const uint4*>((tail ? job.scalars2 : job.scalars) + 8 * (size_t)wire); const uint4 a = sp[0], b = sp[1];
             t.s[k][0] = a.x; t.s[k][1] = a.y; t.s[k][2] = a.z; t.s[k][3] = a.w; t.s[k][4] = b.x; t.s[k][5] = b.y; t.s[k][6] = b.z; t.s[k][7] = b.w;
-            t.pt[k] = (uint32_t)((int32_t)wire - job.pt_shift);
+            t.pt[k] = (uint32_t)((int32_t)wire - (tail ? job.pt_shift2 : job.pt_shift));
         }
     }
 }
diff --git a/zk-franchise-proof-circuit_amd/csrc/zkc_ntt.hip b/zk-franchise-proof-circuit_amd/csrc/zkc_ntt.hip
--- a/zk-franchise-proof-circuit_amd/csrc/zkc_ntt.hip
+++ b/zk-franchise-proof-circuit_amd/csrc/zkc_ntt.hip
@@ -245,10 +245,12 @@
         __syncthreads();
     }
 }
+constexpr int HEAD_PLAIN = 0, HEAD_C = 1, HEAD_AB = 2;
 template <int RADIX>
-__device__ __forceinline__ void ntt_nr_head_body(const Fr* src_all, Fr* dst_all, const uint32_t* __restrict__ tw29, int logn, int q0, int b) {
-    const Fr* src = src_all + ((size_t)blockIdx.y << logn);
-    Fr* dst = dst_all + ((size_t)blockIdx.y << logn);
+__device__ __forceinline__ void ntt_nr_head_body(const Fr* src_all, Fr* dst_all, const uint32_t* __restrict__ tw29, int logn, int q0, int b, int mode) {
+    const size_t vec = mode == HEAD_C ? 3 * (size_t)blockIdx.y + 2 : mode == HEAD_AB ? 3 * (size_t)(blockIdx.y >> 1) + (blockIdx.y & 1) : (size_t)blockIdx.y;
+    const Fr* src = src_all + (vec << logn);
+    Fr* dst = dst_all + (vec << logn);
     extern __shared__ uint32_t tile[];
     const int mid_n = 1 << b, sh = logn - q0 - b, lo_t = NTT_TILE >> b, elems = mid_n * lo_t;
     const int bpp = (1 << sh) / lo_t;
@@ -256,8 +258,13 @@
     const size_t base = ((size_t)prefix << (logn - q0)) + (size_t)(blockIdx.x % bpp) * lo_t;
     for (int e = threadIdx.x; e < elems; e += blockDim.x) {
         const int mid = e / lo_t, l = e - mid * lo_t;
-        const Fr x = ld_fr(src + (base + ((size_t)mid << sh) + l));
-        uint32_t t[9]; f29_from_fp_shl5(t, x.v);
+        const size_t gi = base + ((size_t)mid << sh) + l;
+        uint32_t t[9];
+        if (mode == HEAD_C) {
+            const Fr av = ld_fr(src - ((size_t)2 << logn) + gi), bv = ld_fr(src - ((size_t)1 << logn) + gi);
+            uint32_t a29[9], b29[9]; f29_from_fp_shl5(a29, av.v); f29_from_fp_shl5(b29, bv.v);
+            f29_mul<FrParams>(t, a29, b29);
+        } else { const Fr x = ld_fr(src + gi); f29_from_fp_shl5(t, x.v); }
 #pragma unroll
         for (int k = 0; k < 9; k++) tile[9 * e + k] = t[k];
     }
@@ -273,9 +280,9 @@
     }
 }
 extern "C" __global__ void __launch_bounds__(256)
-zkc_ntt_nr_head(const Fr* src_all, Fr* dst_all, const uint32_t* __restrict__ tw29, int logn, int q0, int b) { ntt_nr_head_body<1>(src_all, dst_all, tw29, logn, q0, b); }
-extern "C" __global__ void __launch_bounds__(256)
-zkc_ntt_nr_head_r4(const Fr* src_all, Fr* dst_all, const uint32_t* __restrict__ tw29, int logn, int q0, int b) { ntt_nr_head_body<4>(src_all, dst_all, tw29, logn, q0, b); }
+zkc_ntt_nr_head(const Fr* src_all, Fr* dst_all, const uint32_t* __restrict__ tw29, int logn, int q0, int b, int mode) { ntt_nr_head_body<1>(src_all, dst_all, tw29, logn, q0, b, mode); }
+extern "C" __global__ void __launch_bounds__(256)
+zkc_ntt_nr_head_r4(const Fr* src_all, Fr* dst_all, const uint32_t* __restrict__ tw29, int logn, int q0, int b, int mode) { ntt_nr_head_body<4>(src_all, dst_all, tw29, logn, q0, b, mode); }
 extern "C" __global__ void __launch_bounds__(256)
 zkc_ntt_mid(Fr* __restrict__ data_all, const uint32_t* __restrict__ tw_inv29, const uint32_t* __restrict__ tw_fwd29, const Fr* __restrict__ scale_br, int logn) {
     Fr* __restrict__ data = data_all + ((size_t)blockIdx.y << logn);
@@ -339,15 +346,19 @@
     ZKC_HIP_CHECK(ctx, hipGetLastError());
     return ZKC_OK;
 }
-int ntt_pair_run(zkc_ctx* ctx, hipStream_t st, Fr* data, const uint32_t* tw_inv29, const uint32_t* tw_fwd29, const Fr* scale_br, int logn, int nvec) {
+int ntt_pair_run(zkc_ctx* ctx, hipStream_t st, Fr* data, const uint32_t* tw_inv29, const uint32_t* tw_fwd29, const Fr* scale_br, int logn, int nvec, bool form_c) {
     if (logn < 12 || logn > 27) return zkc_fail(ctx, ZKC_ERR_BAD_ARG, "ntt_pair_run: 12 <= logn <= 27");
+    if (form_c && nvec % 3) return zkc_fail(ctx, ZKC_ERR_BAD_ARG, "ntt_pair_run: the fused product needs whole [A | B | C] triples");
     const int bh = logn - 9;
     const int b1 = bh <= 9 ? bh : (bh + 1) / 2, b2 = bh - b1;
     const unsigned blocks = (1u << logn) / NTT_TILE;
     const int radix = (int)sw::value<sw::ZKC_NTT_RADIX>(4);
     auto head = radix >= 4 ? zkc_ntt_nr_head_r4 : zkc_ntt_nr_head;
-    hipLaunchKernelGGL(head, dim3(blocks, nvec), dim3(256), (size_t)NTT_TILE * 36, st, (const Fr*)data, data, tw_inv29, logn, 0, b1);
-    if (b2) hipLaunchKernelGGL(head, dim3(blocks, nvec), dim3(256), (size_t)NTT_TILE * 36, st, (const Fr*)data, data, tw_inv29, logn, b1, b2);
+    if (form_c) {
+        hipLaunchKernelGGL(head, dim3(blocks, nvec / 3), dim3(256), (size_t)NTT_TILE * 36, st, (const Fr*)data, data, tw_inv29, logn, 0, b1, HEAD_C);
+        hipLaunchKernelGGL(head, dim3(blocks, 2 * (nvec / 3)), dim3(256), (size_t)NTT_TILE * 36, st, (const Fr*)data, data, tw_inv29, logn, 0, b1, HEAD_AB);
+    } else hipLaunchKernelGGL(head, dim3(blocks, nvec), dim3(256), (size_t)NTT_TILE * 36, st, (const Fr*)data, data, tw_inv29, logn, 0, b1, HEAD_PLAIN);
+    if (b2) hipLaunchKernelGGL(head, dim3(blocks, nvec), dim3(256), (size_t)NTT_TILE * 36, st, (const Fr*)data, data, tw_inv29, logn, b1, b2, HEAD_PLAIN);
     hipLaunchKernelGGL(zkc_ntt_mid, dim3(blocks, nvec), dim3(256), (size_t)NTT_TILE * 36, st, data, tw_inv29, tw_fwd29, scale_br, logn);
     hipLaunchKernelGGL(zkc_ntt_pass, dim3(blocks, nvec), dim3(256), (size_t)NTT_TILE * 36, st, (const Fr*)data, data, tw_fwd29, (const Fr*)nullptr, logn, 9, b1, 0);
     if (b2) hipLaunchKernelGGL(zkc_ntt_pass, dim3(blocks, nvec), dim3(256), (size_t)NTT_TILE * 36, st, (const Fr*)data, data, tw_fwd29, (const Fr*)nullptr, logn, 9 + b1, b2, 0);
diff --git a/zk-franchise-proof-circuit_amd/csrc/zkc_prove.hip b/zk-franchise-proof-circuit_amd/csrc/zkc_prove.hip
--- a/zk-franchise-proof-circuit_amd/csrc/zkc_prove.hip
+++ b/zk-franchise-proof-circuit_amd/csrc/zkc_prove.hip
@@ -10,13 +10,14 @@
 
 using namespace zkc;
 
-static void matvec_launch(zkc_zkey* zk, zkc_lane& L, const uint32_t* d_wtns0, int nb, hipStream_t mv) {
+static bool pair_path(const zkc_zkey* zk) { return !sw::on<sw::ZKC_NTT_SEPARATE>() && zk->logn >= 12 && zk->logn <= 27; }
+static void matvec_launch(zkc_zkey* zk, zkc_lane& L, const uint32_t* d_wtns0, int nb, hipStream_t mv, bool with_c) {
     const uint32_t n = zk->n, nv = zk->nVars;
     const bool units = zk->n_unit_coeffs > 0 && nv <= 3 * (size_t)n && sw::on<sw::ZKC_MATVEC_UNITS>();
     if (units) hipLaunchKernelGGL(zkc_wtns_mont, dim3((nv + 255) / 256, nb), dim3(256), 0, mv, (const Fr*)d_wtns0, (size_t)nv, L.d_t, 3 * (size_t)n, nv);
     hipLaunchKernelGGL(zkc_matvec_jds, dim3((2 * n + 63 * zk->nlong + 255) / 256, nb), dim3(256), 0, mv, zk->d_perm, zk->d_rowlen, zk->d_jdptr, zk->d_col, zk->d_val,
                        (const Fr*)d_wtns0, (size_t)nv, L.d_abc, (int)n, zk->nlong, units ? (const Fr*)L.d_t : (const Fr*)nullptr, 3 * (size_t)n);
-    hipLaunchKernelGGL(zkc_pointwise_mul, dim3((n + 255) / 256, nb), dim3(256), 0, mv, L.d_abc, (int)n);
+    if (with_c) hipLaunchKernelGGL(zkc_pointwise_mul, dim3((n + 255) / 256, nb), dim3(256), 0, mv, L.d_abc, (int)n);
 }
 static constexpr uint32_t MATVEC_LONG = 16;
 
@@ -263,23 +264,29 @@
       zk->c_deep = (zk->nLevels >= 0 && (nv >= (1u << 16) || dt == 2) && zk->c_sec < cd && dt != 0) ? cd : 0; }
     zk->c_h = std::max(zk->c_h, std::max(zk->c_sec, zk->c_deep));
     const int NWB = msm_nw(zk->c_h);
-    zk->offA = 0; zk->offB1 = NWS * nv; zk->offC = 2 * NWS * nv; zk->offH = 2 * NWS * nv + NWS * nc;
+    zk->merge_ch = sw::on<sw::ZKC_MERGE_CH>() && nc > 0;
+    { const int min_lbits = std::max(0, zk->c_h - 1 - (int)MSM_MAX_HBITS); if ((uint64_t)NWB * ((uint64_t)n + nc) >= (1ull << (31 - min_lbits))) zk->merge_ch = false; }
+    const bool mch = zk->merge_ch;
+    zk->hTbl = mch ? n + nc : n;
+    zk->offA = 0; zk->offB1 = NWS * nv;
+    if (mch) { zk->offH = 2 * NWS * nv; zk->offC = zk->offH + n; } else { zk->offC = 2 * NWS * nv; zk->offH = 2 * NWS * nv + NWS * nc; }
     const int NWD = zk->c_deep ? msm_nw(zk->c_deep) : 0;
-    zk->offA_deep = zk->offH + NWB * n; zk->offB1_deep = zk->offA_deep + NWD * nv; zk->offC_deep = zk->offB1_deep + NWD * nv;
-    const size_t g1_points = (size_t)NWS * (2 * (size_t)nv + nc) + (size_t)NWB * n + (size_t)NWD * (2 * (size_t)nv + nc);
+    zk->offA_deep = zk->offH + NWB * zk->hTbl; zk->offB1_deep = zk->offA_deep + NWD * nv; zk->offC_deep = zk->offB1_deep + NWD * nv;
+    const size_t g1_points = (size_t)NWS * (2 * (size_t)nv + (mch ? 0 : nc)) + (size_t)NWB * zk->hTbl + (size_t)NWD * (2 * (size_t)nv + (mch ? 0 : nc));
     if (g1_points >= (1ull << 31)) return bail(zkc_fail(ctx, ZKC_ERR_FORMAT, "zkey too large for 31-bit point indices"));
+    if (mch && (uint64_t)NWB * zk->hTbl >= (1ull << 31)) return bail(zkc_fail(ctx, ZKC_ERR_BAD_ARG, "zkc_zkey_load: the merged H + C table needs more than 31 bits of row index"));
     if ((rc = dmalloc(ctx, &zk->d_g1, g1_points)) || (rc = dmalloc(ctx, &zk->d_g2, (size_t)NWS * nv))) return bail(rc);
     ZKC_UP(zk->d_g1 + zk->offA, sec[5], 64ull * nv); ZKC_UP(zk->d_g1 + zk->offB1, sec[6], 64ull * nv);
     ZKC_UP(zk->d_g1 + zk->offC, sec[8], 64ull * nc); ZKC_UP(zk->d_g1 + zk->offH, sec[9], 64ull * n);
     ZKC_UP(zk->d_g2, sec[7], 128ull * nv);
     if ((rc = msm_precompute_g1(ctx, nv, zk->d_g1 + zk->offA, zk->c_sec)) || (rc = msm_precompute_g1(ctx, nv, zk->d_g1 + zk->offB1, zk->c_sec)) ||
-        (rc = msm_precompute_g1(ctx, nc, zk->d_g1 + zk->offC, zk->c_sec)) || (rc = msm_precompute_g1(ctx, n, zk->d_g1 + zk->offH, zk->c_h)) ||
+        (!mch && (rc = msm_precompute_g1(ctx, nc, zk->d_g1 + zk->offC, zk->c_sec))) || (rc = msm_precompute_g1(ctx, zk->hTbl, zk->d_g1 + zk->offH, zk->c_h)) ||
         (rc = msm_precompute_g2(ctx, nv, zk->d_g2, zk->c_sec))) return bail(rc);
     if ((rc = dmalloc(ctx, &zk->d_g2_29, 60 * (size_t)NWS * nv)) || (rc = msm_g2_table29(ctx, zk->d_g2, zk->d_g2_29, (size_t)NWS * nv))) return bail(rc);
     if (zk->c_deep) {
-        ZKC_UP(zk->d_g1 + zk->offA_deep, sec[5], 64ull * nv); ZKC_UP(zk->d_g1 + zk->offB1_deep, sec[6], 64ull * nv); ZKC_UP(zk->d_g1 + zk->offC_deep, sec[8], 64ull * nc);
+        ZKC_UP(zk->d_g1 + zk->offA_deep, sec[5], 64ull * nv); ZKC_UP(zk->d_g1 + zk->offB1_deep, sec[6], 64ull * nv); if (!mch) ZKC_UP(zk->d_g1 + zk->offC_deep, sec[8], 64ull * nc);
         if ((rc = msm_precompute_g1(ctx, nv, zk->d_g1 + zk->offA_deep, zk->c_deep)) || (rc = msm_precompute_g1(ctx, nv, zk->d_g1 + zk->offB1_deep, zk->c_deep)) ||
-            (rc = msm_precompute_g1(ctx, nc, zk->d_g1 + zk->offC_deep, zk->c_deep))) return bail(rc);
+            (!mch && (rc = msm_precompute_g1(ctx, nc, zk->d_g1 + zk->offC_deep, zk->c_deep)))) return bail(rc);
         G2Affine* tmp = nullptr;
         if ((rc = dmalloc(ctx, &tmp, (size_t)NWD * nv))) return bail(rc);
         hipError_t e2 = hipMemcpyAsync(tmp, zk->d_g2, 128ull * nv, hipMemcpyDeviceToDevice, ctx->stream);
@@ -465,7 +472,7 @@
 static int h_matvec_dev(zkc_zkey* zk, zkc_lane& L, const uint32_t* d_wtns0, int nb, hipStream_t mv) {
     zkc_ctx* ctx = zk->ctx; const uint32_t n = zk->n, nv = zk->nVars;
     zkc_prof_scope _ps(ctx, ZKC_PROF_MATVEC, (uint64_t)nb * ((uint64_t)zk->nCoeffs * 68 + 3ull * n * 32), mv);
-    matvec_launch(zk, L, d_wtns0, nb, mv);
+    matvec_launch(zk, L, d_wtns0, nb, mv, !pair_path(zk));
     ZKC_HIP_CHECK(ctx, hipGetLastError());
     return ZKC_OK;
 }
@@ -474,8 +481,8 @@
     if (with_matvec) { int rc0 = h_matvec_dev(zk, L, d_wtns0, nb, st); if (rc0) return rc0; }
     zkc_prof_scope _pn(ctx, ZKC_PROF_NTT, (uint64_t)nb * (6ull * 2 * n * 32 + 4ull * n * 32), st);
     int rc;
-    if (!sw::on<sw::ZKC_NTT_SEPARATE>() && zk->logn >= 12 && zk->logn <= 27) {
-        if ((rc = ntt_pair_run(ctx, st, L.d_abc, zk->d_tw_inv29, zk->d_tw_fwd29, zk->d_coset_br, (int)zk->logn, 3 * nb))) return rc;
+    if (pair_path(zk)) {
+        if ((rc = ntt_pair_run(ctx, st, L.d_abc, zk->d_tw_inv29, zk->d_tw_fwd29, zk->d_coset_br, (int)zk->logn, 3 * nb, true))) return rc;
     } else {
         if ((rc = ntt_run(ctx, st, L.d_abc, L.d_t, zk->d_tw_inv29, zk->d_coset, (int)zk->logn, 3 * nb))) return rc;
         if ((rc = ntt_run(ctx, st, L.d_t, L.d_abc, zk->d_tw_fwd29, nullptr, (int)zk->logn, 3 * nb))) return rc;
@@ -493,7 +500,7 @@
     { int rc0 = lanes_ensure(zk, 1, 0, 1); if (rc0) return rc0; }
     zkc_lane& L0 = ctx->lanes[0]; const hipStream_t st0 = lane_st(zk, L0).st;
     if (stage == 0) {
-        matvec_launch(zk, L0, (const uint32_t*)d_wtns, 1, st0);
+        matvec_launch(zk, L0, (const uint32_t*)d_wtns, 1, st0, true);
         ZKC_HIP_CHECK(ctx, hipGetLastError());
         ZKC_HIP_CHECK(ctx, hipMemcpyAsync(host_out, L0.d_abc, 96ull * n, hipMemcpyDeviceToHost, st0));
     } else {
@@ -515,7 +522,8 @@
     if (count != full) return zkc_fail(ctx, ZKC_ERR_BAD_ARG, "zkc_msm_debug: count must equal the section size");
     static thread_local MsmJobList jl; jl.clear(256, 1024, which == 2 ? (uint32_t)MSM_MAX_VW_PER_JOB : (uint32_t)MSM_MAX_VW_G1);
     const uint32_t offs[5] = {zk->offA, zk->offB1, 0, zk->offC, zk->offH};
-    jl.add((const uint32_t*)d_scalars, nullptr, count, offs[which], full, 0, which == 4 ? zk->c_h : zk->c_sec);
+    if (which == 4 || (which == 3 && zk->merge_ch)) jl.add((const uint32_t*)d_scalars, nullptr, count, zk->offH, zk->hTbl, which == 3 ? -(int32_t)zk->n : 0, zk->c_h);
+    else jl.add((const uint32_t*)d_scalars, nullptr, count, offs[which], full, 0, zk->c_sec);
     int rc = which == 2 ? msm_pass_g2(zk, L0.w2, jl, 0, true, st_l0) : msm_pass_g1(zk, L0.w1, jl, 0, true, st_l0); if (rc) return rc;
     ZKC_HIP_CHECK(ctx, hipStreamSynchronize(st_l0));
     if (which == 2) g2_to_std((uint8_t*)host_out, xyzz_to_affine(*(G2XYZZ*)L0.w2.h_results));
@@ -670,7 +678,12 @@
         const int c2 = (nb <= 2 && zk->d_g2_29_lone && lone_entries <= LN.w2.max_entries) ? MSM_C_G2_LONE : cw;
         const uint32_t vwg2_env = (uint32_t)sw::value<sw::ZKC_VW_G2>(0);
         j1.clear(vws, vwb, MSM_MAX_VW_G1); j2.clear(c2 == MSM_C_G2_LONE ? 128u : (vwg2_env && nb >= 32) ? vwg2_env : vws, 1024, MSM_MAX_VW_PER_JOB);
-        for (int q = 0; q < nb; q++) j1.add(LN.d_p + 8 * (size_t)n * q, nullptr, n, zk->offH, n, 0, zk->c_h);
+        const bool mch = zk->merge_ch;
+        for (int q = 0; q < nb; q++) {
+            j1.add(LN.d_p + 8 * (size_t)n * q, nullptr, n, zk->offH, zk->hTbl, 0, zk->c_h);
+            if (mch && listed) j1.add_tail(w0 + (size_t)q * nv * 8, vms[q].d + vms[q].offC, vms[q].nC, (int32_t)np + 1 - (int32_t)n);
+            else if (mch) j1.add_tail(w0 + (size_t)q * nv * 8 + 8ull * (np + 1), nullptr, nc, -(int32_t)n);
+        }
         size_t tree_entries = 0; for (int q = 0; q < nb; q++) tree_entries += (size_t)msm_nw(zk->c_h) * n + (size_t)msm_nw(zk->c_sec) * (listed ? 2 * (size_t)vms[q].nA + 2 * (size_t)vms[q].nB + vms[q].nC : 4 * (size_t)nv + nc);
         const bool tree = zk->d_fb4 != nullptr && nb <= 2 && 6 * nb <= LN.w1.max_jobs && tree_entries <= LN.w1.max_entries && (size_t)nb * (5 * msm_half(zk->c_sec) + msm_half(zk->c_h)) <= LN.w1.max_buckets;
         BlindArgs ba{}; ba.rs = CS.d_rs + 64 * (size_t)p0; ba.nv = nv;
@@ -682,14 +695,14 @@
                 const zkc_zkey::Fold::VMap& vm = vms[q];
                 j1.add(w, vm.d + vm.offA, vm.nA, oA, nv, 0, cw);
                 j1.add(w, vm.d + vm.offB, vm.nB, oB1, nv, 0, cw);
-                j1.add(w, vm.d + vm.offC, vm.nC, oC, nc, (int32_t)np + 1, cw);
+                if (!mch) j1.add(w, vm.d + vm.offC, vm.nC, oC, nc, (int32_t)np + 1, cw);
                 if (tree) { j1.add(bs, vm.d + vm.offA, vm.nA, oA, nv, 0, cw); j1.add(bs + 8ull * nv, vm.d + vm.offB, vm.nB, oB1, nv, 0, cw); }
                 j2.add(w, vm.d + vm.offB, vm.nB, 0, nv, 0, c2);
                 if (tree) { ba.mapA[q] = vm.d + vm.offA; ba.nA[q] = vm.nA; ba.mapB[q] = vm.d + vm.offB; ba.nB[q] = vm.nB; }
             } else {
                 j1.add(w, nullptr, nv, oA, nv, 0, cw);
                 j1.add(w, nullptr, nv, oB1, nv, 0, cw);
-                j1.add(w + 8ull * (np + 1), nullptr, nc, oC, nc, 0, cw);
+                if (!mch) j1.add(w + 8ull * (np + 1), nullptr, nc, oC, nc, 0, cw);
                 if (tree) { j1.add(bs, nullptr, nv, oA, nv, 0, cw); j1.add(bs + 8ull * nv, nullptr, nv, oB1, nv, 0, cw); }
                 j2.add(w, nullptr, nv, 0, nv, 0, c2);
                 if (tree) { ba.mapA[q] = ba.mapB[q] = nullptr; ba.nA[q] = ba.nB[q] = nv; }
@@ -702,7 +715,7 @@
         for (int q = 0; q < nb; q++) { fa.dc[q] = fold ? dcq[q] : (uint8_t)255; fa.ds[q] = fold ? dsq[q] : (uint8_t)255; }
         fa.tblDelta1 = zk->d_tblDelta1; fa.tblAlpha1 = zk->d_tblAlpha1; fa.tblBeta1 = zk->d_tblBeta1; fa.tblDelta2 = zk->d_tblDelta2;
         fa.alpha1 = zk->alpha1; fa.beta2 = zk->beta2; fa.rs = CS.d_rs + 64 * (size_t)p0; fa.out = CS.d_proofs + 256 * (size_t)p0; fa.scratch = LN.d_fin;
-        fa.per = tree ? 5 : 3; fa.fb4 = zk->d_fb4; fa.fb4g2 = zk->d_fb4g2; fa.out_xyzz = CS.d_xyzz + 512 * (size_t)p0;
+        fa.per = tree ? 5 : 3; fa.merged = mch ? 1 : 0; fa.fb4 = zk->d_fb4; fa.fb4g2 = zk->d_fb4g2; fa.out_xyzz = CS.d_xyzz + 512 * (size_t)p0;
         const bool g2_early = !sw::on<sw::ZKC_G2_LATE>();
         const bool g2_hold_env = sw::on<sw::ZKC_G2_ACC_HOLD>(), g2_early_env = sw::on<sw::ZKC_G2_ACC_EARLY>();
         const bool g2_acc_with_sort = g2_hold_env || ((nb < 32 || !one_lane) && !g2_early_env);
diff --git a/zk-franchise-proof-circuit_amd/csrc/zkc_prover.h b/zk-franchise-proof-circuit_amd/csrc/zkc_prover.h
--- a/zk-franchise-proof-circuit_amd/csrc/zkc_prover.h
+++ b/zk-franchise-proof-circuit_amd/csrc/zkc_prover.h
@@ -43,6 +43,7 @@
     uint32_t c, nw, vw;
     uint32_t ent_off, win_off;
     uint32_t bucket0, bin0, hbits, lbits, tile0, cnt0;
+    const uint32_t* scalars2; const uint32_t* vmap2; uint32_t count2; int32_t pt_shift2;
 };
 struct FinalizeArgs {
     const G1XYZZ* r1; const G2XYZZ* r2;
@@ -53,6 +54,7 @@
     const uint8_t* rs; uint8_t* out;
     void* scratch;
     int per; const G1XYZZ* fb4; const G2XYZZ* fb4g2;
+    int merged;
     uint8_t* out_xyzz;
 };
 constexpr int FB4_WIN = 64, FB4_ROW = 15;
@@ -70,8 +72,13 @@
         uint32_t vw = c >= 16 ? vw_big : vw_small;
         if (vw > (uint32_t)msm_half(c)) vw = (uint32_t)msm_half(c);
         while ((uint32_t)msm_half(c) / vw > max_vw_per_job) vw <<= 1;
-        j = MsmJob{scalars, vmap, count, tbl_off, tbl_count, pt_shift, (uint32_t)c, (uint32_t)msm_nw(c), vw, total_entries, total_windows, 0, 0, 0, 0, 0, 0};
+        j = MsmJob{scalars, vmap, count, tbl_off, tbl_count, pt_shift, (uint32_t)c, (uint32_t)msm_nw(c), vw, total_entries, total_windows, 0, 0, 0, 0, 0, 0, nullptr, nullptr, 0, 0};
         total_entries += count * (uint32_t)msm_nw(c); total_windows += (uint32_t)msm_half(c) / vw;
+    }
+    void add_tail(const uint32_t* scalars2, const uint32_t* vmap2, uint32_t count2, int32_t pt_shift2) {
+        MsmJob& j = job[njobs - 1];
+        j.scalars2 = scalars2; j.vmap2 = vmap2; j.count2 = count2; j.pt_shift2 = pt_shift2; j.count += count2;
+        total_entries += count2 * j.nw;
     }
     uint32_t max_vw_per_job = 256;
     void clear(uint32_t vw_small_jobs = 256, uint32_t vw_big_jobs = 1024, uint32_t max_per_job = 256) { vw_small = vw_small_jobs; vw_big = vw_big_jobs; max_vw_per_job = max_per_job; njobs = 0; total_buckets = total_entries = total_windows = total_bins = total_tiles = total_tilecnt = 0; hs = hb = nbig = 0; }
@@ -161,6 +168,7 @@
     uint32_t* d_g2_29 = nullptr;
     uint32_t* d_g2_29_lone = nullptr;
     uint32_t offA = 0, offB1 = 0, offC = 0, offH = 0;
+    bool merge_ch = false; uint32_t hTbl = 0;
     int c_deep = 0; uint32_t offA_deep = 0, offB1_deep = 0, offC_deep = 0; uint32_t* d_g2_29_deep = nullptr;
     int c_h = zkc::MSM_C_BIG;
     int c_sec = zkc::MSM_C_SMALL;
@@ -200,7 +208,7 @@
 namespace zkc {
 int ntt_run(zkc_ctx* ctx, hipStream_t st, const Fr* src, Fr* dst, const uint32_t* tw29, const Fr* scale, int logn, int nvec);
 int ntt_make_tw29(zkc_ctx* ctx, const Fr* d_tw, uint32_t count, uint32_t** out);
-int ntt_pair_run(zkc_ctx* ctx, hipStream_t st, Fr* data, const uint32_t* tw_inv29, const uint32_t* tw_fwd29, const Fr* scale_br, int logn, int nvec);
+int ntt_pair_run(zkc_ctx* ctx, hipStream_t st, Fr* data, const uint32_t* tw_inv29, const uint32_t* tw_fwd29, const Fr* scale_br, int logn, int nvec, bool form_c = false);
 int ntt_bitrev_table(zkc_ctx* ctx, const Fr* d_src, Fr** out, int logn);
 int msm_work_alloc(zkc_ctx* ctx, MsmWork& w, size_t max_entries, size_t max_buckets, int max_jobs, bool g2);
 void msm_work_free(MsmWork& w);
diff --git a/zk-franchise-proof-circuit_amd/csrc/zkc_switches.h b/zk-franchise-proof-circuit_amd/csrc/zkc_switches.h
--- a/zk-franchise-proof-circuit_amd/csrc/zkc_switches.h
+++ b/zk-franchise-proof-circuit_amd/csrc/zkc_switches.h
@@ -51,6 +51,7 @@
     X(ZKC_MATVEC_INLINE,        SET,         ANY, ANY,   PROCESS, "set (any value, 0 included): buildABC of the next pass is not prefetched on the blinding stream")              \
     X(ZKC_MV_PREFETCH_AT_NTT,   ON_IF_ONE,   ANY, ANY,   PROCESS, "=1: that prefetch starts beside the pass' bucketing instead of beside its accumulation")                       \
     X(ZKC_EARLY_LAYOUT,         OFF_IF_ZERO, ANY, ANY,   PROCESS, "=0: one-pass calls of more than two voters wait for their fold flags instead of reading the depths off the inputs") \
+    X(ZKC_MERGE_CH,             OFF_IF_ZERO, ANY, ANY,   LIVE,    "key load: =0 keeps the C section a job of its own with its own 12-bit tables instead of the tail of the H job")     \
     X(ZKC_NOFOLD_LISTS,         OFF_IF_ZERO, ANY, ANY,   PROCESS, "=0: unfolded passes keep the wires whose bases are at infinity")                                               \
     X(ZKC_NTT_SEPARATE,         SET,         ANY, ANY,   PROCESS, "set (any value, 0 included): two self-contained transforms instead of the fused pair")                         \
     X(ZKC_NTT_RADIX,            NUMBER,      ANY, ANY,   PROCESS, "below 4: the head transform kernel runs one stage at a time instead of two (4)")                               \
```

New measurement: 3172 (median of 6 runs). No clear change (+0.8%).
